# facebookresearch/detectron2

Measured on NVIDIA H100. Metric: Mask R-CNN R50-FPN training hot-path images/sec (custom-op path fwd+bwd, 2 images/GPU), higher is better.
Workload: dtype f32

## Files before the change

detectron2_b200/csrc/abi.cu:

```cuda
#include "common.cuh"

D2B_API int d2b_abi_version(void) { return D2B_ABI_VERSION; }
D2B_API int d2b_cuda_version(void) { return CUDART_VERSION; }
D2B_API const char* d2b_arch(void) { return "sm_90a"; }

namespace {
struct ZeroList {
  int n;
  void* p[D2B_MAX_ZERO];
  size_t bytes[D2B_MAX_ZERO];
  size_t blk0[D2B_MAX_ZERO + 1];
};
constexpr size_t kZeroChunk = 16384;

__global__ void __launch_bounds__(256) zero_buffers_kernel(const ZeroList z) {
  int i = 0;
  while (i + 1 < z.n && blockIdx.x >= z.blk0[i + 1]) ++i;
  const size_t off = (blockIdx.x - z.blk0[i]) * kZeroChunk;
  const size_t len = min(kZeroChunk, z.bytes[i] - off);
  char* base = (char*)z.p[i] + off;
  if ((reinterpret_cast<uintptr_t>(base) & 15) == 0) {
    uint4* q = reinterpret_cast<uint4*>(base);
    for (size_t e = threadIdx.x; e < len / 16; e += 256) q[e] = make_uint4(0u, 0u, 0u, 0u);
    for (size_t e = (len / 16) * 16 + threadIdx.x; e < len; e += 256) base[e] = 0;
  } else {
    for (size_t e = threadIdx.x; e < len; e += 256) base[e] = 0;
  }
}
}

int d2b_num_sms() {
  static std::atomic<int> cached[64];
  int dev = 0;
  if (cudaGetDevice(&dev) != cudaSuccess || dev < 0 || dev >= 64) return 132;
  int n = cached[dev].load(std::memory_order_relaxed);
  if (n <= 0) {
    if (cudaDeviceGetAttribute(&n, cudaDevAttrMultiProcessorCount, dev) != cudaSuccess || n <= 0) return 132;
    cached[dev].store(n, std::memory_order_relaxed);
  }
  return n;
}

int d2b_zero_buffers(void* const* ptrs, const size_t* bytes, int n, cudaStream_t stream) {
  ZeroList z = {};
  size_t blocks = 0;
  for (int i = 0; i < n && z.n < D2B_MAX_ZERO; ++i) {
    if (!ptrs[i] || !bytes[i]) continue;
    z.p[z.n] = ptrs[i];
    z.bytes[z.n] = bytes[i];
    z.blk0[z.n] = blocks;
    blocks += (bytes[i] + kZeroChunk - 1) / kZeroChunk;
    ++z.n;
  }
  z.blk0[z.n] = blocks;
  if (z.n == 0) return D2B_OK;
  if (blocks > 0x7fffffffULL) return D2B_EUNSUPPORTED;
  zero_buffers_kernel<<<(unsigned)blocks, 256, 0, stream>>>(z);
  D2B_CHECK_LAUNCH();
  return D2B_OK;
}
```

detectron2_b200/csrc/common.cuh:

```cuda
#pragma once
#include <cuda_runtime.h>
#include <stdint.h>

#include <atomic>

#include "../../include/d2b200.h"

#define D2B_API extern "C" __attribute__((visibility("default")))

#define D2B_CHECK_LAUNCH()                               \
  do {                                                   \
    cudaError_t e__ = cudaGetLastError();                \
    if (e__ != cudaSuccess) return (int)e__;             \
  } while (0)

#define D2B_CUDA(expr)                                   \
  do {                                                   \
    cudaError_t e__ = (expr);                            \
    if (e__ != cudaSuccess) return (int)e__;             \
  } while (0)

__host__ __device__ static inline int d2b_cdiv(long long a, long long b) { return (int)((a + b - 1) / b); }

int d2b_num_sms();

#define D2B_MAX_ZERO 8
int d2b_zero_buffers(void* const* ptrs, const size_t* bytes, int n, cudaStream_t stream);

#define D2B_ALLOW_BIG_SMEM(kernel)                                                                              \
  do {                                                                                                          \
    static std::atomic<unsigned long long> done__{0ull};                                                        \
    int dev__ = 0;                                                                                              \
    cudaError_t e__ = cudaGetDevice(&dev__);                                                                    \
    if (e__ != cudaSuccess) return (int)e__;                                                                    \
    const unsigned long long bit__ = 1ull << (dev__ & 63);                                                      \
    if (!(done__.load(std::memory_order_acquire) & bit__)) {                                                    \
      cudaFuncAttributes fa__;                                                                                  \
      e__ = cudaFuncGetAttributes(&fa__, kernel);                                                               \
      if (e__ != cudaSuccess) return (int)e__;                                                                  \
      e__ = cudaFuncSetAttribute(kernel, cudaFuncAttributeMaxDynamicSharedMemorySize,                           \
                                 227 * 1024 - (int)fa__.sharedSizeBytes);       \
      if (e__ != cudaSuccess) return (int)e__;                                                                  \
      done__.fetch_or(bit__, std::memory_order_release);                                                        \
    }                                                                                                           \
  } while (0)
```

detectron2_b200/csrc/deform_conv_tc.cu:

```cuda
#include <algorithm>
#include <cstdlib>

#include "common.cuh"
#include "tc_common.cuh"

using namespace d2b_tc;

namespace {

constexpr int kWorkerWarps = 16;
constexpr int kWorkers = kWorkerWarps * 32;
constexpr int kThreads = kWorkers + 128;
constexpr int kLaunchRegs = (65536 / kThreads) & ~7;
constexpr int kWorkerRegs = 112, kSideRegs = 24;
static_assert(kWorkers * kWorkerRegs + (kThreads - kWorkers) * kSideRegs <= kThreads * kLaunchRegs,
              "register budget exceeds the launch allocation");
constexpr int kMaxBN = 128;
constexpr int kRowsPerHalf = 128 / (2 * kWorkerWarps);
constexpr int kTile = 16384;
constexpr int kMaxSmem = 227 * 1024;
constexpr int kGcolPitch = 132;

struct TC {
  int N, Cin, H, W, Cout, kh, kw, sh, sw, ph, pw, dh, dw, G, DG, Ho, Wo, cpg, opg, cpdg, KK, HoWo;
  int pack, SG, cps, ops, cbs, U;
  int tiles_img;
  int stages_img;
  int MC;
  int nks;
  long long off_bs, mask_bs;
  int mask_sigmoid;
};

struct Epi {
  const float* scale;
  const float* shift;
  int relu;
};

struct K1P { int BN, noct, goct, nkp, ksplit, S, tap_bytes, stage_bytes, red; };
struct K2P { int mper, msplit, tap_bytes; };
struct K3P { int BN, noct, sper, nsplit, S, stage_bytes; };

inline size_t align256(size_t v) { return (v + 255) & ~(size_t)255; }

bool make_tc(const d2b_dcn_params* p, TC& d) {
  if (!p) return false;
  d.N = p->N; d.Cin = p->Cin; d.H = p->H; d.W = p->W; d.Cout = p->Cout; d.kh = p->kh; d.kw = p->kw;
  d.sh = p->stride_h; d.sw = p->stride_w; d.ph = p->pad_h; d.pw = p->pad_w; d.dh = p->dil_h; d.dw = p->dil_w;
  d.G = p->groups; d.DG = p->deformable_groups;
  if (d.N < 0 || d.Cin <= 0 || d.H <= 0 || d.W <= 0 || d.Cout <= 0 || d.kh <= 0 || d.kw <= 0 || d.sh <= 0 || d.sw <= 0 ||
      d.ph < 0 || d.pw < 0 || d.dh <= 0 || d.dw <= 0 || d.G <= 0 || d.DG <= 0)
    return false;
  if (d.Cin % d.G || d.Cout % d.G || d.Cin % d.DG) return false;
  d.Ho = (d.H + 2 * d.ph - (d.dh * (d.kh - 1) + 1)) / d.sh + 1;
  d.Wo = (d.W + 2 * d.pw - (d.dw * (d.kw - 1) + 1)) / d.sw + 1;
  if (d.Ho <= 0 || d.Wo <= 0) return false;
  d.cpg = d.Cin / d.G; d.opg = d.Cout / d.G; d.cpdg = d.Cin / d.DG; d.KK = d.kh * d.kw; d.HoWo = d.Ho * d.Wo;
  if (d.cpg >= 64) {
    if (d.cpg % 64) return false;
    d.pack = 1;
  } else {
    if (d.cpg != 16 && d.cpg != 32) return false;
    d.pack = 64 / d.cpg;
    if (d.G % d.pack) return false;
  }
  if (d.cpdg % 64) return false;
  d.SG = d.G / d.pack; d.cps = d.cpg * d.pack; d.ops = d.opg * d.pack; d.cbs = d.cps / 64; d.U = d.KK * d.cbs;
  if (d.ops % 16) return false;
  if (d.KK > 49) return false;
  if ((long long)d.H * d.W * d.Cin >= (1LL << 29)) return false;
  if ((long long)d.HoWo * d.Cout >= (1LL << 31) || (long long)d.Cout * d.cpg * d.KK >= (1LL << 31)) return false;
  d.tiles_img = d2b_cdiv(d.HoWo, 128);
  d.stages_img = d2b_cdiv(d.HoWo, 64);
  d.MC = (d.U + 1) / 2;
  d.nks = d.ops / 64;
  if ((long long)d.N * d.tiles_img > 0x7fffffffLL) return false;
  d.off_bs = (long long)d.DG * 2 * d.KK * d.HoWo;
  d.mask_bs = (long long)d.DG * d.KK * d.HoWo;
  d.mask_sigmoid = 0;
  return true;
}

const float* use_fused_offset_mask(TC& d, const float* offset_mask) {
  d.off_bs = d.mask_bs = (long long)d.DG * 3 * d.KK * d.HoWo;
  d.mask_sigmoid = 1;
  return offset_mask + (size_t)d.DG * 2 * d.KK * d.HoWo;
}

int largest_tile(int n) {
  for (int t = kMaxBN; t >= 16; t >>= 1)
    if (n % t == 0) return t;
  return 0;
}

int best_split(long long base, int work, int max_split, int overhead) {
  int best = 1;
  long long best_cost = -1;
  for (int s = 1; s <= max_split; ++s) {
    const int per = d2b_cdiv(work, s);
    const int parts = d2b_cdiv(work, per);
    const long long cost = (long long)d2b_cdiv(base * parts, d2b_num_sms()) * (per + overhead);
    if (best_cost < 0 || cost < best_cost) {
      best_cost = cost;
      best = parts;
    }
  }
  return best;
}

bool plan_k1(const TC& d, K1P& k, bool colfed = false) {
  k.BN = largest_tile(d.ops);
  if (k.BN < 16) return false;
  k.noct = d.ops / k.BN;
  k.goct = colfed ? 1 : k.noct;
  const int base = d.N * d.tiles_img * d.SG * k.goct;
  k.ksplit = best_split(base, d.KK, d.KK, 1);
  k.nkp = d2b_cdiv(d.KK, k.ksplit);
  k.ksplit = d2b_cdiv(d.KK, k.nkp);
  k.red = k.ksplit > 1;
  const int ndg = d.DG == 1 ? 1 : std::min(d.DG, d2b_cdiv(d.cps, d.cpdg) + 1);
  k.tap_bytes = ndg * k.nkp * 128 * 16;
  k.stage_bytes = 2 * kTile + 2 * k.BN * 128;
  k.S = 3;
  while (k.S > 1 && k.S * k.stage_bytes + k.tap_bytes + 1024 + 128 > kMaxSmem) --k.S;
  return k.S >= 2;
}

bool plan_k1c(const TC& d, K1P& k1, K1P& kc) {
  const long long base = (long long)d.N * d.tiles_img * d.SG * (k1.noct - 1);
  if (k1.goct != 1 || k1.noct < 2 || (long long)d.N * d.tiles_img * (k1.noct - 1) > 0x7fffffffLL) return false;
  kc = k1;
  kc.goct = k1.noct - 1;
  kc.ksplit = best_split(base, d.KK, d.KK, 1);
  kc.nkp = d2b_cdiv(d.KK, kc.ksplit);
  kc.ksplit = d2b_cdiv(d.KK, kc.nkp);
  kc.tap_bytes = 0;
  kc.S = 3;
  while (kc.S > 1 && kc.S * kc.stage_bytes + 1024 + 128 > kMaxSmem) --kc.S;
  if (kc.S < 2) return false;
  k1.red = kc.red = k1.ksplit > 1 || kc.ksplit > 1;
  return true;
}

bool plan_k2(const TC& d, K2P& k) {
  if (d.ops % 64) return false;
  const int base = d.N * d.tiles_img * d.SG;
  k.msplit = best_split(base, d.MC, d.MC, 1);
  k.mper = d2b_cdiv(d.MC, k.msplit);
  k.msplit = d2b_cdiv(d.MC, k.mper);
  const int nkp = std::min(d.KK, (2 * k.mper + d.cbs - 1) / d.cbs + 1);
  const int ndg = d.DG == 1 ? 1 : std::min(d.DG, d2b_cdiv(d.cps, d.cpdg) + 1);
  k.tap_bytes = ndg * nkp * 128 * 16;
  return 2 * 4 * kTile + 128 * kGcolPitch * 4 + k.tap_bytes + 1024 + 128 <= kMaxSmem;
}

bool plan_k3(const TC& d, K3P& k) {
  if (d.ops % 64) return false;
  k.BN = largest_tile(d.ops);
  k.noct = d.ops / k.BN;
  const int units = d.MC * d.SG * k.noct;
  const int total = d.N * d.stages_img;
  k.nsplit = best_split(units, total, std::min(total, 4 * d2b_num_sms()), 3);
  k.sper = d2b_cdiv(total, k.nsplit);
  k.nsplit = d2b_cdiv(total, k.sper);
  k.stage_bytes = 2 * kTile + 2 * k.BN * 128;
  k.S = 3;
  while (k.S > 1 && k.S * k.stage_bytes + 4096 + 1024 + 128 > kMaxSmem) --k.S;
  return k.S >= 2;
}

struct TapRaw {
  float oh, ow, m;
};

__device__ __forceinline__ TapRaw tap_loads(const TC& d, const float* __restrict__ offset, const float* __restrict__ mask,
                                            int b, int dg, int kp, int p) {
  TapRaw r = {0.f, 0.f, 1.f};
  if (p < d.HoWo) {
    const size_t ob = (size_t)b * d.off_bs + ((size_t)dg * 2 * d.KK) * d.HoWo;
    r.oh = __ldg(offset + ob + (size_t)(2 * kp) * d.HoWo + p);
    r.ow = __ldg(offset + ob + (size_t)(2 * kp + 1) * d.HoWo + p);
    if (mask) r.m = __ldg(mask + (size_t)b * d.mask_bs + ((size_t)dg * d.KK + kp) * d.HoWo + p);
  }
  return r;
}

__device__ __forceinline__ int4 tap_finish(const TC& d, const TapRaw& r, bool has_mask, int kp, int p) {
  int4 t = make_int4(0, 0, 0, 0);
  if (p < d.HoWo) {
    const int ho = p / d.Wo, wo = p - ho * d.Wo;
    const int ki = kp / d.kw, kj = kp - ki * d.kw;
    const float hf = (float)(ho * d.sh - d.ph + ki * d.dh) + r.oh;
    const float wf = (float)(wo * d.sw - d.pw + kj * d.dw) + r.ow;
    float m = r.m;
    if (has_mask && d.mask_sigmoid) m = 1.f / (1.f + expf(-m));
    if (hf > -1.f && wf > -1.f && hf < (float)d.H && wf < (float)d.W) {
      const float hfl = floorf(hf), wfl = floorf(wf);
      const int hl = (int)hfl, wl = (int)wfl;
      const bool t0 = hl >= 0, t1 = hl + 1 <= d.H - 1, l0 = wl >= 0, l1 = wl + 1 <= d.W - 1;
      const int flags = (t0 && l0 ? 1 : 0) | (t0 && l1 ? 2 : 0) | (t1 && l0 ? 4 : 0) | (t1 && l1 ? 8 : 0);
      t.x = ((hl * d.W + wl + d.W + 1) << 4) | flags;
      t.y = __float_as_int(hf - hfl);
      t.z = __float_as_int(wf - wfl);
      t.w = __float_as_int(m);
    }
  }
  return t;
}

__device__ __forceinline__ int4 make_tap(const TC& d, const float* __restrict__ offset, const float* __restrict__ mask,
                                         int b, int dg, int kp, int p) {
  return tap_finish(d, tap_loads(d, offset, mask, b, dg, kp, p), mask != nullptr, kp, p);
}

struct Taps4 {
  float4 v0, v1, v2, v3;
};

__device__ __forceinline__ void load_corners(const float* __restrict__ xcb, uint32_t Cin, uint32_t rs, int code, Taps4& t) {
  const float* __restrict__ p = xcb + (uint32_t)(code >> 4) * Cin;
  const float4 z = make_float4(0.f, 0.f, 0.f, 0.f);
  t.v0 = (code & 1) ? __ldg(reinterpret_cast<const float4*>(p)) : z;
  t.v1 = (code & 2) ? __ldg(reinterpret_cast<const float4*>(p + Cin)) : z;
  t.v2 = (code & 4) ? __ldg(reinterpret_cast<const float4*>(p + rs)) : z;
  t.v3 = (code & 8) ? __ldg(reinterpret_cast<const float4*>(p + (rs + Cin))) : z;
}

__device__ __forceinline__ void interp4(const Taps4& t, float w0, float w1, float w2, float w3, float (&v)[4]) {
  const F2 z = f2_pack(0.f, 0.f), p0 = f2_pack(w0, w0), p1 = f2_pack(w1, w1), p2 = f2_pack(w2, w2), p3 = f2_pack(w3, w3);
  F2 a = f2_fma(p0, f2_pack(t.v0.x, t.v0.y), z), b = f2_fma(p0, f2_pack(t.v0.z, t.v0.w), z);
  a = f2_fma(p1, f2_pack(t.v1.x, t.v1.y), a);
  b = f2_fma(p1, f2_pack(t.v1.z, t.v1.w), b);
  a = f2_fma(p2, f2_pack(t.v2.x, t.v2.y), a);
  b = f2_fma(p2, f2_pack(t.v2.z, t.v2.w), b);
  a = f2_fma(p3, f2_pack(t.v3.x, t.v3.y), a);
  b = f2_fma(p3, f2_pack(t.v3.z, t.v3.w), b);
  f2_unpack(a, v[0], v[1]);
  f2_unpack(b, v[2], v[3]);
}

__device__ __forceinline__ void gather_store(const Taps4& t, int4 tap, uint8_t* a_hi, uint8_t* a_lo, uint32_t off,
                                             bool split) {
  const float lh = __int_as_float(tap.y), lw = __int_as_float(tap.z), m = __int_as_float(tap.w);
  const float hh = 1.f - lh, hw = 1.f - lw;
  float v[4];
  interp4(t, hh * hw * m, hh * lw * m, lh * hw * m, lh * lw * m, v);
  uint2 hi, lo;
  split4(v, hi, lo);
  *reinterpret_cast<uint2*>(a_hi + off) = hi;
  if (split) *reinterpret_cast<uint2*>(a_lo + off) = lo;
}

template <int BN, int kTransA, int kSplit>
__device__ __forceinline__ void mma_stage_(float (&acc)[BN / 4], uint32_t a_hi, uint32_t a_lo, uint32_t b_hi, uint32_t b_lo) {
  const int g = (threadIdx.x >> 7);
  const uint32_t ao = kTransA ? (uint32_t)(g & 1) * 8192u : (uint32_t)(g & 1) * 64u * 128u;
  const uint32_t bo = (uint32_t)(g >> 1) * (uint32_t)(BN / 2) * 128u;
  const uint32_t lbo = kTransA ? 8192u : 0u;
  wgmma_fence();
#pragma unroll
  for (int kk = 0; kk < 4; ++kk) {
    const uint32_t ak = ao + (kTransA ? (uint32_t)kk * 2048u : (uint32_t)kk * 32u), bk = bo + (uint32_t)kk * 32u;
    Wgmma<BN / 2, kTransA>::mma(acc, wgmma_desc(a_hi + ak, lbo, 1024), wgmma_desc(b_hi + bk, 0, 1024), 1);
    if (kSplit) {
      Wgmma<BN / 2, kTransA>::mma(acc, wgmma_desc(a_hi + ak, lbo, 1024), wgmma_desc(b_lo + bk, 0, 1024), 1);
      Wgmma<BN / 2, kTransA>::mma(acc, wgmma_desc(a_lo + ak, lbo, 1024), wgmma_desc(b_hi + bk, 0, 1024), 1);
    }
  }
  wgmma_commit();
}
template <int BN, int kTransA>
__device__ __forceinline__ void mma_stage(float (&acc)[BN / 4], uint32_t a_hi, uint32_t a_lo, uint32_t b_hi, uint32_t b_lo,
                                          int split) {
  if (split) mma_stage_<BN, kTransA, 1>(acc, a_hi, a_lo, b_hi, b_lo);
  else mma_stage_<BN, kTransA, 0>(acc, a_hi, a_lo, b_hi, b_lo);
}

template <int BN>
__device__ __forceinline__ int acc_row(int i) {
  const int t = threadIdx.x & 127;
  return (threadIdx.x >> 7 & 1) * 64 + (t >> 5) * 16 + ((t & 31) >> 2) + ((i >> 1) & 1) * 8;
}
template <int BN>
__device__ __forceinline__ int acc_col(int i) {
  return (threadIdx.x >> 8) * (BN / 2) + (i >> 2) * 8 + (threadIdx.x & 3) * 2 + (i & 1);
}

template <int BN>
__device__ __forceinline__ void fwd_epilogue(const float (&acc)[BN / 4], const Epi& ep, const TC& d, const K1P& k,
                                             float* __restrict__ out, int b, int p0, int oc0) {
  const bool add_shift = ep.shift != nullptr && blockIdx.z == 0;
#pragma unroll
  for (int i = 0; i < BN / 4; ++i) {
    const int p = p0 + acc_row<BN>(i);
    if (p >= d.HoWo) continue;
    const int oc = oc0 + acc_col<BN>(i);
    float* dst = out + ((size_t)b * d.Cout + oc) * d.HoWo + p;
    float v = acc[i];
    if (k.red) {
      red_add(dst, v + ((add_shift && !ep.scale && !ep.relu) ? __ldg(ep.shift + oc) : 0.f));
    } else {
      if (ep.scale) v *= __ldg(ep.scale + oc);
      if (ep.shift) v += __ldg(ep.shift + oc);
      if (ep.relu) v = fmaxf(v, 0.f);
      *dst = v;
    }
  }
}

template <int BN>
__global__ void __launch_bounds__(kThreads, 1) dcn_fwd_tc_kernel(const float* __restrict__ xh,
                                                                   const float* __restrict__ offset,
                                                                   const float* __restrict__ mask,
                                                                   const uint8_t* __restrict__ wt, const Epi ep, const TC d,
                                                                   const K1P k, const int split, float* __restrict__ out,
                                                                   uint8_t* __restrict__ cols) {
  extern __shared__ uint8_t smem_raw[];
  uint8_t* smem = smem_raw + ((1024u - (smem_u32(smem_raw) & 1023u)) & 1023u);
  int4* taps = reinterpret_cast<int4*>(smem + k.S * k.stage_bytes);
  uint64_t* bars = reinterpret_cast<uint64_t*>(reinterpret_cast<uint8_t*>(taps) + k.tap_bytes);
  uint64_t* full_bar = bars;
  uint64_t* empty_bar = bars + k.S;

  const int tid = threadIdx.x, warp = tid >> 5, lane = tid & 31;
  const int b = blockIdx.x / d.tiles_img, p0 = (blockIdx.x - b * d.tiles_img) * 128;
  const int sg = blockIdx.y / k.goct, oct = blockIdx.y - sg * k.goct;
  const int kp0 = blockIdx.z * k.nkp, nkp = min(d.KK, kp0 + k.nkp) - kp0;
  const int nt = nkp * d.cbs;
  const int dg0 = (sg * d.cps) / d.cpdg;
  const bool saving = cols != nullptr && oct == 0;

  if (tid == 0) {
    for (int s = 0; s < k.S; ++s) {
      mbar_init(&full_bar[s], kWorkerWarps + 1);
      mbar_init(&empty_bar[s], kWorkerWarps + (saving ? 1 : 0));
    }
    mbar_init_fence();
  }
  if (tid < kWorkers) {
    const int ndg = ((sg + 1) * d.cps - 1) / d.cpdg - dg0 + 1;
    for (int i = tid; i < ndg * nkp * 128; i += kWorkers) {
      const int row = i & 127, r = i >> 7;
      const int dgl = r / nkp, kpl = r - dgl * nkp;
      taps[i] = make_tap(d, offset, mask, b, dg0 + dgl, kp0 + kpl, p0 + row);
    }
  }
  __syncthreads();
  if (warp < kWorkerWarps) reg_alloc<kWorkerRegs>();
  else reg_dealloc<kSideRegs>();

  if (warp < kWorkerWarps) {
    const int half = lane >> 4, q = lane & 15;
    const float* __restrict__ ximg = xh + (size_t)b * d.H * d.W * d.Cin - (size_t)(d.W + 1) * d.Cin;
    const uint32_t ucin = (uint32_t)d.Cin, urs = (uint32_t)(d.W * d.Cin);
    float acc[BN / 4];
#pragma unroll
    for (int i = 0; i < BN / 4; ++i) acc[i] = 0.f;
    int kpl = 0, cb = 0;
    auto stage = [&](int t) {
      const int s = t % k.S;
      const uint32_t par = (uint32_t)((t / k.S) & 1);
      const int cbase = sg * d.cps + cb * 64;
      const int4* __restrict__ tp = taps + ((cbase / d.cpdg - dg0) * nkp + kpl) * 128;
      const float* __restrict__ xc = ximg + cbase + q * 4;
      uint8_t* a_hi = smem + s * k.stage_bytes;
      uint8_t* a_lo = a_hi + kTile;
      mbar_wait(&empty_bar[s], par ^ 1u);
      {
        int4 tap[kRowsPerHalf];
        Taps4 c[kRowsPerHalf];
#pragma unroll
        for (int j = 0; j < kRowsPerHalf; ++j) tap[j] = tp[warp * 2 * kRowsPerHalf + j * 2 + half];
#pragma unroll
        for (int j = 0; j < kRowsPerHalf; ++j) load_corners(xc, ucin, urs, tap[j].x, c[j]);
#pragma unroll
        for (int j = 0; j < kRowsPerHalf; ++j) {
          const uint32_t r = (uint32_t)(warp * 2 * kRowsPerHalf + j * 2 + half);
          gather_store(c[j], tap[j], a_hi, a_lo, swz128(r, (uint32_t)(q >> 1)) + (uint32_t)(q & 1) * 8u, split != 0);
        }
      }
      fence_proxy_async();
      __syncwarp();
      if (lane == 0) mbar_arrive(&full_bar[s]);
      mbar_wait(&full_bar[s], par);
      const uint32_t sa = smem_u32(a_hi), sb = sa + 2 * kTile;
      mma_stage<BN, 0>(acc, sa, sa + kTile, sb, sb + (uint32_t)BN * 128u, split);
      if (++cb == d.cbs) { cb = 0; ++kpl; }
    };
    stage(0);
    for (int t = 1; t < nt; ++t) {
      stage(t);
      wgmma_wait<1>();
      __syncwarp();
      if (lane == 0) mbar_arrive(&empty_bar[(t - 1) % k.S]);
    }
    wgmma_wait<0>();
    fwd_epilogue<BN>(acc, ep, d, k, out, b, p0, sg * d.ops + oct * k.BN);
  } else if (warp == kWorkerWarps) {
    if (lane == 0) {
      const uint32_t bytes = (uint32_t)(split ? 2 : 1) * (uint32_t)k.BN * 128u;
      for (int t = 0; t < nt; ++t) {
        const int s = t % k.S;
        const uint32_t par = (uint32_t)((t / k.S) & 1);
        mbar_wait(&empty_bar[s], par ^ 1u);
        const size_t tile = ((size_t)(sg * k.noct + oct) * d.U + (size_t)kp0 * d.cbs + t);
        mbar_arrive_expect_tx(&full_bar[s], bytes);
        bulk_g2s(smem + s * k.stage_bytes + 2 * kTile, wt + tile * (size_t)(2 * k.BN * 128), bytes, &full_bar[s]);
      }
    }
  } else if (warp == kWorkerWarps + 1) {
    if (saving && lane == 0) {
      const uint32_t tile_bytes = (uint32_t)(split ? 2 : 1) * (uint32_t)kTile;
      for (int t = 0; t < nt; ++t) {
        const int s = t % k.S;
        const uint32_t par = (uint32_t)((t / k.S) & 1);
        mbar_wait(&full_bar[s], par);
        const size_t tile = ((size_t)blockIdx.x * d.SG + sg) * d.U + (size_t)kp0 * d.cbs + t;
        bulk_s2g(cols + tile * tile_bytes, smem + s * k.stage_bytes, tile_bytes);
        bulk_commit();
        bulk_wait_read0();
        mbar_arrive(&empty_bar[s]);
      }
      bulk_wait0();
    }
  }
}

template <int BN>
__global__ void __launch_bounds__(kThreads, 1) dcn_fwd_cols_kernel(const uint8_t* __restrict__ cols,
                                                                   const uint8_t* __restrict__ wt, const Epi ep, const TC d,
                                                                   const K1P k, const int split, float* __restrict__ out) {
  extern __shared__ uint8_t smem_raw[];
  uint8_t* smem = smem_raw + ((1024u - (smem_u32(smem_raw) & 1023u)) & 1023u);
  uint64_t* bars = reinterpret_cast<uint64_t*>(smem + k.S * k.stage_bytes);
  uint64_t* full_bar = bars;
  uint64_t* empty_bar = bars + k.S;

  const int tid = threadIdx.x, warp = tid >> 5, lane = tid & 31;
  const int tile = blockIdx.x / k.goct, oct = 1 + (blockIdx.x - tile * k.goct);
  const int b = tile / d.tiles_img, p0 = (tile - b * d.tiles_img) * 128;
  const int sg = blockIdx.y;
  const int kp0 = blockIdx.z * k.nkp, nkp = min(d.KK, kp0 + k.nkp) - kp0;
  const int nt = nkp * d.cbs;

  if (tid == 0) {
    for (int s = 0; s < k.S; ++s) {
      mbar_init(&full_bar[s], 1);
      mbar_init(&empty_bar[s], kWorkerWarps);
    }
    mbar_init_fence();
  }
  __syncthreads();
  if (warp < kWorkerWarps) reg_alloc<kWorkerRegs>();
  else reg_dealloc<kSideRegs>();

  if (warp < kWorkerWarps) {
    float acc[BN / 4];
#pragma unroll
    for (int i = 0; i < BN / 4; ++i) acc[i] = 0.f;
    auto issue = [&](int t) {
      const int s = t % k.S;
      mbar_wait(&full_bar[s], (uint32_t)((t / k.S) & 1));
      const uint32_t sa = smem_u32(smem + s * k.stage_bytes), sb = sa + 2 * kTile;
      mma_stage<BN, 0>(acc, sa, sa + kTile, sb, sb + (uint32_t)BN * 128u, split);
    };
    issue(0);
    for (int t = 1; t < nt; ++t) {
      issue(t);
      wgmma_wait<1>();
      __syncwarp();
      if (lane == 0) mbar_arrive(&empty_bar[(t - 1) % k.S]);
    }
    wgmma_wait<0>();
    fwd_epilogue<BN>(acc, ep, d, k, out, b, p0, sg * d.ops + oct * k.BN);
  } else if (warp == kWorkerWarps) {
    if (lane == 0) {
      const uint32_t parts = split ? 2u : 1u;
      const uint32_t abytes = parts * (uint32_t)kTile;
      const size_t u0 = (size_t)kp0 * d.cbs;
      const uint8_t* asrc = cols + (((size_t)tile * d.SG + sg) * d.U + u0) * abytes;
      const uint8_t* bsrc = wt + ((size_t)(sg * k.noct + oct) * d.U + u0) * (size_t)(2 * BN * 128);
      int s = 0;
      uint32_t par = 1u;
      for (int t = nt; t > 0; --t, asrc += abytes, bsrc += 2 * BN * 128) {
        mbar_wait(&empty_bar[s], par);
        mbar_arrive_expect_tx(&full_bar[s], abytes / 128u * (128u + BN));
        bulk_g2s(smem + s * k.stage_bytes, asrc, abytes, &full_bar[s]);
        bulk_g2s(smem + s * k.stage_bytes + 2 * kTile, bsrc, abytes / 128u * BN, &full_bar[s]);
        if (++s == k.S) {
          s = 0;
          par ^= 1u;
        }
      }
    }
  }
}

__global__ void __launch_bounds__(kThreads, 1) dcn_bwd_data_tc_kernel(const float* __restrict__ xh,
                                                                      const float* __restrict__ offset,
                                                                      const float* __restrict__ mask,
                                                                      const uint8_t* __restrict__ gt,
                                                                      const uint8_t* __restrict__ wt, const TC d,
                                                                      const K2P k, const int split,
                                                                      float* __restrict__ gxh, float* __restrict__ goff,
                                                                      float* __restrict__ gmask) {
  extern __shared__ uint8_t smem_raw[];
  uint8_t* smem = smem_raw + ((1024u - (smem_u32(smem_raw) & 1023u)) & 1023u);
  constexpr int kStage = 4 * kTile;
  float* gcol = reinterpret_cast<float*>(smem + 2 * kStage);
  int4* taps = reinterpret_cast<int4*>(smem + 2 * kStage + 128 * kGcolPitch * 4);
  uint64_t* bars = reinterpret_cast<uint64_t*>(reinterpret_cast<uint8_t*>(taps) + k.tap_bytes);
  uint64_t* full_bar = bars;
  uint64_t* empty_bar = bars + 2;

  const int tid = threadIdx.x, warp = tid >> 5, lane = tid & 31;
  const int b = blockIdx.x / d.tiles_img, pt = blockIdx.x - b * d.tiles_img, p0 = pt * 128;
  const int sg = blockIdx.y;
  const int m0 = blockIdx.z * k.mper, m1 = min(d.MC, m0 + k.mper), nm = m1 - m0;
  const int u_begin = 2 * m0, u_end = min(d.U, 2 * m1);
  const int kp0 = u_begin / d.cbs, nkp = (u_end - 1) / d.cbs - kp0 + 1;
  const int dg0 = (sg * d.cps) / d.cpdg;

  if (tid == 0) {
    for (int s = 0; s < 2; ++s) {
      mbar_init(&full_bar[s], 1);
      mbar_init(&empty_bar[s], kWorkerWarps);
    }
    mbar_init_fence();
  }
  if (tid < kWorkers) {
    const int ndg = ((sg + 1) * d.cps - 1) / d.cpdg - dg0 + 1;
    for (int i = tid; i < ndg * nkp * 128; i += kWorkers) {
      const int row = i & 127, r = i >> 7;
      const int dgl = r / nkp, kpl = r - dgl * nkp;
      taps[i] = make_tap(d, offset, mask, b, dg0 + dgl, kp0 + kpl, p0 + row);
    }
  }
  __syncthreads();
  if (warp < kWorkerWarps) reg_alloc<kWorkerRegs>();
  else reg_dealloc<kSideRegs>();

  if (warp < kWorkerWarps) {
    const int half = lane >> 4, q = lane & 15;
    const size_t img_off = (size_t)b * d.H * d.W * d.Cin - (size_t)(d.W + 1) * d.Cin;
    const float* __restrict__ ximg = xh + img_off;
    float* __restrict__ gimg = gxh ? gxh + img_off : nullptr;
    const uint32_t ucin = (uint32_t)d.Cin, urs = (uint32_t)(d.W * d.Cin);
    constexpr int R = kRowsPerHalf;
    float sh[R], sw[R], sm[R];
#pragma unroll
    for (int j = 0; j < R; ++j) sh[j] = sw[j] = sm[j] = 0.f;
    int cur_kp = -1, cur_dg = -1;

    auto flush = [&]() {
      if (cur_kp < 0) return;
      static_assert(R == 4, "the reduction below is written for 4 rows per half-warp");
      float v12[12];
#pragma unroll
      for (int j = 0; j < R; ++j) {
        v12[3 * j] = sh[j];
        v12[3 * j + 1] = sw[j];
        v12[3 * j + 2] = sm[j];
      }
      const bool b8 = q & 8, b4 = q & 4, b2 = q & 2, b1 = q & 1;
      float v6[6], v3[3];
#pragma unroll
      for (int i = 0; i < 6; ++i) {
        const float keep = b8 ? v12[i + 6] : v12[i], send = b8 ? v12[i] : v12[i + 6];
        v6[i] = keep + __shfl_xor_sync(0xffffffffu, send, 8);
      }
#pragma unroll
      for (int i = 0; i < 3; ++i) {
        const float keep = b4 ? v6[i + 3] : v6[i], send = b4 ? v6[i] : v6[i + 3];
        v3[i] = keep + __shfl_xor_sync(0xffffffffu, send, 4);
      }
      const float k0 = b2 ? v3[2] : v3[0], s0 = b2 ? v3[0] : v3[2];
      const float k1 = b2 ? 0.f : v3[1], s1 = b2 ? v3[1] : 0.f;
      const float u0 = k0 + __shfl_xor_sync(0xffffffffu, s0, 2);
      const float u1 = k1 + __shfl_xor_sync(0xffffffffu, s1, 2);
      float v = (b1 ? u1 : u0) + __shfl_xor_sync(0xffffffffu, b1 ? u0 : u1, 1);
      {
        const int j = q >> 2, which = q & 3;
        const int row = warp * 2 * R + j * 2 + half;
        const int p = p0 + row;
        if (which < 3 && p < d.HoWo) {
          if (which < 2) {
            if (goff) red_add(goff + (size_t)b * d.off_bs + ((size_t)cur_dg * 2 * d.KK + 2 * cur_kp + which) * d.HoWo + p, v);
          } else if (gmask) {
            if (d.mask_sigmoid) {
              const float m = __int_as_float(taps[((cur_dg - dg0) * nkp + (cur_kp - kp0)) * 128 + row].w);
              v *= m * (1.f - m);
            }
            red_add(gmask + (size_t)b * d.mask_bs + ((size_t)cur_dg * d.KK + cur_kp) * d.HoWo + p, v);
          }
        }
      }
#pragma unroll
      for (int j = 0; j < R; ++j) sh[j] = sw[j] = sm[j] = 0.f;
    };

    for (int ml = 0; ml < nm; ++ml) {
      const int buf = ml & 1;
      const int m = m0 + ml;
      const int nu = (2 * m + 1 < d.U) ? 2 : 1;
      {
        float acc[32];
#pragma unroll
        for (int i = 0; i < 32; ++i) acc[i] = 0.f;
        for (int ks = 0; ks < d.nks; ++ks) {
          const int c = ml * d.nks + ks, s = c & 1;
          mbar_wait(&full_bar[s], (uint32_t)((c >> 1) & 1));
          const uint32_t sa = smem_u32(smem + s * kStage);
          mma_stage<128, 0>(acc, sa, sa + kTile, sa + 2 * kTile, sa + 3 * kTile, split);
          wgmma_wait<0>();
          __syncwarp();
          if (lane == 0) mbar_arrive(&empty_bar[s]);
        }
#pragma unroll
        for (int i = 0; i < 32; i += 2)
          *reinterpret_cast<float2*>(gcol + acc_row<128>(i) * kGcolPitch + acc_col<128>(i)) = make_float2(acc[i], acc[i + 1]);
      }
      named_bar_sync(1, kWorkers);
      for (int ul = 0; ul < nu; ++ul) {
        const int u = 2 * m + ul;
        const int kp = u / d.cbs, cb = u - kp * d.cbs;
        const int cbase = sg * d.cps + cb * 64;
        const int dg = cbase / d.cpdg;
        if (kp != cur_kp || dg != cur_dg) {
          flush();
          cur_kp = kp;
          cur_dg = dg;
        }
        const int4* __restrict__ tp = taps + ((dg - dg0) * nkp + (kp - kp0)) * 128;
        const float* __restrict__ xc = ximg + cbase + q * 4;
        float* __restrict__ gc = gimg + cbase + q * 4;
        constexpr int kB2 = 2;
#pragma unroll
        for (int it = 0; it < R / kB2; ++it) {
          int4 tap[kB2];
          Taps4 c[kB2];
#pragma unroll
          for (int e = 0; e < kB2; ++e) tap[e] = tp[warp * 2 * R + (it * kB2 + e) * 2 + half];
#pragma unroll
          for (int e = 0; e < kB2; ++e) load_corners(xc, ucin, urs, tap[e].x, c[e]);
#pragma unroll
          for (int e = 0; e < kB2; ++e) {
            if ((tap[e].x & 15) == 0) continue;
            const int j = it * kB2 + e;
            const int row = warp * 2 * R + j * 2 + half;
            const float4 g4 = *reinterpret_cast<const float4*>(gcol + row * kGcolPitch + ul * 64 + q * 4);
            const float lh = __int_as_float(tap[e].y), lw = __int_as_float(tap[e].z), mk = __int_as_float(tap[e].w);
            const float hh = 1.f - lh, hw = 1.f - lw;
            const float w0 = hh * hw, w1 = hh * lw, w2 = lh * hw, w3 = lh * lw;
            const F2 LH = f2_pack(lh, lh), LW = f2_pack(lw, lw), HH = f2_pack(hh, hh), HW = f2_pack(hw, hw);
            const F2 W0 = f2_pack(w0, w0), W1 = f2_pack(w1, w1), W2 = f2_pack(w2, w2), W3 = f2_pack(w3, w3);
            const F2 MK = f2_pack(mk, mk);
            const F2 G[2] = {f2_pack(g4.x, g4.y), f2_pack(g4.z, g4.w)};
            const F2 A0[2] = {f2_pack(c[e].v0.x, c[e].v0.y), f2_pack(c[e].v0.z, c[e].v0.w)};
            const F2 A1[2] = {f2_pack(c[e].v1.x, c[e].v1.y), f2_pack(c[e].v1.z, c[e].v1.w)};
            const F2 A2[2] = {f2_pack(c[e].v2.x, c[e].v2.y), f2_pack(c[e].v2.z, c[e].v2.w)};
            const F2 A3[2] = {f2_pack(c[e].v3.x, c[e].v3.y), f2_pack(c[e].v3.z, c[e].v3.w)};
            F2 GM[2];
            F2 th2 = f2_pack(0.f, 0.f), tw2 = th2, tm2 = th2;
#pragma unroll
            for (int i = 0; i < 2; ++i) {
              GM[i] = f2_mul(G[i], MK);
              const F2 dh = f2_fma(LW, f2_sub(A3[i], A1[i]), f2_mul(HW, f2_sub(A2[i], A0[i])));
              const F2 dw = f2_fma(LH, f2_sub(A3[i], A2[i]), f2_mul(HH, f2_sub(A1[i], A0[i])));
              const F2 val = f2_fma(W3, A3[i], f2_fma(W2, A2[i], f2_fma(W1, A1[i], f2_mul(W0, A0[i]))));
              th2 = f2_fma(GM[i], dh, th2);
              tw2 = f2_fma(GM[i], dw, tw2);
              tm2 = f2_fma(G[i], val, tm2);
            }
            {
              float e0, e1;
              f2_unpack(th2, e0, e1);
              sh[j] += e0 + e1;
              f2_unpack(tw2, e0, e1);
              sw[j] += e0 + e1;
              f2_unpack(tm2, e0, e1);
              sm[j] += e0 + e1;
            }
            if (gimg) {
              float* gp = gc + (uint32_t)(tap[e].x >> 4) * ucin;
              red_add_v4_if(tap[e].x & 1, gp, f2_mul(GM[0], W0), f2_mul(GM[1], W0));
              red_add_v4_if(tap[e].x & 2, gp + ucin, f2_mul(GM[0], W1), f2_mul(GM[1], W1));
              red_add_v4_if(tap[e].x & 4, gp + urs, f2_mul(GM[0], W2), f2_mul(GM[1], W2));
              red_add_v4_if(tap[e].x & 8, gp + (urs + ucin), f2_mul(GM[0], W3), f2_mul(GM[1], W3));
            }
          }
        }
      }
      named_bar_sync(1, kWorkers);
    }
    flush();
  } else if (warp == kWorkerWarps) {
    if (lane == 0) {
      const uint32_t half_bytes = (uint32_t)(split ? 2 : 1) * (uint32_t)kTile;
      int c = 0;
      for (int ml = 0; ml < nm; ++ml) {
        const int m = m0 + ml;
        for (int ks = 0; ks < d.nks; ++ks, ++c) {
          const int s = c & 1;
          const uint32_t par = (uint32_t)((c >> 1) & 1);
          mbar_wait(&empty_bar[s], par ^ 1u);
          mbar_arrive_expect_tx(&full_bar[s], 2 * half_bytes);
          const size_t atile = (((size_t)b * d.tiles_img + pt) * d.SG + sg) * d.nks + ks;
          const size_t btile = ((size_t)sg * d.MC + m) * d.nks + ks;
          bulk_g2s(smem + s * kStage, gt + atile * (size_t)(2 * kTile), half_bytes, &full_bar[s]);
          bulk_g2s(smem + s * kStage + 2 * kTile, wt + btile * (size_t)(2 * kTile), half_bytes, &full_bar[s]);
        }
      }
    }
  }
}

template <int BN>
__device__ __forceinline__ void gw_tile_store(const float (&acc)[BN / 4], float* __restrict__ tile, int pitch) {
#pragma unroll
  for (int i = 0; i < BN / 4; i += 2) red_add_v2(tile + (size_t)acc_row<BN>(i) * pitch + acc_col<BN>(i), acc[i], acc[i + 1]);
}

__global__ void dcn_gw_reduce_kernel(const float* __restrict__ part, const TC d, float* __restrict__ gw) {
  const long long total = (long long)d.SG * d.U * 64 * d.ops;
  const long long idx = (long long)blockIdx.x * blockDim.x + threadIdx.x;
  if (idx >= total) return;
  const int ocl = (int)(idx % d.ops);
  const long long r = idx / d.ops;
  const int rowu = (int)(r % ((long long)d.U * 64)), sg = (int)(r / ((long long)d.U * 64));
  const int u = rowu >> 6, ch = rowu & 63;
  const int kp = u / d.cbs, cb = u - kp * d.cbs;
  const int ec = sg * d.cps + cb * 64 + ch, egrp = ec / d.cpg, ecin = ec - egrp * d.cpg;
  const int oc = sg * d.ops + ocl;
  if (oc / d.opg != egrp) return;
  gw[((size_t)oc * d.cpg + ecin) * d.KK + kp] = __ldg(part + ((size_t)sg * d.MC * 128 + rowu) * d.ops + ocl);
}

constexpr int kRedOc = 16, kRedCh = 16;
__global__ void __launch_bounds__(256) dcn_gw_reduce_tile_kernel(const float* __restrict__ part, const TC d,
                                                                  float* __restrict__ gw) {
  __shared__ float tile[9 * kRedCh][kRedOc + 1];
  const int per_sg = d.cps / kRedCh;
  const int sg = blockIdx.x / per_sg, c0 = (blockIdx.x - sg * per_sg) * kRedCh;
  const int cb = c0 >> 6, ch0 = c0 & 63;
  const int ocl0 = blockIdx.y * kRedOc;
  const int tid = threadIdx.x;
  {
    const int j = tid & (kRedOc - 1), r0 = tid / kRedOc;
    for (int row = r0; row < d.KK * kRedCh; row += 256 / kRedOc) {
      const int kp = row / kRedCh, ch = row - kp * kRedCh;
      tile[row][j] = __ldg(part + ((size_t)sg * d.MC * 128 + (size_t)(kp * d.cbs + cb) * 64 + ch0 + ch) * d.ops + ocl0 + j);
    }
  }
  __syncthreads();
  const int ec0 = sg * d.cps + c0;
  for (int i = tid; i < kRedOc * kRedCh * d.KK; i += 256) {
    const int j = i / (kRedCh * d.KK), e = i - j * (kRedCh * d.KK);
    const int ch = e / d.KK, kp = e - ch * d.KK;
    const int oc = sg * d.ops + ocl0 + j, grp = oc / d.opg;
    const int ec = ec0 + ch;
    if (ec / d.cpg == grp) gw[((size_t)oc * d.cpg + (ec - grp * d.cpg)) * d.KK + kp] = tile[kp * kRedCh + ch][j];
  }
}

template <int BN>
__global__ void __launch_bounds__(kThreads, 1) dcn_bwd_weight_tc_kernel(const float* __restrict__ xh,
                                                                        const float* __restrict__ offset,
                                                                        const float* __restrict__ mask,
                                                                        const uint8_t* __restrict__ gt, const TC d,
                                                                        const K3P k, const int split,
                                                                        float* __restrict__ gw) {
  extern __shared__ uint8_t smem_raw[];
  uint8_t* smem = smem_raw + ((1024u - (smem_u32(smem_raw) & 1023u)) & 1023u);
  int4* tap_s = reinterpret_cast<int4*>(smem + k.S * k.stage_bytes);
  uint64_t* bars = reinterpret_cast<uint64_t*>(reinterpret_cast<uint8_t*>(tap_s) + 4096);
  uint64_t* full_bar = bars;
  uint64_t* empty_bar = bars + k.S;

  const int tid = threadIdx.x, warp = tid >> 5, lane = tid & 31;
  const int mb = blockIdx.y;
  const int sg = blockIdx.x / k.noct, oct = blockIdx.x - sg * k.noct;
  const int total = d.N * d.stages_img;
  const int gs0 = blockIdx.z * k.sper, gs1 = min(total, gs0 + k.sper), ns = gs1 - gs0;

  if (tid == 0) {
    for (int s = 0; s < k.S; ++s) {
      mbar_init(&full_bar[s], kWorkerWarps + 1);
      mbar_init(&empty_bar[s], kWorkerWarps);
    }
    mbar_init_fence();
  }
  __syncthreads();
  if (warp < kWorkerWarps) reg_alloc<kWorkerRegs>();
  else reg_dealloc<kSideRegs>();

  if (warp < kWorkerWarps) {
    const int half = lane >> 4, q = lane & 15;
    const int u = 2 * mb + half;
    const bool u_ok = u < d.U;
    const int kp = u_ok ? u / d.cbs : 0, cb = u_ok ? u - kp * d.cbs : 0;
    const int cbase = sg * d.cps + cb * 64;
    const int dg = cbase / d.cpdg;
    constexpr int PX = 64 / kWorkerWarps;
    const int tl_half = (lane / PX) & 1, tl_j = lane % PX;
    const int tl_u = 2 * mb + tl_half;
    const bool tl_ok = lane < 2 * PX && tl_u < d.U;
    const int tl_kp = tl_ok ? tl_u / d.cbs : 0;
    const int tl_dg = tl_ok ? (sg * d.cps + (tl_u - tl_kp * d.cbs) * 64) / d.cpdg : 0;
    int4* my_taps = tap_s + warp * 2 * (2 * PX);
    auto stage_of = [&](int i, int& b, int& pbase) {
      const int gs = gs0 + i;
      b = gs / d.stages_img;
      pbase = (gs - b * d.stages_img) * 64;
    };
    if (ns > 0) {
      int b0, pb0;
      stage_of(0, b0, pb0);
      if (lane < 2 * PX) my_taps[lane] = tl_ok ? make_tap(d, offset, mask, b0, tl_dg, tl_kp, pb0 + warp * PX + tl_j) : make_int4(0, 0, 0, 0);
    }
    __syncwarp();
    float acc[BN / 4];
#pragma unroll
    for (int i = 0; i < BN / 4; ++i) acc[i] = 0.f;
    auto stage = [&](int i) {
      const int s = i % k.S;
      const uint32_t par = (uint32_t)((i / k.S) & 1);
      int b, pbase, bn = 0, pbn = 0;
      stage_of(i, b, pbase);
      const bool have_next = i + 1 < ns;
      TapRaw raw = {0.f, 0.f, 1.f};
      if (have_next) {
        stage_of(i + 1, bn, pbn);
        if (tl_ok) raw = tap_loads(d, offset, mask, bn, tl_dg, tl_kp, pbn + warp * PX + tl_j);
      }
      const float* __restrict__ xc = xh + ((size_t)b * d.H * d.W - (size_t)(d.W + 1)) * d.Cin + cbase + q * 4;
      const uint32_t ucin = (uint32_t)d.Cin, urs = (uint32_t)(d.W * d.Cin);
      uint8_t* a_hi = smem + s * k.stage_bytes + half * 8192;
      uint8_t* a_lo = a_hi + kTile;
      const int4* cur = my_taps + (i & 1) * (2 * PX) + half * PX;
      mbar_wait(&empty_bar[s], par ^ 1u);
      {
        int4 tap[PX];
        Taps4 c[PX];
#pragma unroll
        for (int j = 0; j < PX; ++j) tap[j] = cur[j];
#pragma unroll
        for (int j = 0; j < PX; ++j) load_corners(xc, ucin, urs, tap[j].x, c[j]);
#pragma unroll
        for (int j = 0; j < PX; ++j) {
          const uint32_t r = (uint32_t)(warp * PX + j);
          gather_store(c[j], tap[j], a_hi, a_lo, swz128(r, (uint32_t)(q >> 1)) + (uint32_t)(q & 1) * 8u, split != 0);
        }
      }
      if (have_next && lane < 2 * PX)
        my_taps[((i + 1) & 1) * (2 * PX) + lane] =
            tl_ok ? tap_finish(d, raw, mask != nullptr, tl_kp, pbn + warp * PX + tl_j) : make_int4(0, 0, 0, 0);
      fence_proxy_async();
      __syncwarp();
      if (lane == 0) mbar_arrive(&full_bar[s]);
      mbar_wait(&full_bar[s], par);
      const uint32_t sa = smem_u32(smem + s * k.stage_bytes), sb = sa + 2 * kTile;
      mma_stage<BN, 1>(acc, sa, sa + kTile, sb, sb + (uint32_t)BN * 128u, split);
    };
    stage(0);
    for (int i = 1; i < ns; ++i) {
      stage(i);
      wgmma_wait<1>();
      __syncwarp();
      if (lane == 0) mbar_arrive(&empty_bar[(i - 1) % k.S]);
    }
    wgmma_wait<0>();
    gw_tile_store<BN>(acc, gw + ((size_t)sg * d.MC * 128 + (size_t)mb * 128) * d.ops + (size_t)oct * k.BN, d.ops);
  } else if (warp == kWorkerWarps) {
    if (lane == 0) {
      const uint32_t bytes = (uint32_t)(split ? 2 : 1) * (uint32_t)k.BN * 128u;
      for (int i = 0; i < ns; ++i) {
        const int s = i % k.S;
        const uint32_t par = (uint32_t)((i / k.S) & 1);
        mbar_wait(&empty_bar[s], par ^ 1u);
        mbar_arrive_expect_tx(&full_bar[s], bytes);
        const size_t tile = ((size_t)(gs0 + i) * d.SG + sg) * k.noct + oct;
        bulk_g2s(smem + s * k.stage_bytes + 2 * kTile, gt + tile * (size_t)(2 * k.BN * 128), bytes, &full_bar[s]);
      }
    }
  }
}

template <int BN>
__global__ void __launch_bounds__(kThreads, 1) dcn_bwd_weight_cols_kernel(const uint8_t* __restrict__ cols,
                                                                          const uint8_t* __restrict__ gt, const TC d,
                                                                          const K3P k, const int S, const int split,
                                                                          float* __restrict__ gw) {
  extern __shared__ uint8_t smem_raw[];
  uint8_t* smem = smem_raw + ((1024u - (smem_u32(smem_raw) & 1023u)) & 1023u);
  uint64_t* bars = reinterpret_cast<uint64_t*>(smem + S * k.stage_bytes);
  uint64_t* full_bar = bars;
  uint64_t* empty_bar = bars + S;

  const int tid = threadIdx.x, warp = tid >> 5, lane = tid & 31;
  const int mb = blockIdx.y;
  const int sg = blockIdx.x / k.noct, oct = blockIdx.x - sg * k.noct;
  const int total = d.N * d.stages_img;
  const int gs0 = blockIdx.z * k.sper, gs1 = min(total, gs0 + k.sper), ns = gs1 - gs0;
  const int nu = (2 * mb + 1 < d.U) ? 2 : 1;

  if (tid == 0) {
    for (int s = 0; s < S; ++s) {
      mbar_init(&full_bar[s], 1);
      mbar_init(&empty_bar[s], kWorkerWarps);
    }
    mbar_init_fence();
  }
  if (nu == 1 && tid < kWorkers) {
    for (int s = 0; s < S; ++s)
      for (int i = tid; i < 2 * 512; i += kWorkers) {
        const int part = i >> 9, w = i & 511;
        reinterpret_cast<uint4*>(smem + s * k.stage_bytes + part * kTile + 8192)[w] = make_uint4(0, 0, 0, 0);
      }
    fence_proxy_async();
  }
  __syncthreads();
  if (warp < kWorkerWarps) reg_alloc<kWorkerRegs>();
  else reg_dealloc<kSideRegs>();

  if (warp < kWorkerWarps) {
    float acc[BN / 4];
#pragma unroll
    for (int i = 0; i < BN / 4; ++i) acc[i] = 0.f;
    auto issue = [&](int i) {
      const int s = i % S;
      mbar_wait(&full_bar[s], (uint32_t)((i / S) & 1));
      const uint32_t sa = smem_u32(smem + s * k.stage_bytes), sb = sa + 2 * kTile;
      mma_stage<BN, 1>(acc, sa, sa + kTile, sb, sb + (uint32_t)BN * 128u, split);
    };
    issue(0);
    for (int i = 1; i < ns; ++i) {
      issue(i);
      wgmma_wait<1>();
      __syncwarp();
      if (lane == 0) mbar_arrive(&empty_bar[(i - 1) % S]);
    }
    wgmma_wait<0>();
    gw_tile_store<BN>(acc, gw + ((size_t)sg * d.MC * 128 + (size_t)mb * 128) * d.ops + (size_t)oct * k.BN, d.ops);
  } else if (warp == kWorkerWarps) {
    if (lane == 0) {
      const uint32_t parts = split ? 2u : 1u;
      const uint32_t tile_bytes = parts * (uint32_t)kTile;
      const uint32_t gbytes = parts * (uint32_t)k.BN * 128u;
      for (int i = 0; i < ns; ++i) {
        const int s = i % S;
        const uint32_t par = (uint32_t)((i / S) & 1);
        const int gs = gs0 + i;
        const int b = gs / d.stages_img, st = gs - b * d.stages_img;
        mbar_wait(&empty_bar[s], par ^ 1u);
        mbar_arrive_expect_tx(&full_bar[s], (uint32_t)nu * parts * 8192u + gbytes);
        uint8_t* stage = smem + s * k.stage_bytes;
        const uint8_t* src =
            cols + ((((size_t)b * d.tiles_img + (st >> 1)) * d.SG + sg) * d.U + 2 * mb) * tile_bytes + (size_t)(st & 1) * 8192;
        for (int ul = 0; ul < nu; ++ul)
          for (uint32_t part = 0; part < parts; ++part)
            bulk_g2s(stage + part * kTile + ul * 8192, src + (size_t)ul * tile_bytes + (size_t)part * kTile, 8192u, &full_bar[s]);
        const size_t tile = ((size_t)gs * d.SG + sg) * k.noct + oct;
        bulk_g2s(stage + 2 * kTile, gt + tile * (size_t)(2 * k.BN * 128), gbytes, &full_bar[s]);
      }
    }
  }
}

__device__ __forceinline__ void split8(const float (&v)[8], uint4& hi, uint4& lo) {
  split2(v[0], v[1], hi.x, lo.x);
  split2(v[2], v[3], hi.y, lo.y);
  split2(v[4], v[5], hi.z, lo.z);
  split2(v[6], v[7], hi.w, lo.w);
}

__device__ __forceinline__ float w_elem(const float* __restrict__ w, const TC& d, int oc, int c, int kp) {
  const int g = c / d.cpg;
  if (oc / d.opg != g) return 0.f;
  return __ldg(w + ((size_t)oc * d.cpg + (c - g * d.cpg)) * d.KK + kp);
}

__global__ void dcn_wtile_fwd_kernel(const float* __restrict__ w, const TC d, int BN, int noct, uint8_t* __restrict__ dst) {
  const long long idx = (long long)blockIdx.x * blockDim.x + threadIdx.x;
  const long long total = (long long)d.SG * noct * d.U * BN * 8;
  if (idx >= total) return;
  const int c16 = (int)(idx & 7);
  const int r = (int)((idx >> 3) % BN);
  const long long tile = idx / (8LL * BN);
  const int u = (int)(tile % d.U);
  const int oct = (int)((tile / d.U) % noct);
  const int sg = (int)(tile / ((long long)d.U * noct));
  const int kp = u / d.cbs, cb = u - kp * d.cbs;
  const int oc = sg * d.ops + oct * BN + r;
  float v[8];
#pragma unroll
  for (int e = 0; e < 8; ++e) v[e] = w_elem(w, d, oc, sg * d.cps + cb * 64 + c16 * 8 + e, kp);
  uint4 hi, lo;
  split8(v, hi, lo);
  uint8_t* base = dst + tile * (size_t)(2 * BN * 128);
  *reinterpret_cast<uint4*>(base + swz128((uint32_t)r, (uint32_t)c16)) = hi;
  *reinterpret_cast<uint4*>(base + BN * 128 + swz128((uint32_t)r, (uint32_t)c16)) = lo;
}

__global__ void dcn_wtile_bwd_kernel(const float* __restrict__ w, const TC d, uint8_t* __restrict__ dst) {
  const long long idx = (long long)blockIdx.x * blockDim.x + threadIdx.x;
  const long long total = (long long)d.SG * d.MC * d.nks * 128 * 8;
  if (idx >= total) return;
  const int c16 = (int)(idx & 7);
  const int r = (int)((idx >> 3) & 127);
  const long long tile = idx >> 10;
  const int ks = (int)(tile % d.nks);
  const int m = (int)((tile / d.nks) % d.MC);
  const int sg = (int)(tile / ((long long)d.nks * d.MC));
  const int u = 2 * m + (r >> 6);
  float v[8];
#pragma unroll
  for (int e = 0; e < 8; ++e) v[e] = 0.f;
  if (u < d.U) {
    const int kp = u / d.cbs, cb = u - kp * d.cbs;
    const int c = sg * d.cps + cb * 64 + (r & 63);
#pragma unroll
    for (int e = 0; e < 8; ++e) v[e] = w_elem(w, d, sg * d.ops + ks * 64 + c16 * 8 + e, c, kp);
  }
  uint4 hi, lo;
  split8(v, hi, lo);
  uint8_t* base = dst + tile * (size_t)(2 * kTile);
  *reinterpret_cast<uint4*>(base + swz128((uint32_t)r, (uint32_t)c16)) = hi;
  *reinterpret_cast<uint4*>(base + kTile + swz128((uint32_t)r, (uint32_t)c16)) = lo;
}

__device__ __forceinline__ float gout_elem(const float* __restrict__ gout, const float* __restrict__ ysaved, const Epi& ep,
                                           size_t idx, int oc) {
  float g = __ldg(gout + idx);
  if (ep.relu && !(__ldg(ysaved + idx) > 0.f)) g = 0.f;
  if (ep.scale) g *= __ldg(ep.scale + oc);
  return g;
}

__global__ void __launch_bounds__(256) dcn_gout_px_tiles_kernel(const float* __restrict__ gout,
                                                                const float* __restrict__ ysaved, const Epi ep, const TC d,
                                                                uint8_t* __restrict__ dst, uint8_t* __restrict__ dst_oc,
                                                                int BN, int noct) {
  __shared__ float t[64][33];
  const long long tile = blockIdx.x;
  const int ks = (int)(tile % d.nks);
  const int sg = (int)((tile / d.nks) % d.SG);
  const int pt = (int)((tile / ((long long)d.nks * d.SG)) % d.tiles_img);
  const int b = (int)(tile / ((long long)d.nks * d.SG * d.tiles_img));
  const int r0 = blockIdx.y * 32;
  const int p0 = pt * 128 + r0, oc0 = sg * d.ops + ks * 64;
  const int tid = threadIdx.x;
#pragma unroll
  for (int i = 0; i < 8; ++i) {
    const int e = tid + i * 256;
    const int o = e >> 5, pp = e & 31;
    const int p = p0 + pp;
    t[o][pp] = p < d.HoWo ? gout_elem(gout, ysaved, ep, ((size_t)b * d.Cout + oc0 + o) * d.HoWo + p, oc0 + o) : 0.f;
  }
  __syncthreads();
  uint8_t* base = dst + tile * (size_t)(2 * kTile);
  {
    const int r = tid >> 3, c16 = tid & 7;
    float v[8];
#pragma unroll
    for (int i = 0; i < 8; ++i) v[i] = t[c16 * 8 + i][r];
    uint4 hi, lo;
    split8(v, hi, lo);
    *reinterpret_cast<uint4*>(base + swz128((uint32_t)(r0 + r), (uint32_t)c16)) = hi;
    *reinterpret_cast<uint4*>(base + kTile + swz128((uint32_t)(r0 + r), (uint32_t)c16)) = lo;
  }
  if (dst_oc) {
    const int o = tid >> 2, ch = tid & 3;
    const int ocs = ks * 64 + o;
    const int oct = ocs / BN, row = ocs - oct * BN;
    const int pglob = pt * 128 + r0;
    const int ps = pglob >> 6, c16 = ((pglob & 63) >> 3) + ch;
    float v[8];
#pragma unroll
    for (int i = 0; i < 8; ++i) v[i] = t[o][ch * 8 + i];
    uint4 hi, lo;
    split8(v, hi, lo);
    if (ps < d.stages_img) {
      const size_t tile_oc = (((size_t)b * d.stages_img + ps) * d.SG + sg) * noct + oct;
      uint8_t* bo = dst_oc + tile_oc * (size_t)(2 * BN * 128);
      *reinterpret_cast<uint4*>(bo + swz128((uint32_t)row, (uint32_t)c16)) = hi;
      *reinterpret_cast<uint4*>(bo + BN * 128 + swz128((uint32_t)row, (uint32_t)c16)) = lo;
    }
  }
}

__global__ void dcn_gout_oc_tiles_kernel(const float* __restrict__ gout, const float* __restrict__ ysaved, const Epi ep,
                                         const TC d, int BN, int noct, uint8_t* __restrict__ dst) {
  const long long idx = (long long)blockIdx.x * blockDim.x + threadIdx.x;
  const long long total = (long long)d.N * d.stages_img * d.SG * noct * BN * 8;
  if (idx >= total) return;
  const int c16 = (int)(idx & 7);
  const int r = (int)((idx >> 3) % BN);
  const long long tile = idx / (8LL * BN);
  const int oct = (int)(tile % noct);
  const int sg = (int)((tile / noct) % d.SG);
  const int ps = (int)((tile / ((long long)noct * d.SG)) % d.stages_img);
  const int b = (int)(tile / ((long long)noct * d.SG * d.stages_img));
  const int oc = sg * d.ops + oct * BN + r;
  const size_t src = ((size_t)b * d.Cout + oc) * d.HoWo;
  float v[8];
#pragma unroll
  for (int e = 0; e < 8; ++e) {
    const int p = ps * 64 + c16 * 8 + e;
    v[e] = p < d.HoWo ? gout_elem(gout, ysaved, ep, src + p, oc) : 0.f;
  }
  uint4 hi, lo;
  split8(v, hi, lo);
  uint8_t* base = dst + tile * (size_t)(2 * BN * 128);
  *reinterpret_cast<uint4*>(base + swz128((uint32_t)r, (uint32_t)c16)) = hi;
  *reinterpret_cast<uint4*>(base + BN * 128 + swz128((uint32_t)r, (uint32_t)c16)) = lo;
}

__global__ void __launch_bounds__(256) nhwc_to_nchw_kernel(const float* __restrict__ src, int C, int HW,
                                                           float* __restrict__ dst) {
  __shared__ float t[64][33];
  const int hw0 = blockIdx.x * 64, c0 = blockIdx.y * 32;
  const float* __restrict__ s = src + (size_t)blockIdx.z * HW * C;
  float* __restrict__ o = dst + (size_t)blockIdx.z * C * HW;
  const int tid = threadIdx.x;
  for (int e = tid; e < 64 * 32; e += 256) {
    const int pp = e >> 5, cc = e & 31;
    t[pp][cc] = (hw0 + pp < HW && c0 + cc < C) ? __ldg(s + (size_t)(hw0 + pp) * C + c0 + cc) : 0.f;
  }
  __syncthreads();
  for (int e = tid; e < 64 * 32; e += 256) {
    const int cc = e >> 6, pp = e & 63;
    if (hw0 + pp < HW && c0 + cc < C) o[(size_t)(c0 + cc) * HW + hw0 + pp] = t[pp][cc];
  }
}

__global__ void dcn_epilogue_kernel(float* __restrict__ y, long long total, int Cout, int HoWo, const Epi ep) {
  const long long i = (long long)blockIdx.x * blockDim.x + threadIdx.x;
  if (i >= total) return;
  const int oc = (int)((i / HoWo) % Cout);
  float v = y[i];
  if (ep.scale) v *= __ldg(ep.scale + oc);
  if (ep.shift) v += __ldg(ep.shift + oc);
  if (ep.relu) v = fmaxf(v, 0.f);
  y[i] = v;
}

int to_nhwc(const float* x, const TC& d, float* dst, cudaStream_t stream) {
  d2b_pyramid P = {};
  P.num_levels = 1;
  P.feat[0] = x;
  P.H[0] = d.H;
  P.W[0] = d.W;
  P.scale[0] = 1.f;
  float* dsts[1] = {dst};
  return d2b_pyramid_nchw_to_nhwc(&P, d.N, d.Cin, dsts, (void*)stream);
}

}

int d2b_deform_conv_tc_supported(const d2b_dcn_params* p) {
  TC d;
  K1P k1;
  return make_tc(p, d) && plan_k1(d, k1);
}

int d2b_deform_conv_tc_bwd_supported(const d2b_dcn_params* p) {
  TC d;
  K2P k2;
  K3P k3;
  return make_tc(p, d) && plan_k2(d, k2) && plan_k3(d, k3);
}

size_t d2b_deform_conv_tc_fwd_workspace(const d2b_dcn_params* p, int x_nhwc) {
  TC d;
  K1P k;
  if (!make_tc(p, d) || !plan_k1(d, k)) return 0;
  size_t b = align256((size_t)d.SG * k.noct * d.U * 2 * k.BN * 128);
  if (!x_nhwc) b += align256(sizeof(float) * (size_t)d.N * d.H * d.W * d.Cin);
  return b;
}

size_t d2b_deform_conv_tc_cols_bytes(const d2b_dcn_params* p, int precision) {
  TC d;
  K1P k;
  if (precision == 0 || !make_tc(p, d) || !plan_k1(d, k)) return 0;
  return (size_t)d.N * d.tiles_img * d.SG * d.U * (size_t)(precision == 1 ? 2 : 1) * kTile;
}

int d2b_deform_conv_forward_tc(const float* x, const float* offset, const float* mask, const float* weight,
                               const float* scale, const float* shift, int relu, const d2b_dcn_params* p, int precision,
                               int tcflags, float* out, void* cols, void* workspace, size_t workspace_bytes, void* stream_) {
  cudaStream_t stream = (cudaStream_t)stream_;
  const int x_nhwc = tcflags & 1;
  TC d;
  K1P k;
  if (!make_tc(p, d) || !plan_k1(d, k)) return D2B_EUNSUPPORTED;
  if (d.N == 0) return D2B_OK;
  if (tcflags & 2) {
    if (mask) return D2B_EINVAL;
    mask = use_fused_offset_mask(d, offset);
  }
  if (!workspace || workspace_bytes < d2b_deform_conv_tc_fwd_workspace(p, x_nhwc)) return D2B_EWORKSPACE;
  if ((reinterpret_cast<uintptr_t>(workspace) & 255) || (x_nhwc && (reinterpret_cast<uintptr_t>(x) & 15)) ||
      (reinterpret_cast<uintptr_t>(cols) & 15))
    return D2B_EINVAL;
  uint8_t* ws = reinterpret_cast<uint8_t*>(workspace);
  uint8_t* wt = ws;
  ws += align256((size_t)d.SG * k.noct * d.U * 2 * k.BN * 128);
  const float* xh = x;
  if (!x_nhwc) {
    float* xn = reinterpret_cast<float*>(ws);
    int rc = to_nhwc(x, d, xn, stream);
    if (rc) return rc;
    xh = xn;
  }
  {
    const long long total = (long long)d.SG * k.noct * d.U * k.BN * 8;
    dcn_wtile_fwd_kernel<<<d2b_cdiv(total, 256), 256, 0, stream>>>(weight, d, k.BN, k.noct, wt);
    D2B_CHECK_LAUNCH();
  }
  K1P kc;
  bool colfed = false;
  if (cols && k.noct > 1) {
    K1P k1;
    if (plan_k1(d, k1, true) && plan_k1c(d, k1, kc)) {
      k = k1;
      colfed = true;
    }
  }
  if (k.red) D2B_CUDA(cudaMemsetAsync(out, 0, sizeof(float) * (size_t)d.N * d.Cout * d.HoWo, stream));
  const int smem_bytes = k.S * k.stage_bytes + k.tap_bytes + 1024 + 128;
  const int split = precision == 1 ? 1 : 0;
  const Epi ep = {scale, shift, relu};
  dim3 grid(d.N * d.tiles_img, d.SG * k.goct, k.ksplit);
#define D2B_LAUNCH_K1(BN)                                                                                              \
  {                                                                                                                    \
    D2B_ALLOW_BIG_SMEM(dcn_fwd_tc_kernel<BN>);                                                                         \
    dcn_fwd_tc_kernel<BN><<<grid, kThreads, smem_bytes, stream>>>(xh, offset, mask, wt, ep, d, k, split, out,        \
                                                                    reinterpret_cast<uint8_t*>(cols));                 \
  }
  if (k.BN == 16) D2B_LAUNCH_K1(16)
  else if (k.BN == 32) D2B_LAUNCH_K1(32)
  else if (k.BN == 64) D2B_LAUNCH_K1(64)
  else D2B_LAUNCH_K1(128)
#undef D2B_LAUNCH_K1
  D2B_CHECK_LAUNCH();
  if (colfed) {
    const int smem_c = kc.S * kc.stage_bytes + 1024 + 128;
    dim3 grid_c(d.N * d.tiles_img * kc.goct, d.SG, kc.ksplit);
    const uint8_t* cl = reinterpret_cast<const uint8_t*>(cols);
#define D2B_LAUNCH_K1C(BN)                                                                                             \
  {                                                                                                                    \
    D2B_ALLOW_BIG_SMEM(dcn_fwd_cols_kernel<BN>);                                                                       \
    dcn_fwd_cols_kernel<BN><<<grid_c, kThreads, smem_c, stream>>>(cl, wt, ep, d, kc, split, out);                      \
  }
    if (kc.BN == 16) D2B_LAUNCH_K1C(16)
    else if (kc.BN == 32) D2B_LAUNCH_K1C(32)
    else if (kc.BN == 64) D2B_LAUNCH_K1C(64)
    else D2B_LAUNCH_K1C(128)
#undef D2B_LAUNCH_K1C
    D2B_CHECK_LAUNCH();
  }
  if (k.red && (scale || relu)) {
    const long long total = (long long)d.N * d.Cout * d.HoWo;
    dcn_epilogue_kernel<<<d2b_cdiv(total, 256), 256, 0, stream>>>(out, total, d.Cout, d.HoWo, ep);
    D2B_CHECK_LAUNCH();
  }
  return D2B_OK;
}

size_t d2b_deform_conv_tc_bwd_workspace(const d2b_dcn_params* p, int x_nhwc, int need_data, int need_weight) {
  TC d;
  K2P k2;
  K3P k3;
  if (!make_tc(p, d) || !plan_k2(d, k2) || !plan_k3(d, k3)) return 0;
  size_t b = 0;
  const size_t xbytes = align256(sizeof(float) * (size_t)d.N * d.H * d.W * d.Cin);
  if (!x_nhwc) b += xbytes;
  if (need_data && !x_nhwc) b += xbytes;
  if (need_data) {
    b += align256((size_t)d.N * d.tiles_img * d.SG * d.nks * 2 * kTile);
    b += align256((size_t)d.SG * d.MC * d.nks * 2 * kTile);
  }
  if (need_weight) {
    b += align256((size_t)d.N * d.stages_img * d.SG * k3.noct * 2 * k3.BN * 128);
    b += align256(sizeof(float) * (size_t)d.SG * d.MC * 128 * d.ops);
  }
  return b;
}

int d2b_deform_conv_backward_tc(const float* x, const float* offset, const float* mask, const float* weight,
                                const float* grad_out, const float* scale, const float* y_saved, int relu,
                                const d2b_dcn_params* p, int precision, int tcflags, const void* cols, float* grad_x,
                                float* grad_offset, float* grad_mask, float* grad_weight, void* workspace,
                                size_t workspace_bytes, void* stream_) {
  cudaStream_t stream = (cudaStream_t)stream_;
  const int x_nhwc = tcflags & 1;
  TC d;
  K2P k2;
  K3P k3;
  if (!make_tc(p, d) || !plan_k2(d, k2) || !plan_k3(d, k3)) return D2B_EUNSUPPORTED;
  const int need_data = (grad_x || grad_offset || grad_mask) ? 1 : 0, need_weight = grad_weight ? 1 : 0;
  const bool fused_om = (tcflags & 2) != 0;
  if (fused_om && (mask || grad_mask)) return D2B_EINVAL;
  if (relu && !y_saved) return D2B_EINVAL;
  const size_t nx = (size_t)d.N * d.H * d.W * d.Cin, noff = (size_t)d.N * d.DG * (fused_om ? 3 : 2) * d.KK * d.HoWo;
  const size_t nm = (size_t)d.N * d.DG * d.KK * d.HoWo, nw = (size_t)d.Cout * d.cpg * d.KK;
  if (fused_om) {
    mask = use_fused_offset_mask(d, offset);
    if (grad_offset) grad_mask = grad_offset + (size_t)d.DG * 2 * d.KK * d.HoWo;
  }
  const Epi ep = {scale, nullptr, relu};
  if (d.N == 0 || (!need_data && !need_weight)) {
    void* zp[3] = {grad_offset, fused_om ? nullptr : grad_mask, grad_weight};
    size_t zb[3] = {noff * 4, nm * 4, nw * 4};
    return d2b_zero_buffers(zp, zb, 3, stream);
  }
  if (!workspace || workspace_bytes < d2b_deform_conv_tc_bwd_workspace(p, x_nhwc, need_data, need_weight)) return D2B_EWORKSPACE;
  if ((reinterpret_cast<uintptr_t>(workspace) & 255) || (x_nhwc && (reinterpret_cast<uintptr_t>(x) & 15)) ||
      (x_nhwc && grad_x && (reinterpret_cast<uintptr_t>(grad_x) & 15)) || (reinterpret_cast<uintptr_t>(cols) & 15))
    return D2B_EINVAL;
  const int split = precision == 1 ? 1 : 0;
  uint8_t* ws = reinterpret_cast<uint8_t*>(workspace);
  const size_t xbytes = align256(sizeof(float) * nx);
  const float* xh = x;
  if (!x_nhwc) {
    float* xn = reinterpret_cast<float*>(ws);
    ws += xbytes;
    int rc = to_nhwc(x, d, xn, stream);
    if (rc) return rc;
    xh = xn;
  }
  float* gxh = nullptr;
  if (need_data && grad_x) gxh = x_nhwc ? grad_x : reinterpret_cast<float*>(ws);
  uint8_t* gt_px = nullptr;
  uint8_t* wt = nullptr;
  if (need_data) {
    if (!x_nhwc) ws += xbytes;
    gt_px = ws;
    ws += align256((size_t)d.N * d.tiles_img * d.SG * d.nks * 2 * kTile);
    wt = ws;
    ws += align256((size_t)d.SG * d.MC * d.nks * 2 * kTile);
  }
  uint8_t* gt_oc = need_weight ? ws : nullptr;
  float* gw_part = nullptr;
  if (need_weight) {
    ws += align256((size_t)d.N * d.stages_img * d.SG * k3.noct * 2 * k3.BN * 128);
    gw_part = reinterpret_cast<float*>(ws);
  }
  {
    void* zp[4] = {grad_offset, fused_om ? nullptr : grad_mask, gxh, gw_part};
    size_t zb[4] = {noff * 4, nm * 4, nx * 4, sizeof(float) * (size_t)d.SG * d.MC * 128 * d.ops};
    int rc = d2b_zero_buffers(zp, zb, 4, stream);
    if (rc) return rc;
  }
  if (need_data) {
    dcn_gout_px_tiles_kernel<<<dim3((unsigned)((size_t)d.N * d.tiles_img * d.SG * d.nks), 4), 256, 0, stream>>>(
        grad_out, y_saved, ep, d, gt_px, gt_oc, k3.BN, k3.noct);
    D2B_CHECK_LAUNCH();
    {
      const long long total = (long long)d.SG * d.MC * d.nks * 128 * 8;
      dcn_wtile_bwd_kernel<<<d2b_cdiv(total, 256), 256, 0, stream>>>(weight, d, wt);
      D2B_CHECK_LAUNCH();
    }
    const int smem_bytes = 2 * 4 * kTile + 128 * kGcolPitch * 4 + k2.tap_bytes + 1024 + 128;
    D2B_ALLOW_BIG_SMEM(dcn_bwd_data_tc_kernel);
    dim3 grid(d.N * d.tiles_img, d.SG, k2.msplit);
    dcn_bwd_data_tc_kernel<<<grid, kThreads, smem_bytes, stream>>>(xh, offset, mask, gt_px, wt, d, k2, split, gxh, grad_offset,
                                                                  mask ? grad_mask : nullptr);
    D2B_CHECK_LAUNCH();
    if (grad_x && !x_nhwc) {
      dim3 g2(d2b_cdiv(d.H * d.W, 64), d2b_cdiv(d.Cin, 32), d.N);
      nhwc_to_nchw_kernel<<<g2, 256, 0, stream>>>(gxh, d.Cin, d.H * d.W, grad_x);
      D2B_CHECK_LAUNCH();
    }
  }
  if (need_weight) {
    if (!need_data) {
      const long long total = (long long)d.N * d.stages_img * d.SG * k3.noct * k3.BN * 8;
      dcn_gout_oc_tiles_kernel<<<d2b_cdiv(total, 256), 256, 0, stream>>>(grad_out, y_saved, ep, d, k3.BN, k3.noct, gt_oc);
      D2B_CHECK_LAUNCH();
    }
    dim3 grid(d.SG * k3.noct, d.MC, k3.nsplit);
    if (cols) {
      const int S = std::min(6, (kMaxSmem - 2048) / k3.stage_bytes);
      const int smem_bytes = S * k3.stage_bytes + 1024 + 128;
      const uint8_t* cl = reinterpret_cast<const uint8_t*>(cols);
#define D2B_LAUNCH_K3C(BN)                                                                                             \
  {                                                                                                                      \
    D2B_ALLOW_BIG_SMEM(dcn_bwd_weight_cols_kernel<BN>);                                                                \
    dcn_bwd_weight_cols_kernel<BN><<<grid, kThreads, smem_bytes, stream>>>(cl, gt_oc, d, k3, S, split, gw_part);       \
  }
      if (k3.BN == 64) D2B_LAUNCH_K3C(64)
      else D2B_LAUNCH_K3C(128)
#undef D2B_LAUNCH_K3C
    } else {
      const int smem_bytes = k3.S * k3.stage_bytes + 4096 + 1024 + 128;
#define D2B_LAUNCH_K3(BN)                                                                                              \
  {                                                                                                                      \
    D2B_ALLOW_BIG_SMEM(dcn_bwd_weight_tc_kernel<BN>);                                                                  \
    dcn_bwd_weight_tc_kernel<BN><<<grid, kThreads, smem_bytes, stream>>>(xh, offset, mask, gt_oc, d, k3, split, gw_part); \
  }
      if (k3.BN == 64) D2B_LAUNCH_K3(64)
      else D2B_LAUNCH_K3(128)
#undef D2B_LAUNCH_K3
    }
    D2B_CHECK_LAUNCH();
    {
      if (d.KK <= 9) {
        dcn_gw_reduce_tile_kernel<<<dim3(d.SG * (d.cps / kRedCh), d.ops / kRedOc), 256, 0, stream>>>(gw_part, d, grad_weight);
      } else {
        const long long total = (long long)d.SG * d.U * 64 * d.ops;
        dcn_gw_reduce_kernel<<<d2b_cdiv(total, 256), 256, 0, stream>>>(gw_part, d, grad_weight);
      }
      D2B_CHECK_LAUNCH();
    }
  }
  return D2B_OK;
}
```

detectron2_b200/csrc/roi_align.cu:

```cuda
#include <cuda_bf16.h>
#include <cuda_fp16.h>

#include <algorithm>

#include "common.cuh"

namespace {

constexpr int kThreads = 256;

template <int DT>
struct Elem;
template <>
struct Elem<D2B_F32> {
  using T = float;
  static __device__ __forceinline__ float ld(const T* __restrict__ p) { return __ldg(p); }
  static __device__ __forceinline__ void st(T* __restrict__ p, float v) { *p = v; }
};
template <>
struct Elem<D2B_F16> {
  using T = __half;
  static __device__ __forceinline__ float ld(const T* __restrict__ p) { return __half2float(__ldg(p)); }
  static __device__ __forceinline__ void st(T* __restrict__ p, float v) { *p = __float2half_rn(v); }
};
template <>
struct Elem<D2B_BF16> {
  using T = __nv_bfloat16;
  static __device__ __forceinline__ float ld(const T* __restrict__ p) { return __bfloat162float(__ldg(p)); }
  static __device__ __forceinline__ void st(T* __restrict__ p, float v) { *p = __float2bfloat16_rn(v); }
};
#define D2B_DISPATCH_DTYPE(dt, ...)                  \
  do {                                               \
    if ((dt) == D2B_F32) {                           \
      constexpr int DT = D2B_F32;                    \
      __VA_ARGS__;                                   \
    } else if ((dt) == D2B_F16) {                    \
      constexpr int DT = D2B_F16;                    \
      __VA_ARGS__;                                   \
    } else {                                         \
      constexpr int DT = D2B_BF16;                   \
      __VA_ARGS__;                                   \
    }                                                \
  } while (0)
static inline bool dtype_ok(int dt) { return dt == D2B_F32 || dt == D2B_F16 || dt == D2B_BF16; }

struct RoiGeom {
  int b;
  float start_h, start_w, bin_h, bin_w;
  int gh, gw;
  float inv_count;
  float count_raw;
  float ctr_h, ctr_w, cos_t, sin_t;
};

struct Pyr {
  int num_levels;
  const float* feat[D2B_MAX_LEVELS];
  float* grad[D2B_MAX_LEVELS];
  int H[D2B_MAX_LEVELS], W[D2B_MAX_LEVELS];
  float scale[D2B_MAX_LEVELS];
  int min_level, max_level, canonical_level;
  float canonical_box_size;
  const float* level_rois;
};

template <bool ROT = false>
__device__ __forceinline__ int pick_level(const Pyr& P, const float* __restrict__ roi) {
  if (P.num_levels == 1) return 0;
  const float area = ROT ? roi[3] * roi[4] : (roi[3] - roi[1]) * (roi[4] - roi[2]);
  const float size = sqrtf(area);
  float lvl = floorf((float)P.canonical_level + log2f(size / P.canonical_box_size + 1e-8f));
  if (!(lvl == lvl)) return -1;
  lvl = fminf(fmaxf(lvl, (float)P.min_level), (float)P.max_level);
  return (int)lvl - P.min_level;
}

template <bool ROT>
__device__ __forceinline__ RoiGeom load_geom(const float* __restrict__ roi, float scale, int PH, int PW, int sr,
                                             int aligned, bool dead = false) {
  RoiGeom g;
  g.b = (int)roi[0];
  float rw, rh;
  if (ROT) {
    g.ctr_w = roi[1] * scale - 0.5f;
    g.ctr_h = roi[2] * scale - 0.5f;
    rw = roi[3] * scale;
    rh = roi[4] * scale;
    float theta = (float)((double)roi[5] * 3.14159265358979323846 / 180.0);
    sincosf(theta, &g.sin_t, &g.cos_t);
    g.start_h = -rh / 2.0f;
    g.start_w = -rw / 2.0f;
  } else {
    float off = aligned ? 0.5f : 0.0f;
    float sw = roi[1] * scale - off, sh = roi[2] * scale - off;
    float ew = roi[3] * scale - off, eh = roi[4] * scale - off;
    rw = ew - sw;
    rh = eh - sh;
    if (!aligned) {
      rw = fmaxf(rw, 1.f);
      rh = fmaxf(rh, 1.f);
    }
    g.start_h = sh;
    g.start_w = sw;
    g.ctr_h = g.ctr_w = 0.f;
    g.cos_t = 1.f;
    g.sin_t = 0.f;
  }
  g.bin_h = rh / (float)PH;
  g.bin_w = rw / (float)PW;
  g.gh = sr > 0 ? sr : (int)ceilf(rh / (float)PH);
  g.gw = sr > 0 ? sr : (int)ceilf(rw / (float)PW);
  if (g.gh < 0) g.gh = 0;
  if (g.gw < 0) g.gw = 0;
  if (dead) g.gh = g.gw = 0;
  int c = g.gh * g.gw;
  g.count_raw = (float)c;
  g.inv_count = 1.0f / (float)(c < 1 ? 1 : c);
  return g;
}

struct Tap1 {
  int lo, hi;
  float wl, wh;
};

__device__ __forceinline__ Tap1 make_tap1(float v, int size) {
  Tap1 t;
  if (v < -1.0f || v > (float)size) {
    t.lo = t.hi = 0;
    t.wl = t.wh = 0.f;
    return t;
  }
  v = fmaxf(v, 0.f);
  int lo = (int)v;
  int hi;
  if (lo >= size - 1) {
    hi = lo = size - 1;
    v = (float)lo;
  } else {
    hi = lo + 1;
  }
  float l = v - (float)lo;
  t.lo = lo;
  t.hi = hi;
  t.wh = l;
  t.wl = 1.f - l;
  return t;
}

struct Tap2 {
  int p1, p2, p3, p4;
  float w1, w2, w3, w4;
};

__device__ __forceinline__ Tap2 make_tap2(float y, float x, int H, int W) {
  Tap2 t;
  if (y < -1.0f || y > (float)H || x < -1.0f || x > (float)W) {
    t.p1 = t.p2 = t.p3 = t.p4 = -1;
    t.w1 = t.w2 = t.w3 = t.w4 = 0.f;
    return t;
  }
  Tap1 ty = make_tap1(y, H), tx = make_tap1(x, W);
  t.p1 = ty.lo * W + tx.lo;
  t.p2 = ty.lo * W + tx.hi;
  t.p3 = ty.hi * W + tx.lo;
  t.p4 = ty.hi * W + tx.hi;
  t.w1 = ty.wl * tx.wl;
  t.w2 = ty.wl * tx.wh;
  t.w3 = ty.wh * tx.wl;
  t.w4 = ty.wh * tx.wh;
  return t;
}

__device__ __forceinline__ void rot_xy(const RoiGeom& g, int ph, int pw, int iy, int ix, float& y, float& x) {
  float yy = g.start_h + (float)ph * g.bin_h + ((float)iy + .5f) * g.bin_h / (float)g.gh;
  float xx = g.start_w + (float)pw * g.bin_w + ((float)ix + .5f) * g.bin_w / (float)g.gw;
  y = yy * g.cos_t - xx * g.sin_t + g.ctr_h;
  x = yy * g.sin_t + xx * g.cos_t + g.ctr_w;
}

template <int MAXTAP>
__global__ void __launch_bounds__(kThreads) roi_align_rot_fwd_kernel(const Pyr P, const float* __restrict__ rois,
                                                                     int C, int PH, int PW, int sr, int c_per_cta,
                                                                     float* __restrict__ out) {
  __shared__ Tap2 taps[MAXTAP];
  const int k = blockIdx.x;
  const int c0 = blockIdx.y * c_per_cta;
  const int cn = min(c_per_cta, C - c0);
  const int lvl_raw = pick_level<true>(P, rois + (size_t)k * 6);
  const int lvl = max(lvl_raw, 0);
  const float* __restrict__ in = P.feat[lvl];
  const int H = P.H[lvl], W = P.W[lvl];
  const RoiGeom g = load_geom<true>(rois + (size_t)k * 6, P.scale[lvl], PH, PW, sr, 1, lvl_raw < 0);
  const int bins = PH * PW;
  const int spb = g.gh * g.gw;
  const long long ntap = (long long)bins * spb;
  const bool tab = ntap <= MAXTAP;
  if (tab) {
    for (int i = threadIdx.x; i < (int)ntap; i += kThreads) {
      int bin = i / spb, s = i - bin * spb;
      int ph = bin / PW, pw = bin - ph * PW, iy = s / g.gw, ix = s - iy * g.gw;
      float y, x;
      rot_xy(g, ph, pw, iy, ix, y, x);
      taps[i] = make_tap2(y, x, H, W);
    }
    __syncthreads();
  }
  const int total = cn * bins;
  const float* __restrict__ base = in + ((size_t)g.b * C + c0) * H * W;
  float* __restrict__ obase = out + ((size_t)k * C + c0) * bins;
  for (int idx = threadIdx.x; idx < total; idx += kThreads) {
    int c = idx / bins, bin = idx - c * bins;
    int ph = bin / PW, pw = bin - ph * PW;
    const float* __restrict__ plane = base + (size_t)c * H * W;
    float acc = 0.f;
    for (int s = 0; s < spb; ++s) {
      Tap2 t;
      if (tab) t = taps[bin * spb + s];
      else {
        int iy = s / g.gw, ix = s - iy * g.gw;
        float y, x;
        rot_xy(g, ph, pw, iy, ix, y, x);
        t = make_tap2(y, x, H, W);
      }
      if (t.p1 >= 0)
        acc += t.w1 * __ldg(plane + t.p1) + t.w2 * __ldg(plane + t.p2) + t.w3 * __ldg(plane + t.p3) +
               t.w4 * __ldg(plane + t.p4);
    }
    obase[idx] = acc * g.inv_count;
  }
}

template <bool ROT>
__global__ void __launch_bounds__(kThreads) roi_align_bwd_kernel(const Pyr P, const float* __restrict__ gout,
                                                                 const float* __restrict__ rois, int C, int PH, int PW,
                                                                 int sr, int aligned, int c_per_cta) {
  const int k = blockIdx.x;
  const int c0 = blockIdx.y * c_per_cta;
  const int cn = min(c_per_cta, C - c0);
  const int lvl_raw = ROT ? pick_level<true>(P, rois + (size_t)k * 6)
                          : pick_level(P, (P.level_rois ? P.level_rois : rois) + (size_t)k * 5);
  const int lvl = max(lvl_raw, 0);
  float* __restrict__ gin = P.grad[lvl];
  const int H = P.H[lvl], W = P.W[lvl];
  const RoiGeom g = load_geom<ROT>(rois + (size_t)k * (ROT ? 6 : 5), P.scale[lvl], PH, PW, sr, aligned, lvl_raw < 0);
  if (g.gh <= 0 || g.gw <= 0) return;
  const int bins = PH * PW;
  const int total = cn * bins;
  float* __restrict__ base = gin + ((size_t)g.b * C + c0) * H * W;
  const float* __restrict__ gbase = gout + ((size_t)k * C + c0) * bins;
  for (int idx = threadIdx.x; idx < total; idx += kThreads) {
    int c = idx / bins, bin = idx - c * bins;
    int ph = bin / PW, pw = bin - ph * PW;
    float* __restrict__ plane = base + (size_t)c * H * W;
    const float gv = gbase[idx];
    for (int iy = 0; iy < g.gh; ++iy)
      for (int ix = 0; ix < g.gw; ++ix) {
        float y, x;
        if (ROT) rot_xy(g, ph, pw, iy, ix, y, x);
        else {
          y = g.start_h + (float)ph * g.bin_h + ((float)iy + .5f) * g.bin_h / (float)g.gh;
          x = g.start_w + (float)pw * g.bin_w + ((float)ix + .5f) * g.bin_w / (float)g.gw;
        }
        Tap2 t = make_tap2(y, x, H, W);
        if (t.p1 < 0) continue;
        atomicAdd(plane + t.p1, gv * t.w1 / g.count_raw);
        atomicAdd(plane + t.p2, gv * t.w2 / g.count_raw);
        atomicAdd(plane + t.p3, gv * t.w3 / g.count_raw);
        atomicAdd(plane + t.p4, gv * t.w4 / g.count_raw);
      }
  }
}

constexpr int kMaxE = 32;
constexpr int kMaxP = 16;
constexpr int kChW = 4;
constexpr int kV3Warps = 8;
constexpr int kV3Threads = kV3Warps * 32;
constexpr int kCapPx = 448;
constexpr int kRowoffCap = 1536;

struct CTap {
  int idx;
  float w;
};

__device__ __forceinline__ void add_tap(CTap* list, int stride, int& n, int idx, float w, int& overflow) {
  if (w == 0.f) return;
  for (int e = 0; e < n; ++e)
    if (list[e * stride].idx == idx) {
      list[e * stride].w += w;
      return;
    }
  if (n >= kMaxE) {
    overflow = 1;
    return;
  }
  list[n * stride].idx = idx;
  list[n * stride].w = w;
  ++n;
}

template <bool BWD>
__global__ void __launch_bounds__(kV3Threads, 3) roi_align_v3_kernel(const Pyr P, const float* __restrict__ rois, int C,
                                                                     int PH, int PW, int sr, int aligned,
                                                                     int groups_per_cta, const float* __restrict__ gout,
                                                                     float* __restrict__ out) {
  extern __shared__ __align__(16) float stage_all[];
  __shared__ CTap ytab[kMaxE * kMaxP];
  __shared__ CTap xtab[kMaxE * kMaxP];
  __shared__ int rowoff[kRowoffCap];
  __shared__ int yn[kMaxP], xn[kMaxP], ylo[kMaxP], yhi[kMaxP];
  __shared__ int band_ph0[kMaxP + 1], band_yb[kMaxP], band_npx[kMaxP];
  __shared__ int s_overflow, s_tapov, s_xmin, s_xmax, s_nbands, s_direct, s_nyu, s_nxu, s_ymin, s_ymax;

  const int k = blockIdx.x;
  const int tid = threadIdx.x, lane = tid & 31, warp = tid >> 5;
  const int lvl_raw = pick_level(P, (P.level_rois ? P.level_rois : rois) + (size_t)k * 5);
  const int lvl = max(lvl_raw, 0);
  const float* __restrict__ in = BWD ? nullptr : P.feat[lvl];
  float* __restrict__ gin = BWD ? P.grad[lvl] : nullptr;
  const int H = P.H[lvl], W = P.W[lvl];
  const RoiGeom g = load_geom<false>(rois + (size_t)k * 5, P.scale[lvl], PH, PW, sr, aligned, lvl_raw < 0);
  const int bins = PH * PW;
  const int ngroup = d2b_cdiv(C, kChW);
  const int g_begin = blockIdx.y * groups_per_cta, g_end = min(ngroup, g_begin + groups_per_cta);

  if (tid == 0) {
    s_overflow = (PH > kMaxP || PW > kMaxP) ? 1 : 0;
    s_tapov = 0;
    s_xmin = 1 << 30;
    s_xmax = -1;
  }
  __syncthreads();
  if (!s_overflow) {
    if (tid < PH) {
      CTap* list = ytab + tid;
      int n = 0, ov = 0, lo = 1 << 30, hi = -1;
      for (int iy = 0; iy < g.gh; ++iy) {
        Tap1 t = make_tap1(g.start_h + (float)tid * g.bin_h + ((float)iy + .5f) * g.bin_h / (float)g.gh, H);
        add_tap(list, kMaxP, n, t.lo, t.wl, ov);
        add_tap(list, kMaxP, n, t.hi, t.wh, ov);
      }
      for (int e = 0; e < n; ++e) {
        lo = min(lo, list[e * kMaxP].idx);
        hi = max(hi, list[e * kMaxP].idx);
      }
      yn[tid] = n;
      ylo[tid] = lo;
      yhi[tid] = hi;
      if (ov) atomicOr(&s_tapov, 1);
    } else if (tid >= 32 && tid < 32 + PW) {
      const int pw = tid - 32;
      CTap* list = xtab + pw;
      int n = 0, ov = 0;
      for (int ix = 0; ix < g.gw; ++ix) {
        Tap1 t = make_tap1(g.start_w + (float)pw * g.bin_w + ((float)ix + .5f) * g.bin_w / (float)g.gw, W);
        add_tap(list, kMaxP, n, t.lo, t.wl, ov);
        add_tap(list, kMaxP, n, t.hi, t.wh, ov);
      }
      for (int e = 0; e < n; ++e) {
        atomicMin(&s_xmin, list[e * kMaxP].idx);
        atomicMax(&s_xmax, list[e * kMaxP].idx);
      }
      xn[pw] = n;
      if (ov) atomicOr(&s_tapov, 1);
    }
  }
  __syncthreads();
  const int xmin = s_xmin, fw = s_xmax - s_xmin + 1;
  if (tid == 0) {
    const int overflow = s_overflow | s_tapov;
    int direct = overflow, nb = 0, nyu = 0, nxu = 0, ymin = 1 << 30, ymax = -1;
    if (!direct) {
      for (int ph = 0; ph < PH; ++ph) {
        nyu = max(nyu, yn[ph]);
        if (yn[ph] > 0) {
          ymin = min(ymin, ylo[ph]);
          ymax = max(ymax, yhi[ph]);
        }
      }
      for (int pw = 0; pw < PW; ++pw) nxu = max(nxu, xn[pw]);
    }
    if (!direct && fw > 0 && ymax >= ymin) {
      if ((long long)(ymax - ymin + 1) * fw > kRowoffCap) direct = 1;
      int ph0 = 0;
      while (ph0 < PH && !direct) {
        int yb = 1 << 30, ye = -1, ph1 = ph0;
        while (ph1 < PH) {
          int nyb = yb, nye = ye;
          if (yn[ph1] > 0) {
            nyb = min(yb, ylo[ph1]);
            nye = max(ye, yhi[ph1]);
          }
          if (nye >= nyb && (nye - nyb + 1) * fw > kCapPx) {
            if (ph1 == ph0) direct = 1;
            break;
          }
          yb = nyb;
          ye = nye;
          ++ph1;
        }
        band_ph0[nb] = ph0;
        band_yb[nb] = (ye >= yb) ? yb : ymin;
        band_npx[nb] = (ye >= yb) ? (ye - yb + 1) * fw : 0;
        ++nb;
        ph0 = ph1;
      }
    } else if (!direct) {
      band_ph0[0] = 0;
      band_yb[0] = 0;
      band_npx[0] = 0;
      nb = 1;
      nyu = nxu = 0;
      ymin = 0;
      ymax = -1;
    }
    band_ph0[nb] = PH;
    s_nbands = nb;
    int mode = overflow ? 2 : (direct ? 1 : 0);
    if (mode == 0 && fw > 0 && ymax >= ymin) {
      int sy = 0, sx = 0;
      for (int ph = 0; ph < PH; ++ph) sy += yn[ph];
      for (int pw = 0; pw < PW; ++pw) sx += xn[pw];
      if (2LL * sy * sx < (long long)(ymax - ymin + 1) * fw) mode = 1;
    }
    direct = mode;
    s_direct = direct;
    s_nyu = nyu;
    s_nxu = nxu;
    s_ymin = ymin;
    s_ymax = ymax;
  }
  __syncthreads();
  const int mode = s_direct;
  const bool direct = mode == 2;
  const int nbands = s_nbands, nyu = s_nyu, nxu = s_nxu, ymin = s_ymin;
  if (mode != 2) {
    if (tid < PH) {
      const int n = yn[tid];
      const int fill = n > 0 ? ytab[tid].idx : 0;
      for (int e = n; e < nyu; ++e) ytab[e * kMaxP + tid] = CTap{fill, 0.f};
    } else if (tid >= 32 && tid < 32 + PW) {
      const int pw = tid - 32, n = xn[pw];
      for (int e = 0; e < n; ++e) xtab[e * kMaxP + pw].idx -= xmin;
      for (int e = n; e < ((nxu + 3) & ~3); ++e) xtab[e * kMaxP + pw] = CTap{0, 0.f};
    }
    if (mode == 0 && fw > 0 && s_ymax >= ymin) {
      const int npx_all = (s_ymax - ymin + 1) * fw;
      for (int i = tid; i < npx_all; i += kV3Threads) {
        const int y = i / fw, x = i - y * fw;
        rowoff[i] = (ymin + y) * W + xmin + x;
      }
    }
  }
  __syncthreads();

  float* __restrict__ st = stage_all + (size_t)warp * kChW * kCapPx;
  for (int grp = g_begin + warp; grp < g_end; grp += kV3Warps) {
    const int c0 = grp * kChW;
    const int cn = min(kChW, C - c0);
    const float* __restrict__ base = BWD ? nullptr : in + ((size_t)g.b * C + c0) * H * W;
    float* __restrict__ gbase = BWD ? gin + ((size_t)g.b * C + c0) * H * W : nullptr;
    float* __restrict__ obase = BWD ? nullptr : out + ((size_t)k * C + c0) * bins;
    const float* __restrict__ gobase = BWD ? gout + ((size_t)k * C + c0) * bins : nullptr;
    if (direct && BWD) {
      for (int idx = lane; idx < cn * bins; idx += 32) {
        const int c = idx / bins, bin = idx - c * bins;
        const int ph = bin / PW, pw = bin - ph * PW;
        float* __restrict__ plane = gbase + (size_t)c * H * W;
        const float gv = gobase[idx] * g.inv_count;
        for (int iy = 0; iy < g.gh; ++iy) {
          Tap1 ty = make_tap1(g.start_h + (float)ph * g.bin_h + ((float)iy + .5f) * g.bin_h / (float)g.gh, H);
          for (int ix = 0; ix < g.gw; ++ix) {
            Tap1 tx = make_tap1(g.start_w + (float)pw * g.bin_w + ((float)ix + .5f) * g.bin_w / (float)g.gw, W);
            atomicAdd(plane + ty.lo * W + tx.lo, gv * ty.wl * tx.wl);
            atomicAdd(plane + ty.lo * W + tx.hi, gv * ty.wl * tx.wh);
            atomicAdd(plane + ty.hi * W + tx.lo, gv * ty.wh * tx.wl);
            atomicAdd(plane + ty.hi * W + tx.hi, gv * ty.wh * tx.wh);
          }
        }
      }
      continue;
    }
    if (direct) {
      for (int idx = lane; idx < cn * bins; idx += 32) {
        const int c = idx / bins, bin = idx - c * bins;
        const int ph = bin / PW, pw = bin - ph * PW;
        const float* __restrict__ plane = base + (size_t)c * H * W;
        float acc = 0.f;
        for (int iy = 0; iy < g.gh; ++iy) {
          Tap1 ty = make_tap1(g.start_h + (float)ph * g.bin_h + ((float)iy + .5f) * g.bin_h / (float)g.gh, H);
          const float* __restrict__ r0 = plane + (size_t)ty.lo * W;
          const float* __restrict__ r1 = plane + (size_t)ty.hi * W;
          for (int ix = 0; ix < g.gw; ++ix) {
            Tap1 tx = make_tap1(g.start_w + (float)pw * g.bin_w + ((float)ix + .5f) * g.bin_w / (float)g.gw, W);
            acc += (ty.wl * tx.wl) * __ldg(r0 + tx.lo) + (ty.wl * tx.wh) * __ldg(r0 + tx.hi) +
                   (ty.wh * tx.wl) * __ldg(r1 + tx.lo) + (ty.wh * tx.wh) * __ldg(r1 + tx.hi);
          }
        }
        obase[idx] = acc * g.inv_count;
      }
      continue;
    }
    const float* __restrict__ pl[kChW];
    float* __restrict__ gpl[kChW];
#pragma unroll
    for (int q = 0; q < kChW; ++q) {
      pl[q] = BWD ? nullptr : base + (size_t)min(q, cn - 1) * H * W;
      gpl[q] = BWD ? gbase + (size_t)min(q, cn - 1) * H * W : nullptr;
    }

    if (BWD && mode == 1) {
      for (int b0 = 0; b0 < bins; b0 += 32) {
        const int bin = b0 + lane;
        if (bin >= bins) continue;
        const int ph = bin / PW, pw = bin - (bin / PW) * PW;
        float gv[kChW];
#pragma unroll
        for (int q = 0; q < kChW; ++q) gv[q] = q < cn ? gobase[q * bins + bin] * g.inv_count : 0.f;
        for (int ey = 0; ey < nyu; ++ey) {
          const CTap ty = ytab[ey * kMaxP + ph];
          if (ty.w == 0.f) continue;
          const int rbase = ty.idx * W + xmin;
          for (int ex = 0; ex < nxu; ++ex) {
            const CTap tx = xtab[ex * kMaxP + pw];
            const float wgt = ty.w * tx.w;
            if (wgt == 0.f) continue;
#pragma unroll
            for (int q = 0; q < kChW; ++q)
              if (q < cn) atomicAdd(gpl[q] + rbase + tx.idx, wgt * gv[q]);
          }
        }
      }
      continue;
    }
    if (BWD) {
      for (int band = 0; band < nbands; ++band) {
        const int ph0 = band_ph0[band], ph1 = band_ph0[band + 1];
        const int yb = band_yb[band], npx = band_npx[band];
        const int ylast = yb + (fw > 0 ? npx / fw : 0) - 1;
        const int* __restrict__ ro = rowoff + (yb - ymin) * fw;
        __syncwarp();
        for (int i = lane; i < npx; i += 32) {
#pragma unroll
          for (int q = 0; q < kChW; ++q) st[i * kChW + q] = 0.f;
        }
        __syncwarp();
        const int nbin = (ph1 - ph0) * PW;
        for (int b0 = 0; b0 < nbin; b0 += 32) {
          const int bin = b0 + lane;
          if (bin >= nbin) continue;
          const int dph = bin / PW;
          const int ph = ph0 + dph, pw = bin - dph * PW;
          float gv[kChW];
#pragma unroll
          for (int q = 0; q < kChW; ++q) gv[q] = q < cn ? gobase[q * bins + ph * PW + pw] * g.inv_count : 0.f;
          for (int ey = 0; ey < nyu; ++ey) {
            const CTap ty = ytab[ey * kMaxP + ph];
            if (ty.w == 0.f) continue;
            float* __restrict__ srow = st + (min(max(ty.idx, yb), ylast) - yb) * fw * kChW;
            for (int ex = 0; ex < nxu; ++ex) {
              const CTap tx = xtab[ex * kMaxP + pw];
              const float wgt = ty.w * tx.w;
              if (wgt == 0.f) continue;
#pragma unroll
              for (int q = 0; q < kChW; ++q) atomicAdd(srow + tx.idx * kChW + q, wgt * gv[q]);
            }
          }
        }
        __syncwarp();
        for (int i = lane; i < npx; i += 32) {
          const int off = ro[i];
#pragma unroll
          for (int q = 0; q < kChW; ++q) {
            const float v = st[i * kChW + q];
            if (q < cn && v != 0.f) atomicAdd(gpl[q] + off, v);
          }
        }
      }
      continue;
    }

    if (mode == 1) {
      for (int b0 = 0; b0 < bins; b0 += 32) {
        const int bin = b0 + lane;
        const bool live = bin < bins;
        const int bb = live ? bin : 0;
        const int ph = bb / PW, pw = bb - (bb / PW) * PW;
        float acc[kChW];
#pragma unroll
        for (int q = 0; q < kChW; ++q) acc[q] = 0.f;
        for (int ey = 0; ey < nyu; ++ey) {
          const CTap ty = ytab[ey * kMaxP + ph];
          const int rbase = ty.idx * W + xmin;
          float r[kChW];
#pragma unroll
          for (int q = 0; q < kChW; ++q) r[q] = 0.f;
          for (int ex = 0; ex < nxu; ex += 4) {
            CTap tx[4];
            float v[4][kChW];
#pragma unroll
            for (int e = 0; e < 4; ++e) tx[e] = xtab[(ex + e) * kMaxP + pw];
#pragma unroll
            for (int e = 0; e < 4; ++e)
#pragma unroll
              for (int q = 0; q < kChW; ++q) v[e][q] = __ldg(pl[q] + rbase + tx[e].idx);
#pragma unroll
            for (int e = 0; e < 4; ++e)
#pragma unroll
              for (int q = 0; q < kChW; ++q) r[q] = fmaf(tx[e].w, v[e][q], r[q]);
          }
#pragma unroll
          for (int q = 0; q < kChW; ++q) acc[q] = fmaf(ty.w, r[q], acc[q]);
        }
        if (live) {
#pragma unroll
          for (int q = 0; q < kChW; ++q)
            if (q < cn) obase[q * bins + bin] = acc[q] * g.inv_count;
        }
      }
      continue;
    }

    for (int band = 0; band < nbands; ++band) {
      const int ph0 = band_ph0[band], ph1 = band_ph0[band + 1];
      const int yb = band_yb[band], npx = band_npx[band];
      const int ylast = yb + (fw > 0 ? npx / fw : 0) - 1;
      const int* __restrict__ ro = rowoff + (yb - ymin) * fw;
      __syncwarp();
      for (int pix = lane; pix < npx; pix += 64) {
        const bool two = pix + 32 < npx;
        const int o0 = ro[pix], o1 = two ? ro[pix + 32] : o0;
        float a[kChW], b[kChW];
#pragma unroll
        for (int q = 0; q < kChW; ++q) {
          a[q] = __ldg(pl[q] + o0);
          b[q] = __ldg(pl[q] + o1);
        }
        static_assert(kChW == 4, "one float4 per pixel");
        *reinterpret_cast<float4*>(st + pix * kChW) = make_float4(a[0], a[1], a[2], a[3]);
        if (two) *reinterpret_cast<float4*>(st + (pix + 32) * kChW) = make_float4(b[0], b[1], b[2], b[3]);
      }
      __syncwarp();
      const int nbin = (ph1 - ph0) * PW;
      for (int b0 = 0; b0 < nbin; b0 += 32) {
        const int bin = b0 + lane;
        const bool live = bin < nbin;
        const int bb = live ? bin : 0;
        const int dph = bb / PW;
        const int ph = ph0 + dph, pw = bb - dph * PW;
        float acc[kChW];
#pragma unroll
        for (int q = 0; q < kChW; ++q) acc[q] = 0.f;
        for (int ey = 0; ey < nyu; ++ey) {
          const CTap ty = ytab[ey * kMaxP + ph];
          const float* __restrict__ srow = st + (min(max(ty.idx, yb), ylast) - yb) * fw * kChW;
          float r[kChW];
#pragma unroll
          for (int q = 0; q < kChW; ++q) r[q] = 0.f;
          for (int ex = 0; ex < nxu; ++ex) {
            const CTap tx = xtab[ex * kMaxP + pw];
            const float4 dv = *reinterpret_cast<const float4*>(srow + tx.idx * kChW);
            r[0] = fmaf(tx.w, dv.x, r[0]);
            r[1] = fmaf(tx.w, dv.y, r[1]);
            r[2] = fmaf(tx.w, dv.z, r[2]);
            r[3] = fmaf(tx.w, dv.w, r[3]);
          }
#pragma unroll
          for (int q = 0; q < kChW; ++q) acc[q] = fmaf(ty.w, r[q], acc[q]);
        }
        if (live) {
#pragma unroll
          for (int q = 0; q < kChW; ++q)
            if (q < cn) obase[q * bins + ph * PW + pw] = acc[q] * g.inv_count;
        }
      }
    }
  }
}

static int launch_fwd(const Pyr& P, const float* rois, int K, int C, int PH, int PW, int sr, int aligned, float* out,
                      cudaStream_t stream, const float* gout = nullptr) {
  const size_t smem = sizeof(float) * (size_t)kV3Warps * kChW * kCapPx;
  if (gout) D2B_ALLOW_BIG_SMEM(roi_align_v3_kernel<true>);
  else D2B_ALLOW_BIG_SMEM(roi_align_v3_kernel<false>);
  const int ngroup = d2b_cdiv(C, kChW);
  int groups_per_cta = ngroup;
  while (groups_per_cta > kV3Warps && (long long)K * d2b_cdiv(ngroup, groups_per_cta) < 24LL * d2b_num_sms())
    groups_per_cta = (groups_per_cta + 1) / 2;
  dim3 grid(K, d2b_cdiv(ngroup, groups_per_cta));
  if (gout) roi_align_v3_kernel<true><<<grid, kV3Threads, smem, stream>>>(P, rois, C, PH, PW, sr, aligned, groups_per_cta, gout, nullptr);
  else roi_align_v3_kernel<false><<<grid, kV3Threads, smem, stream>>>(P, rois, C, PH, PW, sr, aligned, groups_per_cta, nullptr, out);
  D2B_CHECK_LAUNCH();
  return D2B_OK;
}

int pick_c_per_cta(int K, int C) {
  int cpc = C;
  while (cpc > 16 && (long long)K * d2b_cdiv(C, cpc) < 4LL * d2b_num_sms()) cpc = (cpc + 1) / 2;
  return cpc;
}

constexpr int kNhwcCh = 128;
constexpr int kNhwcChunk = 64;
constexpr int kNhwcThreads = 224;

struct F2 {
  float x, y;
};
__device__ __forceinline__ F2 f2_pack(float a, float b) { return F2{a, b}; }
__device__ __forceinline__ void f2_unpack(F2 p, float& a, float& b) {
  a = p.x;
  b = p.y;
}
__device__ __forceinline__ F2 f2_fma(F2 w, F2 v, F2 c) { return F2{__fmaf_rn(w.x, v.x, c.x), __fmaf_rn(w.y, v.y, c.y)}; }

template <int XC, int RY>
__device__ __forceinline__ void nhwc_bin(const char* __restrict__ base, const CTap* __restrict__ yt0,
                                         const CTap* __restrict__ xt0, int ny, int nx, float4& acc) {
  F2 a01 = f2_pack(acc.x, acc.y), a23 = f2_pack(acc.z, acc.w);
  for (int x0 = 0; x0 < nx; x0 += XC) {
    unsigned xo[XC];
    F2 xw[XC];
#pragma unroll
    for (int e = 0; e < XC; ++e) {
      const CTap t = xt0[(x0 + e) * kMaxP];
      xo[e] = (unsigned)t.idx;
      xw[e] = f2_pack(t.w, t.w);
    }
    for (int ey = 0; ey < ny; ey += RY) {
      const char* __restrict__ rowp[RY];
      F2 wy[RY];
#pragma unroll
      for (int j = 0; j < RY; ++j) {
        const CTap t = yt0[(ey + j) * kMaxP];
        rowp[j] = base + (size_t)(unsigned)t.idx;
        wy[j] = f2_pack(t.w, t.w);
      }
      float4 v[RY][XC];
#pragma unroll
      for (int j = 0; j < RY; ++j)
#pragma unroll
        for (int e = 0; e < XC; ++e) v[j][e] = __ldg(reinterpret_cast<const float4*>(rowp[j] + xo[e]));
#pragma unroll
      for (int j = 0; j < RY; ++j) {
        F2 r01 = f2_pack(0.f, 0.f), r23 = r01;
#pragma unroll
        for (int e = 0; e < XC; ++e) {
          r01 = f2_fma(xw[e], f2_pack(v[j][e].x, v[j][e].y), r01);
          r23 = f2_fma(xw[e], f2_pack(v[j][e].z, v[j][e].w), r23);
        }
        a01 = f2_fma(wy[j], r01, a01);
        a23 = f2_fma(wy[j], r23, a23);
      }
    }
  }
  f2_unpack(a01, acc.x, acc.y);
  f2_unpack(a23, acc.z, acc.w);
}

constexpr int kColCap = 192;

__device__ __forceinline__ void nhwc_emit(float* __restrict__ o, int chunk_pad, F2 c01, F2 c23, float inv, bool first) {
  float a, b, c, d;
  f2_unpack(c01, a, b);
  f2_unpack(c23, c, d);
  o[0] = fmaf(a, inv, first ? 0.f : o[0]);
  o[32 * chunk_pad] = fmaf(b, inv, first ? 0.f : o[32 * chunk_pad]);
  o[64 * chunk_pad] = fmaf(c, inv, first ? 0.f : o[64 * chunk_pad]);
  o[96 * chunk_pad] = fmaf(d, inv, first ? 0.f : o[96 * chunk_pad]);
}

template <int RY, int XC>
__device__ __forceinline__ void nhwc_unit(const char* __restrict__ base, const CTap* __restrict__ yt0, int ny, int nch,
                                          const float4* __restrict__ colE, int cb, int ce, int skip, float* __restrict__ o,
                                          int chunk_pad, float inv) {
  for (int ch = 0; ch < nch; ++ch) {
    unsigned ro[RY];
    float wy[RY];
#pragma unroll
    for (int j = 0; j < RY; ++j) {
      const int e = ch * RY + j;
      const CTap t = yt0[(e < ny ? e : 0) * kMaxP];
      ro[j] = (unsigned)t.idx;
      wy[j] = e < ny ? t.w : 0.f;
    }
    const F2 z = f2_pack(0.f, 0.f);
    F2 c01 = z, c23 = z, n01 = z, n23 = z;
    int b = -skip;
    for (int s = cb; s < ce; s += XC) {
      float4 en[XC];
      float4 v[XC][RY];
#pragma unroll
      for (int x = 0; x < XC; ++x) {
        en[x] = colE[s + x];
        const char* __restrict__ cp = base + (size_t)(unsigned)__float_as_int(en[x].x);
#pragma unroll
        for (int j = 0; j < RY; ++j) v[x][j] = __ldg(reinterpret_cast<const float4*>(cp + ro[j]));
      }
#pragma unroll
      for (int x = 0; x < XC; ++x) {
        const bool live = XC == 1 || s + x < ce;
        F2 t01 = z, t23 = z;
#pragma unroll
        for (int j = 0; j < RY; ++j) {
          const F2 w = f2_pack(wy[j], wy[j]);
          t01 = f2_fma(w, f2_pack(v[x][j].x, v[x][j].y), t01);
          t23 = f2_fma(w, f2_pack(v[x][j].z, v[x][j].w), t23);
        }
        const float wa = live ? en[x].y : 0.f, wb = live ? en[x].z : 0.f;
        const F2 a2 = f2_pack(wa, wa), b2 = f2_pack(wb, wb);
        c01 = f2_fma(a2, t01, c01);
        c23 = f2_fma(a2, t23, c23);
        n01 = f2_fma(b2, t01, n01);
        n23 = f2_fma(b2, t23, n23);
        if (live && __float_as_int(en[x].w) != 0) {
          if (b >= 0) nhwc_emit(o + b, chunk_pad, c01, c23, inv, ch == 0);
          c01 = n01;
          c23 = n23;
          n01 = z;
          n23 = z;
          ++b;
        }
      }
    }
  }
}

template <int ODT>
__global__ void __launch_bounds__(kNhwcThreads, 4) roi_align_nhwc_kernel(const Pyr P, const float* __restrict__ rois, int C, int PH,
                                                             int PW, int sr, int aligned, int chunk, int chunk_pad,
                                                             void* __restrict__ out_v) {
  extern __shared__ __align__(16) float otile[];
  __shared__ CTap ytab[kMaxE * kMaxP];
  __shared__ CTap xtab[kMaxE * kMaxP];
  __shared__ int yn[kMaxP], xn[kMaxP];
  __shared__ int ynr[kMaxP], xnr[kMaxP];
  __shared__ float4 colE[kColCap];
  __shared__ int cbeg[kMaxP + 1];
  __shared__ int s_overflow, s_tapov, s_colok, s_nymax;
  __shared__ RoiGeom sg;

  const int k = blockIdx.x;
  const int c0 = blockIdx.y * kNhwcCh;
  const int tid = threadIdx.x, lane = tid & 31, warp = tid >> 5, nwarps = blockDim.x >> 5;
  const int lvl_raw = pick_level(P, (P.level_rois ? P.level_rois : rois) + (size_t)k * 5);
  const int lvl = max(lvl_raw, 0);
  const int H = P.H[lvl], W = P.W[lvl];
  const int bins = PH * PW;
  const int C4 = C >> 2;
  const int ncta = min(kNhwcCh, C - c0);
  const bool lane_live = lane * 4 < ncta;
  if (tid == 0) {
    s_overflow = (PH > kMaxP || PW > kMaxP) ? 1 : 0;
    s_tapov = 0;
    s_colok = 0;
    s_nymax = 0;
    sg = load_geom<false>(rois + (size_t)k * 5, P.scale[lvl], PH, PW, sr, aligned, lvl_raw < 0);
  }
  __syncthreads();
  const float4* __restrict__ base =
      reinterpret_cast<const float4*>(P.feat[lvl]) + (size_t)sg.b * H * W * C4 + (c0 >> 2) + (lane_live ? lane : 0);
  const char* __restrict__ base_b = reinterpret_cast<const char*>(base);
  if (!s_overflow) {
    if (tid < PH) {
      const RoiGeom g = sg;
      CTap* list = ytab + tid;
      int n = 0, ov = 0;
      for (int iy = 0; iy < g.gh; ++iy) {
        Tap1 t = make_tap1(g.start_h + (float)tid * g.bin_h + ((float)iy + .5f) * g.bin_h / (float)g.gh, H);
        add_tap(list, kMaxP, n, t.lo, t.wl, ov);
        add_tap(list, kMaxP, n, t.hi, t.wh, ov);
      }
      for (int e = 0; e < n; ++e) list[e * kMaxP].idx *= W * C4 * 16;
      ynr[tid] = n;
      atomicMax(&s_nymax, n);
      if (n > 0)
        for (; n & 1; ++n) list[n * kMaxP] = CTap{list[0].idx, 0.f};
      yn[tid] = n;
      if (ov) atomicOr(&s_tapov, 1);
    } else if (warp == 1) {
      const int pw = lane;
      const bool act = pw < PW;
      const RoiGeom g = sg;
      CTap* list = xtab + pw;
      int n = 0, ov = 0;
      if (act) {
        for (int ix = 0; ix < g.gw; ++ix) {
          Tap1 t = make_tap1(g.start_w + (float)pw * g.bin_w + ((float)ix + .5f) * g.bin_w / (float)g.gw, W);
          add_tap(list, kMaxP, n, t.lo, t.wl, ov);
          add_tap(list, kMaxP, n, t.hi, t.wh, ov);
        }
        for (int e = 0; e < n; ++e) list[e * kMaxP].idx *= C4 * 16;
        xnr[pw] = n;
        if (ov) atomicOr(&s_tapov, 1);
      }
      __syncwarp();
      const int n1 = act && pw >= 1 ? xnr[pw - 1] : 0, n2 = act && pw >= 2 ? xnr[pw - 2] : 0;
      const int n3 = act && pw + 1 < PW ? xnr[pw + 1] : 0;
      int own = 0, bad = ov;
      unsigned ownmask = 0;
      for (int e = 0; e < n; ++e) {
        const int c = list[e * kMaxP].idx;
        bool in1 = false, in2 = false;
        for (int q = 0; q < n1; ++q) in1 |= xtab[q * kMaxP + pw - 1].idx == c;
        for (int q = 0; q < n2; ++q) in2 |= xtab[q * kMaxP + pw - 2].idx == c;
        if (in1 && in2) bad = 1;
        if (!in1) {
          ++own;
          ownmask |= 1u << e;
        }
      }
      const int cnt = act ? max(own, 1) : 0;
      int incl = cnt;
#pragma unroll
      for (int d = 1; d < 32; d <<= 1) {
        const int t = __shfl_up_sync(0xffffffffu, incl, d);
        if (lane >= d) incl += t;
      }
      const int beg = incl - cnt;
      const int total = __shfl_sync(0xffffffffu, incl, 31);
      if (total + 4 > kColCap) bad = 1;
      int padded = act ? (n == 0 ? 0 : (n <= 4 ? 4 : (n + 7) & ~7)) : 0;
#pragma unroll
      for (int d = 16; d; d >>= 1) padded += __shfl_xor_sync(0xffffffffu, padded, d);
      if (total * 5 > padded * 4) bad = 1;
      bad = __any_sync(0xffffffffu, bad);
      if (!bad) {
        if (act) {
          cbeg[pw] = beg;
          int i = beg;
          for (int e = 0; e < n; ++e)
            if (ownmask >> e & 1u) {
              const CTap t = list[e * kMaxP];
              float wb = 0.f;
              for (int q = 0; q < n3; ++q)
                if (xtab[q * kMaxP + pw + 1].idx == t.idx) wb = xtab[q * kMaxP + pw + 1].w;
              ++i;
              colE[i - 1] = make_float4(__int_as_float(t.idx), t.w, wb, __int_as_float(i == beg + own ? 1 : 0));
            }
          if (own == 0) colE[beg] = make_float4(__int_as_float(0), 0.f, 0.f, __int_as_float(1));
        }
        if (lane < 4) colE[total + lane] = make_float4(__int_as_float(0), 0.f, 0.f, __int_as_float(0));
        if (lane == 0) {
          cbeg[PW] = total;
          s_colok = 1;
        }
      }
      __syncwarp();
      if (act) {
        if (n > 0)
          for (const int m = n <= 4 ? 3 : 7; n & m; ++n) list[n * kMaxP] = CTap{list[0].idx, 0.f};
        xn[pw] = n;
      }
    }
  }
  __syncthreads();
  const bool onfly = (s_overflow | s_tapov) != 0;

  {
    const int bin0 = blockIdx.z * chunk;
    const int nb = min(chunk, bins - bin0);
    const bool shared_cols = !onfly && s_colok && s_nymax <= 6 && PW % 7 == 0 && chunk % 7 == 0;
    if (shared_cols) {
      const float inv_count = sg.inv_count;
      for (int u = warp; u * 7 < nb; u += nwarps) {
        const int fb = bin0 + u * 7;
        const int ph = fb / PW, pw0 = fb - ph * PW;
        const int ny = ynr[ph];
        float* __restrict__ o = otile + lane * chunk_pad + u * 7;
        if (ny == 0) {
#pragma unroll
          for (int b = 0; b < 7; ++b) o[b] = o[b + 32 * chunk_pad] = o[b + 64 * chunk_pad] = o[b + 96 * chunk_pad] = 0.f;
          continue;
        }
        const int skip = pw0 > 0 ? 1 : 0;
        const int cb = cbeg[pw0 - skip], ce = cbeg[pw0 + 7];
        const int nch = (ny + 5) / 6, ry = (ny + nch - 1) / nch;
        const CTap* __restrict__ yt0 = ytab + ph;
        switch (ry) {
          case 1: nhwc_unit<1, 4>(base_b, yt0, ny, nch, colE, cb, ce, skip, o, chunk_pad, inv_count); break;
          case 2: nhwc_unit<2, 3>(base_b, yt0, ny, nch, colE, cb, ce, skip, o, chunk_pad, inv_count); break;
          case 3: nhwc_unit<3, 2>(base_b, yt0, ny, nch, colE, cb, ce, skip, o, chunk_pad, inv_count); break;
          case 4: nhwc_unit<4, 1>(base_b, yt0, ny, nch, colE, cb, ce, skip, o, chunk_pad, inv_count); break;
          case 5: nhwc_unit<5, 1>(base_b, yt0, ny, nch, colE, cb, ce, skip, o, chunk_pad, inv_count); break;
          default: nhwc_unit<6, 1>(base_b, yt0, ny, nch, colE, cb, ce, skip, o, chunk_pad, inv_count); break;
        }
      }
    } else
    for (int bl = warp; bl < nb; bl += nwarps) {
      const int bin = bin0 + bl;
      const int ph = bin / PW, pw = bin - ph * PW;
      float4 acc = make_float4(0.f, 0.f, 0.f, 0.f);
      if (!onfly) {
        const int ny = yn[ph], nx = xn[pw];
        if (nx <= 4) nhwc_bin<4, 2>(base_b, ytab + ph, xtab + pw, ny, nx, acc);
        else nhwc_bin<8, 1>(base_b, ytab + ph, xtab + pw, ny, nx, acc);
      } else {
        const RoiGeom g = sg;
        for (int iy = 0; iy < g.gh; ++iy) {
          const Tap1 ty = make_tap1(g.start_h + (float)ph * g.bin_h + ((float)iy + .5f) * g.bin_h / (float)g.gh, H);
          const float4* __restrict__ r0 = base + ty.lo * W * C4;
          const float4* __restrict__ r1 = base + ty.hi * W * C4;
          for (int ix = 0; ix < g.gw; ++ix) {
            const Tap1 tx = make_tap1(g.start_w + (float)pw * g.bin_w + ((float)ix + .5f) * g.bin_w / (float)g.gw, W);
            const float4 v1 = __ldg(r0 + tx.lo * C4), v2 = __ldg(r0 + tx.hi * C4);
            const float4 v3 = __ldg(r1 + tx.lo * C4), v4 = __ldg(r1 + tx.hi * C4);
            const float w1 = ty.wl * tx.wl, w2 = ty.wl * tx.wh, w3 = ty.wh * tx.wl, w4 = ty.wh * tx.wh;
            acc.x += w1 * v1.x + w2 * v2.x + w3 * v3.x + w4 * v4.x;
            acc.y += w1 * v1.y + w2 * v2.y + w3 * v3.y + w4 * v4.y;
            acc.z += w1 * v1.z + w2 * v2.z + w3 * v3.z + w4 * v4.z;
            acc.w += w1 * v1.w + w2 * v2.w + w3 * v3.w + w4 * v4.w;
          }
        }
      }
      float* __restrict__ o = otile + lane * chunk_pad + bl;
      const float inv_count = sg.inv_count;
      o[0] = acc.x * inv_count;
      o[32 * chunk_pad] = acc.y * inv_count;
      o[64 * chunk_pad] = acc.z * inv_count;
      o[96 * chunk_pad] = acc.w * inv_count;
    }
    __syncthreads();
    typename Elem<ODT>::T* __restrict__ obase = reinterpret_cast<typename Elem<ODT>::T*>(out_v) + ((size_t)k * C + c0) * bins + bin0;
    const unsigned magic = 0xFFFFFFFFu / (unsigned)nb + 1u;
    for (int i = tid; i < ncta * nb; i += blockDim.x) {
      const int cl = nb == 1 ? i : (int)__umulhi((unsigned)i, magic), bl = i - cl * nb;
      Elem<ODT>::st(obase + (size_t)cl * bins + bl, otile[((cl & 3) * 32 + (cl >> 2)) * chunk_pad + bl]);
    }
  }
}

static int nhwc_supported(int num_levels, const int* H, const int* W, int C, int PH, int PW, int flags);

static int launch_fwd_nhwc(const Pyr& P, int N, const float* rois, int K, int C, int PH, int PW, int sr, int aligned,
                           void* out, cudaStream_t stream, int out_dt = D2B_F32) {
  if (int rc = nhwc_supported(P.num_levels, P.H, P.W, C, PH, PW, 0)) return rc;
  for (int l = 0; l < P.num_levels; ++l)
    if ((reinterpret_cast<uintptr_t>(P.feat[l]) & 15) != 0) return D2B_EINVAL;
  (void)N;
  const int bins = PH * PW;
  const int slabs = d2b_cdiv(C, kNhwcCh);
  const long long want = d2b_cdiv(8LL * d2b_num_sms(), (long long)K * slabs);
  int nchunks = (int)std::max<long long>(d2b_cdiv(bins, kNhwcChunk), std::min<long long>(want, d2b_cdiv(bins, 8)));
  int chunk = d2b_cdiv(bins, nchunks);
  if (nchunks > 1) chunk = std::min(kNhwcChunk - 1, d2b_cdiv(chunk, 7) * 7);
  nchunks = d2b_cdiv(bins, chunk);
  const int chunk_pad = chunk | 1;
  const size_t smem = sizeof(float) * 128 * (size_t)chunk_pad;
  dim3 grid(K, slabs, nchunks);
  D2B_DISPATCH_DTYPE(out_dt, (roi_align_nhwc_kernel<DT><<<grid, kNhwcThreads, smem, stream>>>(P, rois, C, PH, PW, sr, aligned, chunk,
                                                                                            chunk_pad, out)));
  D2B_CHECK_LAUNCH();
  return D2B_OK;
}

constexpr int kBwdBand = 64;
constexpr int kBwdMaxFw = 96;
constexpr int kBwdThreads = 256;

__device__ __forceinline__ void red_add_v4(float* p, float4 v) {
  asm volatile("red.global.add.v4.f32 [%0], {%1, %2, %3, %4};" ::"l"(p), "f"(v.x), "f"(v.y), "f"(v.z), "f"(v.w) : "memory");
}

template <int GDT>
__device__ void bwd_nhwc_per_sample(const RoiGeom& g, const typename Elem<GDT>::T* __restrict__ go, float* __restrict__ gimg,
                                    int H, int W, int C, int PH, int PW, bool lane_live, int ph0, int PHl) {
  const int lane = threadIdx.x & 31, warp = threadIdx.x >> 5, nwarps = blockDim.x >> 5;
  const int bins = PH * PW;
  for (int bl = warp; bl < PHl * PW; bl += nwarps) {
    const int ph = ph0 + bl / PW, pw = bl - (ph - ph0) * PW, bin = ph * PW + pw;
    float4 gv = make_float4(0.f, 0.f, 0.f, 0.f);
    if (lane_live) {
      const typename Elem<GDT>::T* q = go + (size_t)(lane * 4) * bins + bin;
      gv = make_float4(Elem<GDT>::ld(q) * g.inv_count, Elem<GDT>::ld(q + bins) * g.inv_count,
                       Elem<GDT>::ld(q + 2 * bins) * g.inv_count, Elem<GDT>::ld(q + 3 * bins) * g.inv_count);
    }
    for (int iy = 0; iy < g.gh; ++iy) {
      const Tap1 ty = make_tap1(g.start_h + (float)ph * g.bin_h + ((float)iy + .5f) * g.bin_h / (float)g.gh, H);
      for (int ix = 0; ix < g.gw; ++ix) {
        const Tap1 tx = make_tap1(g.start_w + (float)pw * g.bin_w + ((float)ix + .5f) * g.bin_w / (float)g.gw, W);
        if (!lane_live) continue;
        const float w1 = ty.wl * tx.wl, w2 = ty.wl * tx.wh, w3 = ty.wh * tx.wl, w4 = ty.wh * tx.wh;
        if (w1 != 0.f) red_add_v4(gimg + ((size_t)ty.lo * W + tx.lo) * C, make_float4(gv.x * w1, gv.y * w1, gv.z * w1, gv.w * w1));
        if (w2 != 0.f) red_add_v4(gimg + ((size_t)ty.lo * W + tx.hi) * C, make_float4(gv.x * w2, gv.y * w2, gv.z * w2, gv.w * w2));
        if (w3 != 0.f) red_add_v4(gimg + ((size_t)ty.hi * W + tx.lo) * C, make_float4(gv.x * w3, gv.y * w3, gv.z * w3, gv.w * w3));
        if (w4 != 0.f) red_add_v4(gimg + ((size_t)ty.hi * W + tx.hi) * C, make_float4(gv.x * w4, gv.y * w4, gv.z * w4, gv.w * w4));
      }
    }
  }
}

template <int GDT>
__global__ void __launch_bounds__(kBwdThreads) roi_align_bwd_nhwc_kernel(const Pyr P, const float* __restrict__ rois, int C,
                                                                       int PH, int PW, int sr, int aligned, int rows_per_cta,
                                                                       const void* __restrict__ gout) {
  extern __shared__ __align__(16) float gs[];
  __shared__ float WyT[kBwdBand * kMaxP];
  __shared__ float WxT[kBwdMaxFw * kMaxP];
  __shared__ unsigned char ylo[kBwdBand], yhi[kBwdBand], xlo[kBwdMaxFw], xhi[kBwdMaxFw];
  __shared__ float4 colE[kBwdMaxFw], rowE[kBwdBand];
  __shared__ RoiGeom sg;
  __shared__ int s_xmin, s_xmax, s_ymin, s_ymax, s_wide;

  const int k = blockIdx.x;
  const int c0 = blockIdx.y * kNhwcCh;
  const int tid = threadIdx.x, lane = tid & 31, warp = tid >> 5;
  constexpr int kWarps = kBwdThreads / 32;
  const int lvl_raw = pick_level(P, (P.level_rois ? P.level_rois : rois) + (size_t)k * 5);
  const int lvl = max(lvl_raw, 0);
  const int H = P.H[lvl], W = P.W[lvl];
  const int bins = PH * PW;
  const int ph0 = blockIdx.z * rows_per_cta, PHl = min(rows_per_cta, PH - ph0), bins_l = PHl * PW;
  const int ncta = min(kNhwcCh, C - c0);
  const bool lane_live = lane * 4 < ncta;
  if (tid == 0) {
    sg = load_geom<false>(rois + (size_t)k * 5, P.scale[lvl], PH, PW, sr, aligned, lvl_raw < 0);
    s_xmin = s_ymin = 1 << 30;
    s_xmax = s_ymax = -1;
    s_wide = 0;
  }
  __syncthreads();
  const RoiGeom g = sg;
  float* __restrict__ gimg = P.grad[lvl] + (size_t)g.b * H * W * C + c0 + lane * 4;
  const typename Elem<GDT>::T* __restrict__ go = reinterpret_cast<const typename Elem<GDT>::T*>(gout) + ((size_t)k * C + c0) * bins;

  if (PH > kMaxP || PW > kMaxP) {
    bwd_nhwc_per_sample<GDT>(g, go, gimg, H, W, C, PH, PW, lane_live, ph0, PHl);
    return;
  }
  if (tid < PHl) {
    int lo = 1 << 30, hi = -1;
    for (int iy = 0; iy < g.gh; ++iy) {
      const Tap1 t = make_tap1(g.start_h + (float)(ph0 + tid) * g.bin_h + ((float)iy + .5f) * g.bin_h / (float)g.gh, H);
      if (t.wl != 0.f) { lo = min(lo, t.lo); hi = max(hi, t.lo); }
      if (t.wh != 0.f) { lo = min(lo, t.hi); hi = max(hi, t.hi); }
    }
    if (hi >= 0) {
      atomicMin(&s_ymin, lo);
      atomicMax(&s_ymax, hi);
    }
  } else if (tid >= 32 && tid < 32 + PW) {
    const int pw = tid - 32;
    int lo = 1 << 30, hi = -1;
    for (int ix = 0; ix < g.gw; ++ix) {
      const Tap1 t = make_tap1(g.start_w + (float)pw * g.bin_w + ((float)ix + .5f) * g.bin_w / (float)g.gw, W);
      if (t.wl != 0.f) { lo = min(lo, t.lo); hi = max(hi, t.lo); }
      if (t.wh != 0.f) { lo = min(lo, t.hi); hi = max(hi, t.hi); }
    }
    if (hi >= 0) {
      atomicMin(&s_xmin, lo);
      atomicMax(&s_xmax, hi);
    }
  }
  __syncthreads();
  const int xmin = s_xmin, fw = s_xmax - s_xmin + 1, ymin = s_ymin, ymax = s_ymax;
  if (s_xmax < 0 || ymax < 0) return;
  if (fw > kBwdMaxFw) {
    bwd_nhwc_per_sample<GDT>(g, go, gimg, H, W, C, PH, PW, lane_live, ph0, PHl);
    return;
  }
  for (int i = tid; i < fw * kMaxP; i += kBwdThreads) WxT[i] = 0.f;
  __syncthreads();
  if (tid >= 32 && tid < 32 + PW) {
    const int pw = tid - 32;
    for (int ix = 0; ix < g.gw; ++ix) {
      const Tap1 t = make_tap1(g.start_w + (float)pw * g.bin_w + ((float)ix + .5f) * g.bin_w / (float)g.gw, W);
      if (t.wl != 0.f) WxT[(t.lo - xmin) * kMaxP + pw] += t.wl;
      if (t.wh != 0.f) WxT[(t.hi - xmin) * kMaxP + pw] += t.wh;
    }
  }
  for (int e = tid; e < ncta * bins_l; e += kBwdThreads) {
    const int c = e / bins_l, bin = e - c * bins_l;
    gs[bin * kNhwcCh + ((((c >> 2) ^ bin) & 31) << 2) + (c & 3)] =
        Elem<GDT>::ld(go + (size_t)c * bins + ph0 * PW + bin) * g.inv_count;
  }
  __syncthreads();
  for (int x = tid; x < fw; x += kBwdThreads) {
    int lo = 255, hi = 0, cnt = 0, ia = 0, ib = 0;
    float wa = 0.f, wb = 0.f;
    for (int pw = 0; pw < PW; ++pw) {
      const float w = WxT[x * kMaxP + pw];
      if (w != 0.f) {
        lo = min(lo, pw);
        hi = max(hi, pw + 1);
        if (cnt == 0) { ia = pw; wa = w; }
        else if (cnt == 1) { ib = pw; wb = w; }
        ++cnt;
      }
    }
    xlo[x] = (unsigned char)lo;
    xhi[x] = (unsigned char)hi;
    colE[x] = make_float4(__int_as_float(ia), __int_as_float(ib), wa, wb);
    if (cnt > 2) atomicOr(&s_wide, 1);
  }
  float* __restrict__ Ts = gs + (size_t)bins_l * kNhwcCh + (size_t)warp * PW * kNhwcCh;
  for (int yb = ymin; yb <= ymax; yb += kBwdBand) {
    const int nrow = min(kBwdBand, ymax - yb + 1);
    __syncthreads();
    for (int i = tid; i < nrow * kMaxP; i += kBwdThreads) WyT[i] = 0.f;
    __syncthreads();
    if (tid < PHl) {
      for (int iy = 0; iy < g.gh; ++iy) {
        const Tap1 t = make_tap1(g.start_h + (float)(ph0 + tid) * g.bin_h + ((float)iy + .5f) * g.bin_h / (float)g.gh, H);
        if (t.wl != 0.f && t.lo >= yb && t.lo < yb + nrow) WyT[(t.lo - yb) * kMaxP + tid] += t.wl;
        if (t.wh != 0.f && t.hi >= yb && t.hi < yb + nrow) WyT[(t.hi - yb) * kMaxP + tid] += t.wh;
      }
    }
    __syncthreads();
    for (int y = tid; y < nrow; y += kBwdThreads) {
      int lo = 255, hi = 0, cnt = 0, ia = 0, ib = 0;
      float wa = 0.f, wb = 0.f;
      for (int ph = 0; ph < PHl; ++ph) {
        const float w = WyT[y * kMaxP + ph];
        if (w != 0.f) {
          lo = min(lo, ph);
          hi = max(hi, ph + 1);
          if (cnt == 0) { ia = ph; wa = w; }
          else if (cnt == 1) { ib = ph; wb = w; }
          ++cnt;
        }
      }
      ylo[y] = (unsigned char)lo;
      yhi[y] = (unsigned char)hi;
      rowE[y] = make_float4(__int_as_float(ia), __int_as_float(ib), wa, wb);
      if (cnt > 2) atomicOr(&s_wide, 1);
    }
    __syncthreads();
    if (!s_wide) {
      for (int yr = warp; yr < nrow; yr += kWarps) {
        const float4 re = rowE[yr];
        if (re.z == 0.f && re.w == 0.f) continue;
        const int pa = __float_as_int(re.x), pb = __float_as_int(re.y);
        const F2 wya = f2_pack(re.z, re.z), wyb = f2_pack(re.w, re.w);
        __syncwarp();
        for (int pw = 0; pw < PW; ++pw) {
          const int ba = pa * PW + pw, bb = pb * PW + pw;
          const float4 ga = *reinterpret_cast<const float4*>(gs + ba * kNhwcCh + (((lane ^ ba) & 31) << 2));
          const float4 gb = *reinterpret_cast<const float4*>(gs + bb * kNhwcCh + (((lane ^ bb) & 31) << 2));
          const F2 z = f2_pack(0.f, 0.f);
          const F2 t01 = f2_fma(wyb, f2_pack(gb.x, gb.y), f2_fma(wya, f2_pack(ga.x, ga.y), z));
          const F2 t23 = f2_fma(wyb, f2_pack(gb.z, gb.w), f2_fma(wya, f2_pack(ga.z, ga.w), z));
          float4 tv;
          f2_unpack(t01, tv.x, tv.y);
          f2_unpack(t23, tv.z, tv.w);
          *reinterpret_cast<float4*>(Ts + pw * kNhwcCh + lane * 4) = tv;
        }
        __syncwarp();
        float* __restrict__ grow = gimg + (size_t)(yb + yr) * W * C + (size_t)xmin * C;
        for (int xr = 0; xr < fw; ++xr) {
          const float4 ce = colE[xr];
          if (ce.z == 0.f && ce.w == 0.f) continue;
          const float4 ta = *reinterpret_cast<const float4*>(Ts + __float_as_int(ce.x) * kNhwcCh + lane * 4);
          const float4 tb = *reinterpret_cast<const float4*>(Ts + __float_as_int(ce.y) * kNhwcCh + lane * 4);
          const F2 z = f2_pack(0.f, 0.f), wxa = f2_pack(ce.z, ce.z), wxb = f2_pack(ce.w, ce.w);
          const F2 a01 = f2_fma(wxb, f2_pack(tb.x, tb.y), f2_fma(wxa, f2_pack(ta.x, ta.y), z));
          const F2 a23 = f2_fma(wxb, f2_pack(tb.z, tb.w), f2_fma(wxa, f2_pack(ta.z, ta.w), z));
          float4 acc;
          f2_unpack(a01, acc.x, acc.y);
          f2_unpack(a23, acc.z, acc.w);
          if (lane_live) red_add_v4(grow + (size_t)xr * C, acc);
        }
      }
      continue;
    }
    for (int yr = 0; yr < nrow; ++yr) {
      const int pa = ylo[yr], pb = yhi[yr];
      if (pa >= pb) continue;
      float* __restrict__ grow = gimg + (size_t)(yb + yr) * W * C;
      for (int xr = warp; xr < fw; xr += kWarps) {
        const int qa = xlo[xr], qb = xhi[xr];
        if (qa >= qb) continue;
        float4 acc = make_float4(0.f, 0.f, 0.f, 0.f);
        for (int ph = pa; ph < pb; ++ph) {
          const float wy = WyT[yr * kMaxP + ph];
          for (int pw = qa; pw < qb; ++pw) {
            const float w = wy * WxT[xr * kMaxP + pw];
            const int bin = ph * PW + pw;
            const float4 gv = *reinterpret_cast<const float4*>(gs + bin * kNhwcCh + (((lane ^ bin) & 31) << 2));
            acc.x = fmaf(w, gv.x, acc.x);
            acc.y = fmaf(w, gv.y, acc.y);
            acc.z = fmaf(w, gv.z, acc.z);
            acc.w = fmaf(w, gv.w, acc.w);
          }
        }
        if (lane_live) red_add_v4(grow + (size_t)(xmin + xr) * C, acc);
      }
    }
  }
}

static size_t bwd_nhwc_smem(int rows, int PW) {
  return sizeof(float) * kNhwcCh * ((size_t)rows * PW + (size_t)(kBwdThreads / 32) * PW);
}

static int launch_bwd_nhwc(const Pyr& P, int N, const float* rois, int K, int C, int PH, int PW, int sr, int aligned,
                           const void* gout, cudaStream_t stream, int g_dt = D2B_F32) {
  if (int rc = nhwc_supported(P.num_levels, P.H, P.W, C, PH, PW, D2B_ROI_BACKWARD)) return rc;
  for (int l = 0; l < P.num_levels; ++l)
    if ((reinterpret_cast<uintptr_t>(P.grad[l]) & 15) != 0) return D2B_EINVAL;
  (void)N;
  const int slabs = d2b_cdiv(C, kNhwcCh);
  int rows = PH;
  while (rows > 4 &&
         (bwd_nhwc_smem(rows, PW) > 100 * 1024 || (long long)K * slabs * d2b_cdiv(PH, rows) < 4LL * d2b_num_sms()) &&
         bwd_nhwc_smem(rows, PW) > 56 * 1024)
    rows = (rows + 1) / 2;
  const size_t smem = bwd_nhwc_smem(rows, PW);
  dim3 grid(K, slabs, d2b_cdiv(PH, rows));
  D2B_DISPATCH_DTYPE(g_dt, {
    D2B_ALLOW_BIG_SMEM(roi_align_bwd_nhwc_kernel<DT>);
    roi_align_bwd_nhwc_kernel<DT><<<grid, kBwdThreads, smem, stream>>>(P, rois, C, PH, PW, sr, aligned, rows, gout);
  });
  D2B_CHECK_LAUNCH();
  return D2B_OK;
}

constexpr int kRotMaxTap = 1024;

template <bool BWD, int DT>
__global__ void __launch_bounds__(kBwdThreads) roi_align_rot_nhwc_kernel(const Pyr P, const float* __restrict__ rois, int C,
                                                                       int PH, int PW, int sr, const void* __restrict__ gout,
                                                                       void* __restrict__ out) {
  using E = Elem<DT>;
  extern __shared__ __align__(16) float tile[];
  __shared__ Tap2 taps[kRotMaxTap];
  const int k = blockIdx.x;
  const int c0 = blockIdx.y * kNhwcCh;
  const int tid = threadIdx.x, lane = tid & 31, warp = tid >> 5;
  constexpr int kWarps = kBwdThreads / 32;
  const int lvl_raw = pick_level<true>(P, rois + (size_t)k * 6);
  const int lvl = max(lvl_raw, 0);
  const float* __restrict__ in = BWD ? nullptr : P.feat[lvl];
  float* __restrict__ gin = BWD ? P.grad[lvl] : nullptr;
  const int H = P.H[lvl], W = P.W[lvl];
  const RoiGeom g = load_geom<true>(rois + (size_t)k * 6, P.scale[lvl], PH, PW, sr, 1, lvl_raw < 0);
  const int bins = PH * PW;
  const int spb = g.gh * g.gw;
  const int ncta = min(kNhwcCh, C - c0);
  const bool lane_live = lane * 4 < ncta;
  const bool tab = (long long)bins * spb <= kRotMaxTap;
  const int pitch = bins | 1;
  if (tab) {
    for (int i = tid; i < bins * spb; i += kBwdThreads) {
      const int bin = i / spb, sidx = i - bin * spb;
      const int ph = bin / PW, pw = bin - ph * PW, iy = sidx / g.gw, ix = sidx - iy * g.gw;
      float y, x;
      rot_xy(g, ph, pw, iy, ix, y, x);
      taps[i] = make_tap2(y, x, H, W);
    }
  }
  if (BWD) {
    const typename E::T* __restrict__ go = reinterpret_cast<const typename E::T*>(gout) + ((size_t)k * C + c0) * bins;
    for (int e = tid; e < ncta * bins; e += kBwdThreads) {
      const int c = e / bins, bin = e - c * bins;
      tile[bin * kNhwcCh + ((((c >> 2) ^ bin) & 31) << 2) + (c & 3)] = E::ld(go + e) / g.count_raw;
    }
  }
  __syncthreads();
  const size_t img = (size_t)g.b * H * W * C + c0 + (lane_live ? lane * 4 : 0);
  for (int bin = warp; bin < bins; bin += kWarps) {
    const int ph = bin / PW, pw = bin - ph * PW;
    float4 acc = make_float4(0.f, 0.f, 0.f, 0.f);
    float4 gv = make_float4(0.f, 0.f, 0.f, 0.f);
    if (BWD) gv = *reinterpret_cast<const float4*>(tile + bin * kNhwcCh + (((lane ^ bin) & 31) << 2));
    for (int sidx = 0; sidx < spb; ++sidx) {
      Tap2 t;
      if (tab) t = taps[bin * spb + sidx];
      else {
        const int iy = sidx / g.gw, ix = sidx - iy * g.gw;
        float y, x;
        rot_xy(g, ph, pw, iy, ix, y, x);
        t = make_tap2(y, x, H, W);
      }
      if (t.p1 < 0) continue;
      if (BWD) {
        if (lane_live) {
          float* __restrict__ gb = gin + img;
          red_add_v4(gb + (size_t)t.p1 * C, make_float4(gv.x * t.w1, gv.y * t.w1, gv.z * t.w1, gv.w * t.w1));
          red_add_v4(gb + (size_t)t.p2 * C, make_float4(gv.x * t.w2, gv.y * t.w2, gv.z * t.w2, gv.w * t.w2));
          red_add_v4(gb + (size_t)t.p3 * C, make_float4(gv.x * t.w3, gv.y * t.w3, gv.z * t.w3, gv.w * t.w3));
          red_add_v4(gb + (size_t)t.p4 * C, make_float4(gv.x * t.w4, gv.y * t.w4, gv.z * t.w4, gv.w * t.w4));
        }
      } else {
        const float* __restrict__ fb = in + img;
        const float4 v1 = __ldg(reinterpret_cast<const float4*>(fb + (size_t)t.p1 * C));
        const float4 v2 = __ldg(reinterpret_cast<const float4*>(fb + (size_t)t.p2 * C));
        const float4 v3 = __ldg(reinterpret_cast<const float4*>(fb + (size_t)t.p3 * C));
        const float4 v4 = __ldg(reinterpret_cast<const float4*>(fb + (size_t)t.p4 * C));
        acc.x += t.w1 * v1.x + t.w2 * v2.x + t.w3 * v3.x + t.w4 * v4.x;
        acc.y += t.w1 * v1.y + t.w2 * v2.y + t.w3 * v3.y + t.w4 * v4.y;
        acc.z += t.w1 * v1.z + t.w2 * v2.z + t.w3 * v3.z + t.w4 * v4.z;
        acc.w += t.w1 * v1.w + t.w2 * v2.w + t.w3 * v3.w + t.w4 * v4.w;
      }
    }
    if (!BWD) {
      float* __restrict__ o = tile + lane * pitch + bin;
      o[0] = acc.x * g.inv_count;
      o[32 * pitch] = acc.y * g.inv_count;
      o[64 * pitch] = acc.z * g.inv_count;
      o[96 * pitch] = acc.w * g.inv_count;
    }
  }
  if (!BWD) {
    __syncthreads();
    typename E::T* __restrict__ obase = reinterpret_cast<typename E::T*>(out) + ((size_t)k * C + c0) * bins;
    for (int i = tid; i < ncta * bins; i += kBwdThreads) {
      const int cl = i / bins, bl = i - cl * bins;
      E::st(obase + i, tile[((cl & 3) * 32 + (cl >> 2)) * pitch + bl]);
    }
  }
}

template <bool BWD>
static size_t rot_nhwc_smem(int PH, int PW) {
  return sizeof(float) * 128 * (size_t)(BWD ? PH * PW : ((PH * PW) | 1));
}

static int nhwc_supported(int num_levels, const int* H, const int* W, int C, int PH, int PW, int flags) {
  if (C % 4 != 0) return D2B_EUNSUPPORTED;
  for (int l = 0; l < num_levels; ++l)
    if ((long long)H[l] * W[l] * (C / 4) >= (1LL << 28)) return D2B_EUNSUPPORTED;
  const long long bins = (long long)PH * PW;
  if (flags & D2B_ROI_ROTATED) {
    if (sizeof(float) * 128 * (bins | 1) > 150 * 1024) return D2B_EUNSUPPORTED;
  } else if (flags & D2B_ROI_BACKWARD) {
    int rows = PH;
    while (rows > 4 && bwd_nhwc_smem(rows, PW) > 100 * 1024) rows = (rows + 1) / 2;
    if (bwd_nhwc_smem(rows, PW) > 180 * 1024) return D2B_EUNSUPPORTED;
  } else {
    if ((bins + 6) / 7 > 65535) return D2B_EUNSUPPORTED;
  }
  return D2B_OK;
}

template <bool BWD>
static int launch_rot_nhwc(const Pyr& P, const float* rois, int K, int C, int PH, int PW, int sr, const void* gout, void* out,
                           cudaStream_t stream, int dt = D2B_F32) {
  if (int rc = nhwc_supported(P.num_levels, P.H, P.W, C, PH, PW, D2B_ROI_ROTATED | (BWD ? D2B_ROI_BACKWARD : 0))) return rc;
  const size_t smem = rot_nhwc_smem<BWD>(PH, PW);
  dim3 grid(K, d2b_cdiv(C, kNhwcCh));
  D2B_DISPATCH_DTYPE(dt, {
    D2B_ALLOW_BIG_SMEM((roi_align_rot_nhwc_kernel<BWD, DT>));
    roi_align_rot_nhwc_kernel<BWD, DT><<<grid, kBwdThreads, smem, stream>>>(P, rois, C, PH, PW, sr, gout, out);
  });
  D2B_CHECK_LAUNCH();
  return D2B_OK;
}

struct XposeLevels {
  int num_levels;
  const void* src[D2B_MAX_LEVELS];
  void* dst[D2B_MAX_LEVELS];
  int HW[D2B_MAX_LEVELS];
  int tile_begin[D2B_MAX_LEVELS + 1];
};

template <int SDT>
__global__ void __launch_bounds__(256) nchw_to_nhwc_kernel(const XposeLevels L, int C) {
  __shared__ float tile[32][65];
  int l = 0;
  while (l + 1 < L.num_levels && (int)blockIdx.x >= L.tile_begin[l + 1]) ++l;
  const int HW = L.HW[l];
  const int hw0 = ((int)blockIdx.x - L.tile_begin[l]) * 64;
  const int c0 = blockIdx.y * 32;
  const int tid = threadIdx.x, lane = tid & 31, warp = tid >> 5;
  const typename Elem<SDT>::T* __restrict__ src =
      reinterpret_cast<const typename Elem<SDT>::T*>(L.src[l]) + (size_t)blockIdx.z * C * HW;
  float* __restrict__ dst = reinterpret_cast<float*>(L.dst[l]) + (size_t)blockIdx.z * HW * C;
#pragma unroll
  for (int r = warp; r < 32; r += 8) {
    const int c = c0 + r;
    const int hwa = hw0 + lane, hwb = hw0 + 32 + lane;
    const typename Elem<SDT>::T* __restrict__ p = src + (size_t)min(c, C - 1) * HW;
    tile[r][lane] = hwa < HW ? Elem<SDT>::ld(p + hwa) : 0.f;
    tile[r][lane + 32] = hwb < HW ? Elem<SDT>::ld(p + hwb) : 0.f;
  }
  __syncthreads();
  const int cq = tid & 7;
  const int c = c0 + cq * 4;
#pragma unroll
  for (int half = 0; half < 2; ++half) {
    const int hwl = (tid >> 3) + half * 32;
    const int hw = hw0 + hwl;
    if (hw < HW && c < C) {
      const float4 v = make_float4(tile[cq * 4 + 0][hwl], tile[cq * 4 + 1][hwl], tile[cq * 4 + 2][hwl], tile[cq * 4 + 3][hwl]);
      *reinterpret_cast<float4*>(dst + (size_t)hw * C + c) = v;
    }
  }
}

template <int DDT>
__global__ void __launch_bounds__(256) nhwc_to_nchw_kernel(const XposeLevels L, int C) {
  __shared__ float tile[32][65];
  int l = 0;
  while (l + 1 < L.num_levels && (int)blockIdx.x >= L.tile_begin[l + 1]) ++l;
  const int HW = L.HW[l];
  const int hw0 = ((int)blockIdx.x - L.tile_begin[l]) * 64;
  const int c0 = blockIdx.y * 32;
  const int tid = threadIdx.x, lane = tid & 31, warp = tid >> 5;
  const float* __restrict__ src = reinterpret_cast<const float*>(L.src[l]) + (size_t)blockIdx.z * HW * C;
  typename Elem<DDT>::T* __restrict__ dst = reinterpret_cast<typename Elem<DDT>::T*>(L.dst[l]) + (size_t)blockIdx.z * C * HW;
  const int cq = tid & 7;
  const int c = c0 + cq * 4;
#pragma unroll
  for (int half = 0; half < 2; ++half) {
    const int hwl = (tid >> 3) + half * 32;
    const int hw = hw0 + hwl;
    float4 v = make_float4(0.f, 0.f, 0.f, 0.f);
    if (hw < HW && c < C) v = __ldg(reinterpret_cast<const float4*>(src + (size_t)hw * C + c));
    tile[cq * 4 + 0][hwl] = v.x;
    tile[cq * 4 + 1][hwl] = v.y;
    tile[cq * 4 + 2][hwl] = v.z;
    tile[cq * 4 + 3][hwl] = v.w;
  }
  __syncthreads();
#pragma unroll
  for (int r = warp; r < 32; r += 8) {
    const int cc = c0 + r;
    if (cc >= C) continue;
    typename Elem<DDT>::T* __restrict__ p = dst + (size_t)cc * HW;
    const int hwa = hw0 + lane, hwb = hw0 + 32 + lane;
    if (hwa < HW) Elem<DDT>::st(p + hwa, tile[r][lane]);
    if (hwb < HW) Elem<DDT>::st(p + hwb, tile[r][lane + 32]);
  }
}

}

static bool make_pyr(const d2b_pyramid* pyr, Pyr& P) {
  if (!pyr || pyr->num_levels < 1 || pyr->num_levels > D2B_MAX_LEVELS) return false;
  P = Pyr{};
  P.num_levels = pyr->num_levels;
  for (int l = 0; l < pyr->num_levels; ++l) {
    if (pyr->H[l] <= 0 || pyr->W[l] <= 0) return false;
    P.feat[l] = pyr->feat[l];
    P.grad[l] = pyr->grad[l];
    P.H[l] = pyr->H[l];
    P.W[l] = pyr->W[l];
    P.scale[l] = pyr->scale[l];
  }
  P.min_level = pyr->min_level;
  P.max_level = pyr->max_level;
  P.canonical_level = pyr->canonical_level;
  P.canonical_box_size = pyr->canonical_box_size;
  P.level_rois = pyr->level_rois;
  if (P.num_levels > 1 && P.max_level - P.min_level + 1 != P.num_levels) return false;
  return true;
}

static d2b_pyramid one_level(const float* feat, float* grad, int H, int W, float scale) {
  d2b_pyramid p = {};
  p.num_levels = 1;
  p.feat[0] = feat;
  p.grad[0] = grad;
  p.H[0] = H;
  p.W[0] = W;
  p.scale[0] = scale;
  return p;
}

static int zero_grads(const Pyr& P, int N, int C, cudaStream_t stream) {
  void* zp[D2B_MAX_LEVELS];
  size_t zb[D2B_MAX_LEVELS];
  for (int l = 0; l < P.num_levels; ++l) {
    zp[l] = P.grad[l];
    zb[l] = sizeof(float) * (size_t)N * C * P.H[l] * P.W[l];
  }
  return d2b_zero_buffers(zp, zb, P.num_levels, stream);
}

D2B_API int d2b_roi_pooler_nhwc_supported(const d2b_pyramid* pyr, int C, int pooled_h, int pooled_w, int flags) {
  if (!pyr || pyr->num_levels < 1 || pyr->num_levels > D2B_MAX_LEVELS || C < 0 || pooled_h <= 0 || pooled_w <= 0)
    return D2B_EINVAL;
  return nhwc_supported(pyr->num_levels, pyr->H, pyr->W, C, pooled_h, pooled_w, flags);
}

D2B_API int d2b_roi_align_forward(const float* input, int N, int C, int H, int W, const float* rois, int K,
                                  float spatial_scale, int pooled_h, int pooled_w, int sampling_ratio, int aligned,
                                  float* out, void* stream) {
  const d2b_pyramid p = one_level(input, nullptr, H, W, spatial_scale);
  return d2b_roi_pooler_forward(&p, N, C, rois, K, pooled_h, pooled_w, sampling_ratio, aligned, out, stream);
}

D2B_API int d2b_roi_align_forward_nhwc(const float* input, int N, int C, int H, int W, const float* rois, int K,
                                       float spatial_scale, int pooled_h, int pooled_w, int sampling_ratio,
                                       int aligned, float* out, void* stream) {
  const d2b_pyramid p = one_level(input, nullptr, H, W, spatial_scale);
  return d2b_roi_pooler_forward_nhwc(&p, N, C, rois, K, pooled_h, pooled_w, sampling_ratio, aligned, out, stream);
}

D2B_API int d2b_roi_align_backward(const float* grad_out, const float* rois, int K, float spatial_scale, int pooled_h,
                                   int pooled_w, int N, int C, int H, int W, int sampling_ratio, int aligned,
                                   float* grad_in, void* stream) {
  if (!grad_in || N < 0 || C < 0 || H < 0 || W < 0) return D2B_EINVAL;
  if ((size_t)N * C * H * W == 0) return D2B_OK;
  const d2b_pyramid p = one_level(nullptr, grad_in, H, W, spatial_scale);
  return d2b_roi_pooler_backward(&p, N, C, grad_out, rois, K, pooled_h, pooled_w, sampling_ratio, aligned, stream);
}

D2B_API int d2b_roi_align_backward_nhwc(const float* grad_out, const float* rois, int K, float spatial_scale,
                                        int pooled_h, int pooled_w, int N, int C, int H, int W, int sampling_ratio,
                                        int aligned, float* grad_in, void* stream) {
  if (!grad_in || N < 0 || C < 0 || H < 0 || W < 0) return D2B_EINVAL;
  if ((size_t)N * C * H * W == 0) return D2B_OK;
  const d2b_pyramid p = one_level(nullptr, grad_in, H, W, spatial_scale);
  return d2b_roi_pooler_backward_nhwc(&p, N, C, grad_out, rois, K, pooled_h, pooled_w, sampling_ratio, aligned, stream);
}

D2B_API int d2b_roi_align_rotated_forward(const float* input, int N, int C, int H, int W, const float* rois, int K,
                                          float spatial_scale, int pooled_h, int pooled_w, int sampling_ratio,
                                          float* out, void* stream) {
  if (K == 0 || C == 0) return D2B_OK;
  const d2b_pyramid p = one_level(input, nullptr, H, W, spatial_scale);
  return d2b_roi_pooler_rotated_forward(&p, N, C, rois, K, pooled_h, pooled_w, sampling_ratio, out, stream);
}

D2B_API int d2b_roi_align_rotated_forward_nhwc(const float* input, int N, int C, int H, int W, const float* rois, int K,
                                               float spatial_scale, int pooled_h, int pooled_w, int sampling_ratio,
                                               float* out, void* stream) {
  if (K == 0 || C == 0) return D2B_OK;
  const d2b_pyramid p = one_level(input, nullptr, H, W, spatial_scale);
  return d2b_roi_pooler_rotated_forward_nhwc_t(&p, N, C, rois, K, pooled_h, pooled_w, sampling_ratio, out, D2B_F32, stream);
}

D2B_API int d2b_roi_align_rotated_backward(const float* grad_out, const float* rois, int K, float spatial_scale,
                                           int pooled_h, int pooled_w, int N, int C, int H, int W, int sampling_ratio,
                                           float* grad_in, void* stream) {
  if (!grad_in || N < 0 || C < 0 || H < 0 || W < 0) return D2B_EINVAL;
  if ((size_t)N * C * H * W == 0) return D2B_OK;
  const d2b_pyramid p = one_level(nullptr, grad_in, H, W, spatial_scale);
  return d2b_roi_pooler_rotated_backward(&p, N, C, grad_out, rois, K, pooled_h, pooled_w, sampling_ratio, stream);
}

D2B_API int d2b_roi_align_rotated_backward_nhwc(const float* grad_out, const float* rois, int K, float spatial_scale,
                                                int pooled_h, int pooled_w, int N, int C, int H, int W,
                                                int sampling_ratio, float* grad_in, void* stream) {
  if (!grad_in || N < 0 || C < 0 || H < 0 || W < 0 || (reinterpret_cast<uintptr_t>(grad_in) & 15) != 0) return D2B_EINVAL;
  if ((size_t)N * C * H * W == 0) return D2B_OK;
  const d2b_pyramid p = one_level(nullptr, grad_in, H, W, spatial_scale);
  return d2b_roi_pooler_rotated_backward_nhwc_t(&p, N, C, grad_out, D2B_F32, rois, K, pooled_h, pooled_w, sampling_ratio,
                                                stream);
}

D2B_API int d2b_roi_pooler_forward(const d2b_pyramid* pyr, int N, int C, const float* rois, int K, int pooled_h,
                                   int pooled_w, int sampling_ratio, int aligned, float* out, void* stream) {
  if (K == 0 || C == 0) return D2B_OK;
  Pyr P;
  if (!make_pyr(pyr, P) || !rois || !out || N <= 0 || pooled_h <= 0 || pooled_w <= 0 || K < 0) return D2B_EINVAL;
  for (int l = 0; l < P.num_levels; ++l)
    if (!P.feat[l]) return D2B_EINVAL;
  return launch_fwd(P, rois, K, C, pooled_h, pooled_w, sampling_ratio, aligned, out, (cudaStream_t)stream);
}

D2B_API int d2b_roi_pooler_forward_nhwc_t(const d2b_pyramid* pyr, int N, int C, const float* rois, int K, int pooled_h,
                                          int pooled_w, int sampling_ratio, int aligned, void* out, int out_dtype, void* stream) {
  if (K == 0 || C == 0) return D2B_OK;
  Pyr P;
  if (!make_pyr(pyr, P) || !rois || !out || N <= 0 || pooled_h <= 0 || pooled_w <= 0 || K < 0 || !dtype_ok(out_dtype))
    return D2B_EINVAL;
  for (int l = 0; l < P.num_levels; ++l)
    if (!P.feat[l]) return D2B_EINVAL;
  return launch_fwd_nhwc(P, N, rois, K, C, pooled_h, pooled_w, sampling_ratio, aligned, out, (cudaStream_t)stream, out_dtype);
}

D2B_API int d2b_roi_pooler_forward_nhwc(const d2b_pyramid* pyr, int N, int C, const float* rois, int K, int pooled_h,
                                        int pooled_w, int sampling_ratio, int aligned, float* out, void* stream) {
  return d2b_roi_pooler_forward_nhwc_t(pyr, N, C, rois, K, pooled_h, pooled_w, sampling_ratio, aligned, out, D2B_F32, stream);
}

D2B_API int d2b_pyramid_nchw_to_nhwc_t(const d2b_pyramid* pyr, int N, int C, float* const* dst, int src_dtype, void* stream) {
  if (!pyr || !dst || pyr->num_levels < 1 || pyr->num_levels > D2B_MAX_LEVELS || N < 0 || C < 0 || !dtype_ok(src_dtype))
    return D2B_EINVAL;
  if (N == 0 || C == 0) return D2B_OK;
  if (C % 4 != 0) return D2B_EUNSUPPORTED;
  XposeLevels L = {};
  L.num_levels = pyr->num_levels;
  int tiles = 0;
  for (int l = 0; l < pyr->num_levels; ++l) {
    if (!pyr->feat[l] || !dst[l] || pyr->H[l] <= 0 || pyr->W[l] <= 0) return D2B_EINVAL;
    if ((reinterpret_cast<uintptr_t>(dst[l]) & 15) != 0) return D2B_EINVAL;
    L.src[l] = pyr->feat[l];
    L.dst[l] = dst[l];
    L.HW[l] = pyr->H[l] * pyr->W[l];
    L.tile_begin[l] = tiles;
    tiles += d2b_cdiv(L.HW[l], 64);
  }
  L.tile_begin[pyr->num_levels] = tiles;
  if (N > 65535 || d2b_cdiv(C, 32) > 65535) return D2B_EUNSUPPORTED;
  dim3 grid(tiles, d2b_cdiv(C, 32), N);
  D2B_DISPATCH_DTYPE(src_dtype, (nchw_to_nhwc_kernel<DT><<<grid, 256, 0, (cudaStream_t)stream>>>(L, C)));
  D2B_CHECK_LAUNCH();
  return D2B_OK;
}

D2B_API int d2b_pyramid_nchw_to_nhwc(const d2b_pyramid* pyr, int N, int C, float* const* dst, void* stream) {
  return d2b_pyramid_nchw_to_nhwc_t(pyr, N, C, dst, D2B_F32, stream);
}

D2B_API int d2b_pyramid_nhwc_to_nchw_t(const d2b_pyramid* pyr, int N, int C, void* const* dst, int dst_dtype, void* stream) {
  if (!pyr || !dst || pyr->num_levels < 1 || pyr->num_levels > D2B_MAX_LEVELS || N < 0 || C < 0 || !dtype_ok(dst_dtype))
    return D2B_EINVAL;
  if (N == 0 || C == 0) return D2B_OK;
  if (C % 4 != 0) return D2B_EUNSUPPORTED;
  XposeLevels L = {};
  L.num_levels = pyr->num_levels;
  int tiles = 0;
  for (int l = 0; l < pyr->num_levels; ++l) {
    if (!pyr->feat[l] || !dst[l] || pyr->H[l] <= 0 || pyr->W[l] <= 0) return D2B_EINVAL;
    if ((reinterpret_cast<uintptr_t>(pyr->feat[l]) & 15) != 0) return D2B_EINVAL;
    L.src[l] = pyr->feat[l];
    L.dst[l] = dst[l];
    L.HW[l] = pyr->H[l] * pyr->W[l];
    L.tile_begin[l] = tiles;
    tiles += d2b_cdiv(L.HW[l], 64);
  }
  L.tile_begin[pyr->num_levels] = tiles;
  if (N > 65535 || d2b_cdiv(C, 32) > 65535) return D2B_EUNSUPPORTED;
  dim3 grid(tiles, d2b_cdiv(C, 32), N);
  D2B_DISPATCH_DTYPE(dst_dtype, (nhwc_to_nchw_kernel<DT><<<grid, 256, 0, (cudaStream_t)stream>>>(L, C)));
  D2B_CHECK_LAUNCH();
  return D2B_OK;
}

D2B_API int d2b_pyramid_nhwc_to_nchw(const d2b_pyramid* pyr, int N, int C, float* const* dst, void* stream) {
  return d2b_pyramid_nhwc_to_nchw_t(pyr, N, C, reinterpret_cast<void* const*>(dst), D2B_F32, stream);
}

D2B_API int d2b_roi_pooler_backward_nhwc_t(const d2b_pyramid* pyr, int N, int C, const void* grad_out, int grad_dtype,
                                           const float* rois, int K, int pooled_h, int pooled_w, int sampling_ratio, int aligned,
                                           void* stream) {
  Pyr P;
  if (!make_pyr(pyr, P) || N < 0 || C < 0 || !dtype_ok(grad_dtype)) return D2B_EINVAL;
  for (int l = 0; l < P.num_levels; ++l)
    if (!P.grad[l]) return D2B_EINVAL;
  if (int rc = zero_grads(P, N, C, (cudaStream_t)stream)) return rc;
  if (K == 0 || C == 0 || N == 0) return D2B_OK;
  if (!grad_out || !rois || pooled_h <= 0 || pooled_w <= 0) return D2B_EINVAL;
  return launch_bwd_nhwc(P, N, rois, K, C, pooled_h, pooled_w, sampling_ratio, aligned, grad_out, (cudaStream_t)stream, grad_dtype);
}

D2B_API int d2b_roi_pooler_backward_nhwc(const d2b_pyramid* pyr, int N, int C, const float* grad_out, const float* rois,
                                         int K, int pooled_h, int pooled_w, int sampling_ratio, int aligned, void* stream) {
  return d2b_roi_pooler_backward_nhwc_t(pyr, N, C, grad_out, D2B_F32, rois, K, pooled_h, pooled_w, sampling_ratio, aligned, stream);
}

D2B_API int d2b_roi_pooler_backward(const d2b_pyramid* pyr, int N, int C, const float* grad_out, const float* rois,
                                    int K, int pooled_h, int pooled_w, int sampling_ratio, int aligned, void* stream) {
  Pyr P;
  if (!make_pyr(pyr, P) || N < 0 || C < 0) return D2B_EINVAL;
  for (int l = 0; l < P.num_levels; ++l)
    if (!P.grad[l]) return D2B_EINVAL;
  if (int rc = zero_grads(P, N, C, (cudaStream_t)stream)) return rc;
  if (K == 0 || C == 0 || N == 0) return D2B_OK;
  if (!grad_out || !rois || pooled_h <= 0 || pooled_w <= 0) return D2B_EINVAL;
  return launch_fwd(P, rois, K, C, pooled_h, pooled_w, sampling_ratio, aligned, nullptr, (cudaStream_t)stream, grad_out);
}

static int rot_pooler_args(const d2b_pyramid* pyr, int N, int C, int K, int dtype, Pyr& P) {
  if (!make_pyr(pyr, P) || P.level_rois || N < 0 || C < 0 || K < 0 || !dtype_ok(dtype)) return D2B_EINVAL;
  if (N == 0 && K > 0) return D2B_EINVAL;
  return D2B_OK;
}

D2B_API int d2b_roi_pooler_rotated_forward(const d2b_pyramid* pyr, int N, int C, const float* rois, int K, int pooled_h,
                                           int pooled_w, int sampling_ratio, float* out, void* stream) {
  Pyr P;
  if (rot_pooler_args(pyr, N, C, K, D2B_F32, P)) return D2B_EINVAL;
  if (K == 0 || C == 0) return D2B_OK;
  if (!rois || !out || N <= 0 || pooled_h <= 0 || pooled_w <= 0) return D2B_EINVAL;
  for (int l = 0; l < P.num_levels; ++l)
    if (!P.feat[l]) return D2B_EINVAL;
  int cpc = pick_c_per_cta(K, C);
  dim3 grid(K, d2b_cdiv(C, cpc));
  roi_align_rot_fwd_kernel<1024><<<grid, kThreads, 0, (cudaStream_t)stream>>>(P, rois, C, pooled_h, pooled_w, sampling_ratio,
                                                                               cpc, out);
  D2B_CHECK_LAUNCH();
  return D2B_OK;
}

D2B_API int d2b_roi_pooler_rotated_forward_nhwc_t(const d2b_pyramid* pyr, int N, int C, const float* rois, int K, int pooled_h,
                                                  int pooled_w, int sampling_ratio, void* out, int out_dtype, void* stream) {
  Pyr P;
  if (rot_pooler_args(pyr, N, C, K, out_dtype, P)) return D2B_EINVAL;
  if (K == 0 || C == 0) return D2B_OK;
  if (!rois || !out || N <= 0 || pooled_h <= 0 || pooled_w <= 0) return D2B_EINVAL;
  for (int l = 0; l < P.num_levels; ++l)
    if (!P.feat[l] || (reinterpret_cast<uintptr_t>(P.feat[l]) & 15) != 0) return D2B_EINVAL;
  return launch_rot_nhwc<false>(P, rois, K, C, pooled_h, pooled_w, sampling_ratio, nullptr, out, (cudaStream_t)stream,
                                out_dtype);
}

D2B_API int d2b_roi_pooler_rotated_backward(const d2b_pyramid* pyr, int N, int C, const float* grad_out, const float* rois,
                                            int K, int pooled_h, int pooled_w, int sampling_ratio, void* stream) {
  Pyr P;
  if (rot_pooler_args(pyr, N, C, K, D2B_F32, P)) return D2B_EINVAL;
  if (N == 0 || C == 0) return D2B_OK;
  for (int l = 0; l < P.num_levels; ++l)
    if (!P.grad[l]) return D2B_EINVAL;
  if (K > 0 && (!grad_out || !rois || pooled_h <= 0 || pooled_w <= 0)) return D2B_EINVAL;
  int rc = zero_grads(P, N, C, (cudaStream_t)stream);
  if (rc || K == 0) return rc;
  int cpc = pick_c_per_cta(K, C);
  dim3 grid(K, d2b_cdiv(C, cpc));
  roi_align_bwd_kernel<true><<<grid, kThreads, 0, (cudaStream_t)stream>>>(P, grad_out, rois, C, pooled_h, pooled_w,
                                                                          sampling_ratio, 1, cpc);
  D2B_CHECK_LAUNCH();
  return D2B_OK;
}

D2B_API int d2b_roi_pooler_rotated_backward_nhwc_t(const d2b_pyramid* pyr, int N, int C, const void* grad_out, int grad_dtype,
                                                   const float* rois, int K, int pooled_h, int pooled_w, int sampling_ratio,
                                                   void* stream) {
  Pyr P;
  if (rot_pooler_args(pyr, N, C, K, grad_dtype, P)) return D2B_EINVAL;
  if (N == 0 || C == 0) return D2B_OK;
  for (int l = 0; l < P.num_levels; ++l)
    if (!P.grad[l] || (reinterpret_cast<uintptr_t>(P.grad[l]) & 15) != 0) return D2B_EINVAL;
  if (K > 0 && (!grad_out || !rois || pooled_h <= 0 || pooled_w <= 0)) return D2B_EINVAL;
  if (int rc = K > 0 ? nhwc_supported(P.num_levels, P.H, P.W, C, pooled_h, pooled_w, D2B_ROI_ROTATED | D2B_ROI_BACKWARD)
                     : D2B_OK)
    return rc;
  int rc = zero_grads(P, N, C, (cudaStream_t)stream);
  if (rc || K == 0) return rc;
  return launch_rot_nhwc<true>(P, rois, K, C, pooled_h, pooled_w, sampling_ratio, grad_out, nullptr, (cudaStream_t)stream,
                               grad_dtype);
}
```

Measured before the change: 284.6.

## Fuse deformable-conv prepass kernels and enable programmatic dependent launch

```diff
diff --git a/detectron2_b200/csrc/abi.cu b/detectron2_b200/csrc/abi.cu
--- a/detectron2_b200/csrc/abi.cu
+++ b/detectron2_b200/csrc/abi.cu
@@ -5,28 +5,7 @@
 D2B_API const char* d2b_arch(void) { return "sm_90a"; }
 
 namespace {
-struct ZeroList {
-  int n;
-  void* p[D2B_MAX_ZERO];
-  size_t bytes[D2B_MAX_ZERO];
-  size_t blk0[D2B_MAX_ZERO + 1];
-};
-constexpr size_t kZeroChunk = 16384;
-
-__global__ void __launch_bounds__(256) zero_buffers_kernel(const ZeroList z) {
-  int i = 0;
-  while (i + 1 < z.n && blockIdx.x >= z.blk0[i + 1]) ++i;
-  const size_t off = (blockIdx.x - z.blk0[i]) * kZeroChunk;
-  const size_t len = min(kZeroChunk, z.bytes[i] - off);
-  char* base = (char*)z.p[i] + off;
-  if ((reinterpret_cast<uintptr_t>(base) & 15) == 0) {
-    uint4* q = reinterpret_cast<uint4*>(base);
-    for (size_t e = threadIdx.x; e < len / 16; e += 256) q[e] = make_uint4(0u, 0u, 0u, 0u);
-    for (size_t e = (len / 16) * 16 + threadIdx.x; e < len; e += 256) base[e] = 0;
-  } else {
-    for (size_t e = threadIdx.x; e < len; e += 256) base[e] = 0;
-  }
-}
+__global__ void __launch_bounds__(256) zero_buffers_kernel(const D2bZeroList z) { d2b_zero_chunk(z, blockIdx.x); }
 }
 
 int d2b_num_sms() {
@@ -42,17 +21,8 @@
 }
 
 int d2b_zero_buffers(void* const* ptrs, const size_t* bytes, int n, cudaStream_t stream) {
-  ZeroList z = {};
-  size_t blocks = 0;
-  for (int i = 0; i < n && z.n < D2B_MAX_ZERO; ++i) {
-    if (!ptrs[i] || !bytes[i]) continue;
-    z.p[z.n] = ptrs[i];
-    z.bytes[z.n] = bytes[i];
-    z.blk0[z.n] = blocks;
-    blocks += (bytes[i] + kZeroChunk - 1) / kZeroChunk;
-    ++z.n;
-  }
-  z.blk0[z.n] = blocks;
+  D2bZeroList z;
+  const size_t blocks = d2b_zero_list(ptrs, bytes, n, z);
   if (z.n == 0) return D2B_OK;
   if (blocks > 0x7fffffffULL) return D2B_EUNSUPPORTED;
   zero_buffers_kernel<<<(unsigned)blocks, 256, 0, stream>>>(z);
diff --git a/detectron2_b200/csrc/common.cuh b/detectron2_b200/csrc/common.cuh
--- a/detectron2_b200/csrc/common.cuh
+++ b/detectron2_b200/csrc/common.cuh
@@ -27,6 +27,89 @@
 #define D2B_MAX_ZERO 8
 int d2b_zero_buffers(void* const* ptrs, const size_t* bytes, int n, cudaStream_t stream);
 
+struct D2bZeroList {
+  int n;
+  void* p[D2B_MAX_ZERO];
+  size_t bytes[D2B_MAX_ZERO];
+  size_t blk0[D2B_MAX_ZERO + 1];
+};
+constexpr size_t kD2bZeroChunk = 16384;
+
+inline size_t d2b_zero_list(void* const* ptrs, const size_t* bytes, int n, D2bZeroList& z) {
+  z = D2bZeroList{};
+  size_t blocks = 0;
+  for (int i = 0; i < n && z.n < D2B_MAX_ZERO; ++i) {
+    if (!ptrs[i] || !bytes[i]) continue;
+    z.p[z.n] = ptrs[i];
+    z.bytes[z.n] = bytes[i];
+    z.blk0[z.n] = blocks;
+    blocks += (bytes[i] + kD2bZeroChunk - 1) / kD2bZeroChunk;
+    ++z.n;
+  }
+  z.blk0[z.n] = blocks;
+  return blocks;
+}
+
+__device__ __forceinline__ void d2b_zero_chunk(const D2bZeroList& z, size_t blk) {
+  int i = 0;
+  while (i + 1 < z.n && blk >= z.blk0[i + 1]) ++i;
+  const size_t off = (blk - z.blk0[i]) * kD2bZeroChunk;
+  const size_t len = min(kD2bZeroChunk, z.bytes[i] - off);
+  char* base = (char*)z.p[i] + off;
+  if ((reinterpret_cast<uintptr_t>(base) & 15) == 0) {
+    uint4* q = reinterpret_cast<uint4*>(base);
+    for (size_t e = threadIdx.x; e < len / 16; e += 256) q[e] = make_uint4(0u, 0u, 0u, 0u);
+    for (size_t e = (len / 16) * 16 + threadIdx.x; e < len; e += 256) base[e] = 0;
+  } else {
+    for (size_t e = threadIdx.x; e < len; e += 256) base[e] = 0;
+  }
+}
+
+template <class T, class Load>
+__device__ __forceinline__ void d2b_nchw_to_nhwc_tile(const T* __restrict__ src, float* __restrict__ dst, int C, int HW,
+                                                      int hw0, int c0, float (&tile)[32][65], Load ld) {
+  const int tid = threadIdx.x, lane = tid & 31, warp = tid >> 5;
+#pragma unroll
+  for (int r = warp; r < 32; r += 8) {
+    const int c = c0 + r;
+    const int hwa = hw0 + lane, hwb = hw0 + 32 + lane;
+    const T* __restrict__ p = src + (size_t)min(c, C - 1) * HW;
+    tile[r][lane] = hwa < HW ? ld(p + hwa) : 0.f;
+    tile[r][lane + 32] = hwb < HW ? ld(p + hwb) : 0.f;
+  }
+  __syncthreads();
+  const int cq = tid & 7;
+  const int c = c0 + cq * 4;
+#pragma unroll
+  for (int half = 0; half < 2; ++half) {
+    const int hwl = (tid >> 3) + half * 32;
+    const int hw = hw0 + hwl;
+    if (hw < HW && c < C) {
+      const float4 v = make_float4(tile[cq * 4 + 0][hwl], tile[cq * 4 + 1][hwl], tile[cq * 4 + 2][hwl], tile[cq * 4 + 3][hwl]);
+      *reinterpret_cast<float4*>(dst + (size_t)hw * C + c) = v;
+    }
+  }
+}
+
+__device__ __forceinline__ void grid_dep_wait() { asm volatile("griddepcontrol.wait;" ::: "memory"); }
+__device__ __forceinline__ void grid_dep_launch() { asm volatile("griddepcontrol.launch_dependents;" ::: "memory"); }
+
+template <class... Params, class... Args>
+inline cudaError_t d2b_launch_dependent(void (*kernel)(Params...), dim3 grid, dim3 block, size_t smem, cudaStream_t stream,
+                                        Args&&... args) {
+  cudaLaunchAttribute attr = {};
+  attr.id = cudaLaunchAttributeProgrammaticStreamSerialization;
+  attr.val.programmaticStreamSerializationAllowed = 1;
+  cudaLaunchConfig_t cfg = {};
+  cfg.gridDim = grid;
+  cfg.blockDim = block;
+  cfg.dynamicSmemBytes = smem;
+  cfg.stream = stream;
+  cfg.attrs = &attr;
+  cfg.numAttrs = 1;
+  return cudaLaunchKernelEx(&cfg, kernel, static_cast<Params>(args)...);
+}
+
 #define D2B_ALLOW_BIG_SMEM(kernel)                                                                              \
   do {                                                                                                          \
     static std::atomic<unsigned long long> done__{0ull};                                                        \
diff --git a/detectron2_b200/csrc/deform_conv_tc.cu b/detectron2_b200/csrc/deform_conv_tc.cu
--- a/detectron2_b200/csrc/deform_conv_tc.cu
+++ b/detectron2_b200/csrc/deform_conv_tc.cu
@@ -347,6 +347,8 @@
     }
   }
   __syncthreads();
+  grid_dep_launch();
+  grid_dep_wait();
   if (warp < kWorkerWarps) reg_alloc<kWorkerRegs>();
   else reg_dealloc<kSideRegs>();
 
@@ -452,6 +454,8 @@
     mbar_init_fence();
   }
   __syncthreads();
+  grid_dep_launch();
+  grid_dep_wait();
   if (warp < kWorkerWarps) reg_alloc<kWorkerRegs>();
   else reg_dealloc<kSideRegs>();
 
@@ -538,6 +542,8 @@
     }
   }
   __syncthreads();
+  grid_dep_launch();
+  grid_dep_wait();
   if (warp < kWorkerWarps) reg_alloc<kWorkerRegs>();
   else reg_dealloc<kSideRegs>();
 
@@ -723,6 +729,8 @@
 }
 
 __global__ void dcn_gw_reduce_kernel(const float* __restrict__ part, const TC d, float* __restrict__ gw) {
+  grid_dep_launch();
+  grid_dep_wait();
   const long long total = (long long)d.SG * d.U * 64 * d.ops;
   const long long idx = (long long)blockIdx.x * blockDim.x + threadIdx.x;
   if (idx >= total) return;
@@ -746,6 +754,8 @@
   const int cb = c0 >> 6, ch0 = c0 & 63;
   const int ocl0 = blockIdx.y * kRedOc;
   const int tid = threadIdx.x;
+  grid_dep_launch();
+  grid_dep_wait();
   {
     const int j = tid & (kRedOc - 1), r0 = tid / kRedOc;
     for (int row = r0; row < d.KK * kRedCh; row += 256 / kRedOc) {
@@ -792,6 +802,8 @@
     mbar_init_fence();
   }
   __syncthreads();
+  grid_dep_launch();
+  grid_dep_wait();
   if (warp < kWorkerWarps) reg_alloc<kWorkerRegs>();
   else reg_dealloc<kSideRegs>();
 
@@ -921,6 +933,8 @@
     fence_proxy_async();
   }
   __syncthreads();
+  grid_dep_launch();
+  grid_dep_wait();
   if (warp < kWorkerWarps) reg_alloc<kWorkerRegs>();
   else reg_dealloc<kSideRegs>();
 
@@ -981,8 +995,8 @@
   return __ldg(w + ((size_t)oc * d.cpg + (c - g * d.cpg)) * d.KK + kp);
 }
 
-__global__ void dcn_wtile_fwd_kernel(const float* __restrict__ w, const TC d, int BN, int noct, uint8_t* __restrict__ dst) {
-  const long long idx = (long long)blockIdx.x * blockDim.x + threadIdx.x;
+__device__ __forceinline__ void wtile_fwd(long long idx, const float* __restrict__ w, const TC& d, int BN, int noct,
+                                          uint8_t* __restrict__ dst) {
   const long long total = (long long)d.SG * noct * d.U * BN * 8;
   if (idx >= total) return;
   const int c16 = (int)(idx & 7);
@@ -1003,8 +1017,7 @@
   *reinterpret_cast<uint4*>(base + BN * 128 + swz128((uint32_t)r, (uint32_t)c16)) = lo;
 }
 
-__global__ void dcn_wtile_bwd_kernel(const float* __restrict__ w, const TC d, uint8_t* __restrict__ dst) {
-  const long long idx = (long long)blockIdx.x * blockDim.x + threadIdx.x;
+__device__ __forceinline__ void wtile_bwd(long long idx, const float* __restrict__ w, const TC& d, uint8_t* __restrict__ dst) {
   const long long total = (long long)d.SG * d.MC * d.nks * 128 * 8;
   if (idx >= total) return;
   const int c16 = (int)(idx & 7);
@@ -1038,17 +1051,15 @@
   return g;
 }
 
-__global__ void __launch_bounds__(256) dcn_gout_px_tiles_kernel(const float* __restrict__ gout,
-                                                                const float* __restrict__ ysaved, const Epi ep, const TC d,
-                                                                uint8_t* __restrict__ dst, uint8_t* __restrict__ dst_oc,
-                                                                int BN, int noct) {
-  __shared__ float t[64][33];
-  const long long tile = blockIdx.x;
+__device__ __forceinline__ void gout_px_tiles(long long blk, float (&t)[64][33], const float* __restrict__ gout,
+                                              const float* __restrict__ ysaved, const Epi& ep, const TC& d,
+                                              uint8_t* __restrict__ dst, uint8_t* __restrict__ dst_oc, int BN, int noct) {
+  const long long tile = blk >> 2;
   const int ks = (int)(tile % d.nks);
   const int sg = (int)((tile / d.nks) % d.SG);
   const int pt = (int)((tile / ((long long)d.nks * d.SG)) % d.tiles_img);
   const int b = (int)(tile / ((long long)d.nks * d.SG * d.tiles_img));
-  const int r0 = blockIdx.y * 32;
+  const int r0 = (int)(blk & 3) * 32;
   const int p0 = pt * 128 + r0, oc0 = sg * d.ops + ks * 64;
   const int tid = threadIdx.x;
 #pragma unroll
@@ -1090,9 +1101,8 @@
   }
 }
 
-__global__ void dcn_gout_oc_tiles_kernel(const float* __restrict__ gout, const float* __restrict__ ysaved, const Epi ep,
-                                         const TC d, int BN, int noct, uint8_t* __restrict__ dst) {
-  const long long idx = (long long)blockIdx.x * blockDim.x + threadIdx.x;
+__device__ __forceinline__ void gout_oc_tiles(long long idx, const float* __restrict__ gout, const float* __restrict__ ysaved,
+                                              const Epi& ep, const TC& d, int BN, int noct, uint8_t* __restrict__ dst) {
   const long long total = (long long)d.N * d.stages_img * d.SG * noct * BN * 8;
   if (idx >= total) return;
   const int c16 = (int)(idx & 7);
@@ -1117,6 +1127,71 @@
   *reinterpret_cast<uint4*>(base + BN * 128 + swz128((uint32_t)r, (uint32_t)c16)) = lo;
 }
 
+struct XposeX {
+  const float* src;
+  float* dst;
+  int tiles, cblks;
+};
+union PrepassSmem {
+  float g[64][33];
+  float x[32][65];
+};
+
+__device__ __forceinline__ void xpose_x(long long blk, float (&tile)[32][65], const XposeX& X, const TC& d) {
+  const int pt = (int)(blk % X.tiles), cb = (int)((blk / X.tiles) % X.cblks), b = (int)(blk / ((long long)X.tiles * X.cblks));
+  const int HW = d.H * d.W;
+  d2b_nchw_to_nhwc_tile(X.src + (size_t)b * d.Cin * HW, X.dst + (size_t)b * HW * d.Cin, d.Cin, HW, pt * 64, cb * 32, tile,
+                        [](const float* p) { return __ldg(p); });
+}
+
+struct PreFwd {
+  D2bZeroList zero;
+  XposeX X;
+  long long n_zero, n_x;
+  const float* w;
+  uint8_t* wt;
+  int BN, noct;
+};
+__global__ void __launch_bounds__(256) dcn_prepass_fwd_kernel(const PreFwd P, const TC d) {
+  __shared__ PrepassSmem sm;
+  grid_dep_launch();
+  long long blk = blockIdx.x;
+  if (blk < P.n_zero) return d2b_zero_chunk(P.zero, (size_t)blk);
+  blk -= P.n_zero;
+  if (blk < P.n_x) return xpose_x(blk, sm.x, P.X, d);
+  blk -= P.n_x;
+  wtile_fwd(blk * 256 + threadIdx.x, P.w, d, P.BN, P.noct, P.wt);
+}
+
+struct PreBwd {
+  D2bZeroList zero;
+  XposeX X;
+  long long n_gout, n_zero, n_x;
+  const float* gout;
+  const float* ysaved;
+  Epi ep;
+  uint8_t* gt_px;
+  uint8_t* gt_oc;
+  int BN, noct;
+  const float* w;
+  uint8_t* wt;
+};
+__global__ void __launch_bounds__(256) dcn_prepass_bwd_kernel(const PreBwd P, const TC d) {
+  __shared__ PrepassSmem sm;
+  grid_dep_launch();
+  long long blk = blockIdx.x;
+  if (blk < P.n_gout) {
+    if (P.gt_px) return gout_px_tiles(blk, sm.g, P.gout, P.ysaved, P.ep, d, P.gt_px, P.gt_oc, P.BN, P.noct);
+    return gout_oc_tiles(blk * 256 + threadIdx.x, P.gout, P.ysaved, P.ep, d, P.BN, P.noct, P.gt_oc);
+  }
+  blk -= P.n_gout;
+  if (blk < P.n_zero) return d2b_zero_chunk(P.zero, (size_t)blk);
+  blk -= P.n_zero;
+  if (blk < P.n_x) return xpose_x(blk, sm.x, P.X, d);
+  blk -= P.n_x;
+  wtile_bwd(blk * 256 + threadIdx.x, P.w, d, P.wt);
+}
+
 __global__ void __launch_bounds__(256) nhwc_to_nchw_kernel(const float* __restrict__ src, int C, int HW,
                                                            float* __restrict__ dst) {
   __shared__ float t[64][33];
@@ -1124,6 +1199,8 @@
   const float* __restrict__ s = src + (size_t)blockIdx.z * HW * C;
   float* __restrict__ o = dst + (size_t)blockIdx.z * C * HW;
   const int tid = threadIdx.x;
+  grid_dep_launch();
+  grid_dep_wait();
   for (int e = tid; e < 64 * 32; e += 256) {
     const int pp = e >> 5, cc = e & 31;
     t[pp][cc] = (hw0 + pp < HW && c0 + cc < C) ? __ldg(s + (size_t)(hw0 + pp) * C + c0 + cc) : 0.f;
@@ -1136,6 +1213,8 @@
 }
 
 __global__ void dcn_epilogue_kernel(float* __restrict__ y, long long total, int Cout, int HoWo, const Epi ep) {
+  grid_dep_launch();
+  grid_dep_wait();
   const long long i = (long long)blockIdx.x * blockDim.x + threadIdx.x;
   if (i >= total) return;
   const int oc = (int)((i / HoWo) % Cout);
@@ -1146,15 +1225,10 @@
   y[i] = v;
 }
 
-int to_nhwc(const float* x, const TC& d, float* dst, cudaStream_t stream) {
-  d2b_pyramid P = {};
-  P.num_levels = 1;
-  P.feat[0] = x;
-  P.H[0] = d.H;
-  P.W[0] = d.W;
-  P.scale[0] = 1.f;
-  float* dsts[1] = {dst};
-  return d2b_pyramid_nchw_to_nhwc(&P, d.N, d.Cin, dsts, (void*)stream);
+XposeX make_xpose(const float* x, float* dst, const TC& d, bool x_nhwc, long long& ctas) {
+  XposeX X = {x, dst, d2b_cdiv(d.H * d.W, 64), d2b_cdiv(d.Cin, 32)};
+  ctas = x_nhwc ? 0 : (long long)X.tiles * X.cblks * d.N;
+  return X;
 }
 
 }
@@ -1208,18 +1282,8 @@
   uint8_t* ws = reinterpret_cast<uint8_t*>(workspace);
   uint8_t* wt = ws;
   ws += align256((size_t)d.SG * k.noct * d.U * 2 * k.BN * 128);
-  const float* xh = x;
-  if (!x_nhwc) {
-    float* xn = reinterpret_cast<float*>(ws);
-    int rc = to_nhwc(x, d, xn, stream);
-    if (rc) return rc;
-    xh = xn;
-  }
-  {
-    const long long total = (long long)d.SG * k.noct * d.U * k.BN * 8;
-    dcn_wtile_fwd_kernel<<<d2b_cdiv(total, 256), 256, 0, stream>>>(weight, d, k.BN, k.noct, wt);
-    D2B_CHECK_LAUNCH();
-  }
+  float* xn = x_nhwc ? nullptr : reinterpret_cast<float*>(ws);
+  const float* xh = x_nhwc ? x : xn;
   K1P kc;
   bool colfed = false;
   if (cols && k.noct > 1) {
@@ -1229,7 +1293,21 @@
       colfed = true;
     }
   }
-  if (k.red) D2B_CUDA(cudaMemsetAsync(out, 0, sizeof(float) * (size_t)d.N * d.Cout * d.HoWo, stream));
+  {
+    PreFwd P = {};
+    void* zp[1] = {k.red ? out : nullptr};
+    const size_t zb[1] = {sizeof(float) * (size_t)d.N * d.Cout * d.HoWo};
+    P.n_zero = (long long)d2b_zero_list(zp, zb, 1, P.zero);
+    P.X = make_xpose(x, xn, d, x_nhwc, P.n_x);
+    P.w = weight;
+    P.wt = wt;
+    P.BN = k.BN;
+    P.noct = k.noct;
+    const long long ctas = P.n_zero + P.n_x + d2b_cdiv((long long)d.SG * k.noct * d.U * k.BN * 8, 256);
+    if (ctas > 0x7fffffffLL) return D2B_EUNSUPPORTED;
+    dcn_prepass_fwd_kernel<<<(unsigned)ctas, 256, 0, stream>>>(P, d);
+    D2B_CHECK_LAUNCH();
+  }
   const int smem_bytes = k.S * k.stage_bytes + k.tap_bytes + 1024 + 128;
   const int split = precision == 1 ? 1 : 0;
   const Epi ep = {scale, shift, relu};
@@ -1237,15 +1315,14 @@
 #define D2B_LAUNCH_K1(BN)                                                                                              \
   {                                                                                                                    \
     D2B_ALLOW_BIG_SMEM(dcn_fwd_tc_kernel<BN>);                                                                         \
-    dcn_fwd_tc_kernel<BN><<<grid, kThreads, smem_bytes, stream>>>(xh, offset, mask, wt, ep, d, k, split, out,        \
-                                                                    reinterpret_cast<uint8_t*>(cols));                 \
+    D2B_CUDA(d2b_launch_dependent(dcn_fwd_tc_kernel<BN>, grid, kThreads, smem_bytes, stream, xh, offset, mask, wt, ep, d, k, \
+                                  split, out, reinterpret_cast<uint8_t*>(cols)));                                      \
   }
   if (k.BN == 16) D2B_LAUNCH_K1(16)
   else if (k.BN == 32) D2B_LAUNCH_K1(32)
   else if (k.BN == 64) D2B_LAUNCH_K1(64)
   else D2B_LAUNCH_K1(128)
 #undef D2B_LAUNCH_K1
-  D2B_CHECK_LAUNCH();
   if (colfed) {
     const int smem_c = kc.S * kc.stage_bytes + 1024 + 128;
     dim3 grid_c(d.N * d.tiles_img * kc.goct, d.SG, kc.ksplit);
@@ -1253,19 +1330,17 @@
 #define D2B_LAUNCH_K1C(BN)                                                                                             \
   {                                                                                                                    \
     D2B_ALLOW_BIG_SMEM(dcn_fwd_cols_kernel<BN>);                                                                       \
-    dcn_fwd_cols_kernel<BN><<<grid_c, kThreads, smem_c, stream>>>(cl, wt, ep, d, kc, split, out);                      \
+    D2B_CUDA(d2b_launch_dependent(dcn_fwd_cols_kernel<BN>, grid_c, kThreads, smem_c, stream, cl, wt, ep, d, kc, split, out)); \
   }
     if (kc.BN == 16) D2B_LAUNCH_K1C(16)
     else if (kc.BN == 32) D2B_LAUNCH_K1C(32)
     else if (kc.BN == 64) D2B_LAUNCH_K1C(64)
     else D2B_LAUNCH_K1C(128)
 #undef D2B_LAUNCH_K1C
-    D2B_CHECK_LAUNCH();
   }
   if (k.red && (scale || relu)) {
     const long long total = (long long)d.N * d.Cout * d.HoWo;
-    dcn_epilogue_kernel<<<d2b_cdiv(total, 256), 256, 0, stream>>>(out, total, d.Cout, d.HoWo, ep);
-    D2B_CHECK_LAUNCH();
+    D2B_CUDA(d2b_launch_dependent(dcn_epilogue_kernel, d2b_cdiv(total, 256), 256, 0, stream, out, total, d.Cout, d.HoWo, ep));
   }
   return D2B_OK;
 }
@@ -1324,14 +1399,9 @@
   const int split = precision == 1 ? 1 : 0;
   uint8_t* ws = reinterpret_cast<uint8_t*>(workspace);
   const size_t xbytes = align256(sizeof(float) * nx);
-  const float* xh = x;
-  if (!x_nhwc) {
-    float* xn = reinterpret_cast<float*>(ws);
-    ws += xbytes;
-    int rc = to_nhwc(x, d, xn, stream);
-    if (rc) return rc;
-    xh = xn;
-  }
+  float* xn = x_nhwc ? nullptr : reinterpret_cast<float*>(ws);
+  const float* xh = x_nhwc ? x : xn;
+  if (!x_nhwc) ws += xbytes;
   float* gxh = nullptr;
   if (need_data && grad_x) gxh = x_nhwc ? grad_x : reinterpret_cast<float*>(ws);
   uint8_t* gt_px = nullptr;
@@ -1350,38 +1420,40 @@
     gw_part = reinterpret_cast<float*>(ws);
   }
   {
+    PreBwd P = {};
     void* zp[4] = {grad_offset, fused_om ? nullptr : grad_mask, gxh, gw_part};
-    size_t zb[4] = {noff * 4, nm * 4, nx * 4, sizeof(float) * (size_t)d.SG * d.MC * 128 * d.ops};
-    int rc = d2b_zero_buffers(zp, zb, 4, stream);
-    if (rc) return rc;
+    const size_t zb[4] = {noff * 4, nm * 4, nx * 4, sizeof(float) * (size_t)d.SG * d.MC * 128 * d.ops};
+    P.n_zero = (long long)d2b_zero_list(zp, zb, 4, P.zero);
+    P.X = make_xpose(x, xn, d, x_nhwc, P.n_x);
+    P.n_gout = need_data ? (long long)d.N * d.tiles_img * d.SG * d.nks * 4
+                         : d2b_cdiv((long long)d.N * d.stages_img * d.SG * k3.noct * k3.BN * 8, 256);
+    P.gout = grad_out;
+    P.ysaved = y_saved;
+    P.ep = ep;
+    P.gt_px = gt_px;
+    P.gt_oc = gt_oc;
+    P.BN = k3.BN;
+    P.noct = k3.noct;
+    P.w = weight;
+    P.wt = wt;
+    const long long ctas =
+        P.n_gout + P.n_zero + P.n_x + (need_data ? d2b_cdiv((long long)d.SG * d.MC * d.nks * 128 * 8, 256) : 0);
+    if (ctas > 0x7fffffffLL) return D2B_EUNSUPPORTED;
+    dcn_prepass_bwd_kernel<<<(unsigned)ctas, 256, 0, stream>>>(P, d);
+    D2B_CHECK_LAUNCH();
   }
   if (need_data) {
-    dcn_gout_px_tiles_kernel<<<dim3((unsigned)((size_t)d.N * d.tiles_img * d.SG * d.nks), 4), 256, 0, stream>>>(
-        grad_out, y_saved, ep, d, gt_px, gt_oc, k3.BN, k3.noct);
-    D2B_CHECK_LAUNCH();
-    {
-      const long long total = (long long)d.SG * d.MC * d.nks * 128 * 8;
-      dcn_wtile_bwd_kernel<<<d2b_cdiv(total, 256), 256, 0, stream>>>(weight, d, wt);
-      D2B_CHECK_LAUNCH();
-    }
     const int smem_bytes = 2 * 4 * kTile + 128 * kGcolPitch * 4 + k2.tap_bytes + 1024 + 128;
     D2B_ALLOW_BIG_SMEM(dcn_bwd_data_tc_kernel);
     dim3 grid(d.N * d.tiles_img, d.SG, k2.msplit);
-    dcn_bwd_data_tc_kernel<<<grid, kThreads, smem_bytes, stream>>>(xh, offset, mask, gt_px, wt, d, k2, split, gxh, grad_offset,
-                                                                  mask ? grad_mask : nullptr);
-    D2B_CHECK_LAUNCH();
+    D2B_CUDA(d2b_launch_dependent(dcn_bwd_data_tc_kernel, grid, kThreads, smem_bytes, stream, xh, offset, mask, gt_px, wt, d, k2,
+                                  split, gxh, grad_offset, mask ? grad_mask : nullptr));
     if (grad_x && !x_nhwc) {
       dim3 g2(d2b_cdiv(d.H * d.W, 64), d2b_cdiv(d.Cin, 32), d.N);
-      nhwc_to_nchw_kernel<<<g2, 256, 0, stream>>>(gxh, d.Cin, d.H * d.W, grad_x);
-      D2B_CHECK_LAUNCH();
+      D2B_CUDA(d2b_launch_dependent(nhwc_to_nchw_kernel, g2, 256, 0, stream, gxh, d.Cin, d.H * d.W, grad_x));
     }
   }
   if (need_weight) {
-    if (!need_data) {
-      const long long total = (long long)d.N * d.stages_img * d.SG * k3.noct * k3.BN * 8;
-      dcn_gout_oc_tiles_kernel<<<d2b_cdiv(total, 256), 256, 0, stream>>>(grad_out, y_saved, ep, d, k3.BN, k3.noct, gt_oc);
-      D2B_CHECK_LAUNCH();
-    }
     dim3 grid(d.SG * k3.noct, d.MC, k3.nsplit);
     if (cols) {
       const int S = std::min(6, (kMaxSmem - 2048) / k3.stage_bytes);
@@ -1390,7 +1462,8 @@
 #define D2B_LAUNCH_K3C(BN)                                                                                             \
   {                                                                                                                      \
     D2B_ALLOW_BIG_SMEM(dcn_bwd_weight_cols_kernel<BN>);                                                                \
-    dcn_bwd_weight_cols_kernel<BN><<<grid, kThreads, smem_bytes, stream>>>(cl, gt_oc, d, k3, S, split, gw_part);       \
+    D2B_CUDA(d2b_launch_dependent(dcn_bwd_weight_cols_kernel<BN>, grid, kThreads, smem_bytes, stream, cl, gt_oc, d, k3, S, \
+                                  split, gw_part));                                                                     \
   }
       if (k3.BN == 64) D2B_LAUNCH_K3C(64)
       else D2B_LAUNCH_K3C(128)
@@ -1400,21 +1473,19 @@
 #define D2B_LAUNCH_K3(BN)                                                                                              \
   {                                                                                                                      \
     D2B_ALLOW_BIG_SMEM(dcn_bwd_weight_tc_kernel<BN>);                                                                  \
-    dcn_bwd_weight_tc_kernel<BN><<<grid, kThreads, smem_bytes, stream>>>(xh, offset, mask, gt_oc, d, k3, split, gw_part); \
+    D2B_CUDA(d2b_launch_dependent(dcn_bwd_weight_tc_kernel<BN>, grid, kThreads, smem_bytes, stream, xh, offset, mask, gt_oc, d, \
+                                  k3, split, gw_part));                                                                 \
   }
       if (k3.BN == 64) D2B_LAUNCH_K3(64)
       else D2B_LAUNCH_K3(128)
 #undef D2B_LAUNCH_K3
     }
-    D2B_CHECK_LAUNCH();
-    {
-      if (d.KK <= 9) {
-        dcn_gw_reduce_tile_kernel<<<dim3(d.SG * (d.cps / kRedCh), d.ops / kRedOc), 256, 0, stream>>>(gw_part, d, grad_weight);
-      } else {
-        const long long total = (long long)d.SG * d.U * 64 * d.ops;
-        dcn_gw_reduce_kernel<<<d2b_cdiv(total, 256), 256, 0, stream>>>(gw_part, d, grad_weight);
-      }
-      D2B_CHECK_LAUNCH();
+    if (d.KK <= 9) {
+      D2B_CUDA(d2b_launch_dependent(dcn_gw_reduce_tile_kernel, dim3(d.SG * (d.cps / kRedCh), d.ops / kRedOc), 256, 0, stream,
+                                    gw_part, d, grad_weight));
+    } else {
+      const long long total = (long long)d.SG * d.U * 64 * d.ops;
+      D2B_CUDA(d2b_launch_dependent(dcn_gw_reduce_kernel, d2b_cdiv(total, 256), 256, 0, stream, gw_part, d, grad_weight));
     }
   }
   return D2B_OK;
diff --git a/detectron2_b200/csrc/roi_align.cu b/detectron2_b200/csrc/roi_align.cu
--- a/detectron2_b200/csrc/roi_align.cu
+++ b/detectron2_b200/csrc/roi_align.cu
@@ -1465,30 +1465,10 @@
   const int HW = L.HW[l];
   const int hw0 = ((int)blockIdx.x - L.tile_begin[l]) * 64;
   const int c0 = blockIdx.y * 32;
-  const int tid = threadIdx.x, lane = tid & 31, warp = tid >> 5;
-  const typename Elem<SDT>::T* __restrict__ src =
-      reinterpret_cast<const typename Elem<SDT>::T*>(L.src[l]) + (size_t)blockIdx.z * C * HW;
+  using T = typename Elem<SDT>::T;
+  const T* __restrict__ src = reinterpret_cast<const T*>(L.src[l]) + (size_t)blockIdx.z * C * HW;
   float* __restrict__ dst = reinterpret_cast<float*>(L.dst[l]) + (size_t)blockIdx.z * HW * C;
-#pragma unroll
-  for (int r = warp; r < 32; r += 8) {
-    const int c = c0 + r;
-    const int hwa = hw0 + lane, hwb = hw0 + 32 + lane;
-    const typename Elem<SDT>::T* __restrict__ p = src + (size_t)min(c, C - 1) * HW;
-    tile[r][lane] = hwa < HW ? Elem<SDT>::ld(p + hwa) : 0.f;
-    tile[r][lane + 32] = hwb < HW ? Elem<SDT>::ld(p + hwb) : 0.f;
-  }
-  __syncthreads();
-  const int cq = tid & 7;
-  const int c = c0 + cq * 4;
-#pragma unroll
-  for (int half = 0; half < 2; ++half) {
-    const int hwl = (tid >> 3) + half * 32;
-    const int hw = hw0 + hwl;
-    if (hw < HW && c < C) {
-      const float4 v = make_float4(tile[cq * 4 + 0][hwl], tile[cq * 4 + 1][hwl], tile[cq * 4 + 2][hwl], tile[cq * 4 + 3][hwl]);
-      *reinterpret_cast<float4*>(dst + (size_t)hw * C + c) = v;
-    }
-  }
+  d2b_nchw_to_nhwc_tile(src, dst, C, HW, hw0, c0, tile, [](const T* p) { return Elem<SDT>::ld(p); });
 }
 
 template <int DDT>
```

New measurement: 290.0, median of 6. 1.9% higher.
